# nathancunn/ParticleMDI.jl

Hardware: AMD Instinct MI355X
Metric: Gibbs iters/sec (and obs·particles/sec) at 1/2/4/8 GPUs vs CPU ref (higher is better)
Workload: dtype f64

## Files before the change

### include/pmdi_hip.h

```cpp
#ifndef PMDI_HIP_H
#define PMDI_HIP_H

#include <stdint.h>

#ifdef __cplusplus
extern "C" {
#endif

#define PMDI_ABI_VERSION 2
#define PMDI_KMAX 8

enum { PMDI_GAUSSIAN = 0, PMDI_CATEGORICAL = 1, PMDI_NEGBINOM = 2 };

enum {
    PMDI_OK = 0,
    PMDI_E_ARG = -1,
    PMDI_E_DEVICE = -2,
    PMDI_E_MEMORY = -3,
    PMDI_E_POOL = -4,
    PMDI_E_DATA = -5,
    PMDI_E_STATE = -6
};

typedef struct {
    int32_t kind;
    int32_t D;
    int64_t ld;
    const double  *xf;
    const int64_t *xi;
} pmdi_dataset;

typedef struct {
    int32_t settled;
    int32_t continue_inplace;
    int32_t sticky;
    int32_t light_ids;
    int32_t s2_cols, s2_idcap, s2_cls;
    int32_t ksplit;
    int32_t requeue_ksplit;
    int32_t split;
    int32_t heavy_threads;
    int32_t two_per_cu;
    int32_t very_heavy;
    int32_t start_gate;
    int32_t terms_cap;
    int32_t lds_target;
    int32_t phase_timers;
    int32_t profiled;
    int32_t ticket;
    int32_t reserved[5];
} pmdi_tuning;

typedef struct {
    int32_t abi_version;
    int32_t device;
    int32_t K;
    int32_t N;
    int32_t P;
    int32_t n_chains;
    int64_t n;
    uint64_t seed;
    int32_t q1_mode;
    int32_t q2_mode;
    int64_t pool_cap;
    int32_t block_threads;
    int32_t reserved;
    const pmdi_tuning *tuning;
} pmdi_config;

typedef struct pmdi_handle pmdi_handle;

typedef struct {
    int64_t n_operations;
    int64_t n_resamples;
    int64_t n_clones;
    int64_t max_id;
    int64_t sum_classes;
    int64_t steps_fast;
    int64_t steps_converted;
    int64_t steps_fallback;
} pmdi_sweep_stats;

int pmdi_create(const pmdi_config *cfg, const pmdi_dataset *datasets, pmdi_handle **out);

void pmdi_tuning_default(pmdi_tuning *t);
void pmdi_tuning_from_env(pmdi_tuning *t);
int pmdi_destroy(pmdi_handle *h);
const char *pmdi_last_error(void);
int pmdi_abi_version(void);

int pmdi_sweep(pmdi_handle *h, int64_t iter, const int64_t *s_in, const int64_t *order_obs,
               int64_t n1, const double *Pi, const double *Phi, const uint8_t *feature_flag,
               double lw_init, int64_t *s_out, double *logweight, int64_t *p_star,
               pmdi_sweep_stats *stats, double *trace);

int pmdi_sweep_device(pmdi_handle *h, int64_t iter, const int32_t *s_in, const int32_t *order_obs,
                      int64_t n1, const double *Pi, const double *log1p_phi,
                      const uint8_t *feature_flag, double lw_init, int32_t *s_out,
                      double *logweight, int32_t *p_star, int64_t *stats, int32_t *err,
                      void *stream);

int pmdi_feature_select(pmdi_handle *h, int64_t iter, const int64_t *s_traj,
                        uint8_t *feature_flag, double *feature_prob);

int pmdi_export_state(pmdi_handle *h, int32_t chain, int64_t *particle, int64_t *counts,
                      int64_t *cluster_n, int64_t *max_id);

typedef struct pmdi_cluster_batch pmdi_cluster_batch;
int pmdi_clusters_new(pmdi_handle *h, int32_t k, int32_t B, pmdi_cluster_batch **out);
int pmdi_clusters_free(pmdi_cluster_batch *cb);
int pmdi_cluster_add(pmdi_cluster_batch *cb, const int64_t *rows, const uint8_t *feature_flag);
int pmdi_calc_logprob(pmdi_cluster_batch *cb, const int64_t *obs_rows, const uint8_t *feature_flag,
                      double *out);
int pmdi_calc_logmarginal(pmdi_cluster_batch *cb, double *out );
int pmdi_cluster_stats(pmdi_cluster_batch *cb, double *out, int64_t *stride);

int pmdi_label_counts_device(pmdi_handle *h, const int32_t *s, int32_t *counts, void *stream);

int pmdi_psm_counts_device(int32_t device, const uint8_t *samples, int64_t S, int32_t K, int64_t n,
                           int64_t row_lo, int64_t row_hi, int32_t n_labels, int32_t *counts, void *stream);

enum { PMDI_LINK_SINGLE = 0, PMDI_LINK_AVERAGE = 1, PMDI_LINK_COMPLETE = 2, PMDI_LINK_WARD = 3 };
int pmdi_psm_distance_device(int32_t device, const int32_t *counts, int64_t S, int32_t K, int64_t n, int32_t which,
                             double *dist_out, void *stream);
int pmdi_hclust_device(int32_t device, double *dist, int32_t B, int64_t n, int32_t linkage, int64_t *merges_out,
                       double *heights_out, int64_t *order_out, void *stream);
int pmdi_cutree(int64_t n, const int64_t *merges, const double *heights, int64_t k, double h, int64_t *labels_out);

int pmdi_psm_score_device(int32_t device, const int32_t *counts, int64_t S, int32_t K, int64_t n, int32_t which,
                          const int32_t *cand, int64_t B, int64_t ld,
                          int64_t *agree_out , int64_t *pairs_out , int64_t *total_out ,
                          void *stream);

#define PMDI_REFINE_GMAX 4096
int pmdi_psm_rowscore_device(int32_t device, const int32_t *counts, int64_t S, int32_t K, int64_t n, int32_t which,
                             const int32_t *cand, int64_t B, int64_t ld,
                             int64_t *own_out , int32_t *size_out ,
                             int64_t *rowtotal_out , void *stream);
int pmdi_psm_refine_device(int32_t device, const int32_t *counts, int64_t S, int32_t K, int64_t n, int32_t which,
                           const int32_t *start, int64_t B, int64_t ld, int32_t max_sweeps,
                           int32_t *labels_out , int64_t *moves_out ,
                           int32_t *sweeps_out , void *stream);

int pmdi_vi_log2_table(int32_t *out );
int pmdi_psm_refine_vi_device(int32_t device, const int32_t *counts, int64_t S, int32_t K, int64_t n, int32_t which,
                              const int32_t *start, int64_t B, int64_t ld, int32_t max_sweeps,
                              int32_t *labels_out , int64_t *moves_out ,
                              int32_t *sweeps_out , int64_t *objective_out ,
                              void *stream);

#define PMDI_PARTDIST_GMAX 255
int pmdi_partition_rows_device(int32_t device, const void *labels , int32_t is_bytes, int64_t R, int64_t n, int64_t ld,
                               int32_t G, uint8_t *bytes_out , int64_t *pairs_out ,
                               int64_t *hl_out , int32_t *nclust_out , void *stream);
int pmdi_partition_distance_device(int32_t device, const uint8_t *cand_bytes , int64_t B, int32_t Gc,
                                   const uint8_t *draw_bytes , int64_t R, int32_t Gd, int64_t n,
                                   int64_t *both_out , int64_t *jl_out , void *stream);

int pmdi_partition_refine_device(int32_t device, const uint8_t *draw_bytes , int64_t R, int32_t Gd, int64_t n,
                                 const int32_t *start , int64_t B, int64_t ld, int32_t gcap, int32_t loss ,
                                 int32_t max_sweeps, int32_t *labels_out , int64_t *moves_out ,
                                 int32_t *sweeps_out , int32_t *converged_out ,
                                 int64_t *marginal_out , int64_t *joint_out , void *stream);

#define PMDI_BLOCKSUM_GMAX 2048
int pmdi_psm_blocksum_device(int32_t device, const int32_t *counts, int64_t S, int32_t K, int64_t n,
                             const int32_t *group , int32_t G,
                             int64_t *out , void *stream);

enum { PMDI_DATA_RAW = 0, PMDI_DATA_SQDEV = 1, PMDI_DATA_ZBIN = 2, PMDI_DATA_LEVELS = 3 };
int pmdi_data_groupsum_device(int32_t device, int32_t kind, const void *x, int64_t n, int32_t D, int64_t ld,
                              const int32_t *group , int32_t G, int32_t mode,
                              const double *shift , const double *scale ,
                              int32_t L, void *out , void *stream);

typedef struct pmdi_gibbs pmdi_gibbs;
int pmdi_gibbs_create(pmdi_handle *h, double rho, int32_t feature_select, pmdi_gibbs **out);
int pmdi_gibbs_destroy(pmdi_gibbs *g);

int pmdi_gibbs_iterate(pmdi_gibbs *g, int64_t n_iter, uint8_t *samples, void *stream);

int pmdi_gibbs_pack_samples(pmdi_gibbs *g, uint8_t *out, void *stream);

enum { PMDI_STEP_BEGIN = 0, PMDI_STEP_HYPERS = 1, PMDI_STEP_SWEEP = 2, PMDI_STEP_FEATSEL = 3, PMDI_STEP_ALIGN = 4 };
int pmdi_gibbs_step(pmdi_gibbs *g, int32_t what, void *stream);
int64_t pmdi_gibbs_iterations(const pmdi_gibbs *g);

int pmdi_gibbs_get(pmdi_gibbs *g, int32_t chain, double *M, double *gamma, double *gamma0, double *Phi, double *vZ,
                   int64_t *s, int64_t *order_obs, uint8_t *feature_flag);
int pmdi_gibbs_set(pmdi_gibbs *g, int32_t chain, const double *M, const double *gamma, const double *gamma0,
                   const double *Phi, const double *vZ, const int64_t *s, const int64_t *order_obs,
                   const uint8_t *feature_flag);
int pmdi_gibbs_results(pmdi_gibbs *g, int64_t *stats, int32_t *err, int64_t *p_star, double *logweight);

typedef struct pmdi_psm_acc pmdi_psm_acc;
int pmdi_psm_acc_create(int32_t device, int32_t K, int64_t n, int32_t n_labels, pmdi_psm_acc **out);
int pmdi_psm_acc_destroy(pmdi_psm_acc *a);
int pmdi_psm_acc_reset(pmdi_psm_acc *a, void *stream);
int pmdi_psm_acc_add_samples(pmdi_psm_acc *a, const uint8_t *samples, int64_t S, void *stream);
int pmdi_psm_acc_add_gibbs(pmdi_psm_acc *a, pmdi_gibbs *g, void *stream);
int pmdi_psm_acc_merge(pmdi_psm_acc *a, const int32_t *counts, int64_t S, void *stream);
int64_t pmdi_psm_acc_samples(const pmdi_psm_acc *a);
int pmdi_psm_acc_counts(pmdi_psm_acc *a, const int32_t **counts, int64_t *S, void *stream);

int pmdi_gibbs_run(pmdi_gibbs *g, int64_t n_iter, int64_t burnin, int64_t thin, pmdi_psm_acc *acc, void *stream);

typedef struct pmdi_summary pmdi_summary;
int pmdi_summary_create(int32_t device, int32_t n_chains, int32_t K, int32_t N, int64_t n, int64_t sumD, int64_t trace_cap,
                        pmdi_summary **out);
int pmdi_summary_destroy(pmdi_summary *a);
int pmdi_summary_reset(pmdi_summary *a, void *stream);
int pmdi_summary_add_gibbs(pmdi_summary *a, pmdi_gibbs *g, void *stream);
int pmdi_summary_add_arrays(pmdi_summary *a, const int32_t *s, const double *M, const double *Phi, const uint8_t *flags,
                            void *stream);
int64_t pmdi_summary_samples(const pmdi_summary *a);
int pmdi_summary_get(pmdi_summary *a, int64_t *nclust_hist, int64_t *nclust_sum, int64_t *nclust_sumsq, double *M_mean,
                     double *M_m2, double *Phi_mean, double *Phi_m2, int64_t *flag_count, int64_t *trace_nclust,
                     double *trace_M, double *trace_Phi, void *stream);

int pmdi_gibbs_run2(pmdi_gibbs *g, int64_t n_iter, int64_t burnin, int64_t thin, pmdi_psm_acc *acc, pmdi_summary *summ,
                    void *stream);

typedef struct pmdi_fusion pmdi_fusion;
int pmdi_fusion_create(int32_t device, int32_t K, int64_t n, int32_t n_labels, int32_t n_groups, const uint8_t *group_masks,
                       int32_t with_matrix, pmdi_fusion **out);
int pmdi_fusion_destroy(pmdi_fusion *a);
int pmdi_fusion_reset(pmdi_fusion *a, void *stream);
int pmdi_fusion_add_samples(pmdi_fusion *a, const uint8_t *samples, int64_t S, void *stream);
int pmdi_fusion_add_gibbs(pmdi_fusion *a, pmdi_gibbs *g, void *stream);
int pmdi_fusion_merge(pmdi_fusion *a, const int32_t *fused, const int32_t *counts, int64_t S, void *stream);
int64_t pmdi_fusion_samples(const pmdi_fusion *a);
int pmdi_fusion_groups(const pmdi_fusion *a, int32_t *n_groups, uint8_t *masks);
int pmdi_fusion_counts(pmdi_fusion *a, const int32_t **fused, const int32_t **counts, int64_t *S, void *stream);

int pmdi_gibbs_run3(pmdi_gibbs *g, int64_t n_iter, int64_t burnin, int64_t thin, pmdi_psm_acc *acc, pmdi_summary *summ,
                    pmdi_fusion *fus, void *stream);

typedef struct pmdi_mixing pmdi_mixing;
int pmdi_mixing_create(int32_t device, int32_t n_chains, int32_t K, int32_t N, int64_t n, int32_t maxlag, pmdi_mixing **out);
int pmdi_mixing_destroy(pmdi_mixing *a);
int pmdi_mixing_reset(pmdi_mixing *a, void *stream);
int pmdi_mixing_add_gibbs(pmdi_mixing *a, pmdi_gibbs *g, void *stream);
int pmdi_mixing_add_arrays(pmdi_mixing *a, const int32_t *s, const double *M, const double *Phi, void *stream);
int64_t pmdi_mixing_samples(const pmdi_mixing *a);
int pmdi_mixing_get(pmdi_mixing *a, int64_t *rand_num, double *ari_sum, double *sum_y, double *prod, double *head, double *tail,
                    double *first, void *stream);

int pmdi_gibbs_run4(pmdi_gibbs *g, int64_t n_iter, int64_t burnin, int64_t thin, pmdi_psm_acc *acc, pmdi_summary *summ,
                    pmdi_fusion *fus, pmdi_mixing *mix, void *stream);

#define PMDI_PREDICT_MMAX 1048576
#define PMDI_PREDICT_MAX_BYTES 34359738368LL
typedef struct pmdi_predict pmdi_predict;
int pmdi_predict_create(pmdi_handle *h, int64_t m, const pmdi_dataset *new_rows, int32_t keep_last, pmdi_predict **out);
int pmdi_predict_destroy(pmdi_predict *a);
int pmdi_predict_reset(pmdi_predict *a, void *stream);
int64_t pmdi_predict_samples(const pmdi_predict *a);
int pmdi_predict_add_gibbs(pmdi_predict *a, pmdi_gibbs *g, void *stream);
int pmdi_predict_add_arrays(pmdi_predict *a, const int32_t *s, const double *Pi, const uint8_t *flags, void *stream);
int pmdi_predict_merge(pmdi_predict *a, const int64_t *sim, const int64_t *new_cluster, const double *lpd_sum, int64_t T, void *stream);
int pmdi_predict_get(pmdi_predict *a, int64_t *sim, int64_t *new_cluster, double *lpd_sum, void *stream);
int pmdi_predict_counts(pmdi_predict *a, const int64_t **sim_device, int64_t *T, void *stream);
int pmdi_predict_last(pmdi_predict *a, double *lp, double *inc, int32_t *q);
int pmdi_predict_create_coupled(pmdi_handle *h, int64_t m, const pmdi_dataset *new_rows, int32_t keep_last, pmdi_predict **out);
int pmdi_predict_add_arrays_coupled(pmdi_predict *a, const int32_t *s, const double *Pi, const uint8_t *flags, const double *Phi, void *stream);
int pmdi_predict_merge_coupled(pmdi_predict *a, const int64_t *sim, const int64_t *new_cluster, const double *lpd_sum, const int64_t *sim_joint,
                               const int64_t *new_cluster_joint, const int64_t *fused_new, const double *lpd_joint_sum, int64_t T, void *stream);
int pmdi_predict_get_coupled(pmdi_predict *a, int64_t *sim_joint, int64_t *new_cluster_joint, int64_t *fused_new, double *lpd_joint_sum, void *stream);
int pmdi_predict_last_coupled(pmdi_predict *a, double *g, double *Z, int32_t *qj, int32_t *fq, double *incj, double *logZ0, double *Z0);
int pmdi_predict_create_masked(pmdi_handle *h, int64_t m, const pmdi_dataset *new_rows, const uint8_t *const *observed, int32_t keep_last,
                               int32_t coupled, int32_t impute, pmdi_predict **out);
int pmdi_predict_get_imputed(pmdi_predict *a, double *loc_sum, double *loc_joint_sum , int64_t *flag_on, void *stream);
int pmdi_predict_merge_imputed(pmdi_predict *a, const double *loc_sum, const double *loc_joint_sum ,
                               const int64_t *flag_on, void *stream);
int pmdi_predict_last_imputed(pmdi_predict *a, double *mu );

int pmdi_gibbs_run5(pmdi_gibbs *g, int64_t n_iter, int64_t burnin, int64_t thin, pmdi_psm_acc *acc, pmdi_summary *summ,
                    pmdi_fusion *fus, pmdi_mixing *mix, pmdi_predict *pred, void *stream);

#define PMDI_LOO_BUDGET_BYTES 268435456LL
#define PMDI_LOO_E_EMPTY (-9187201950435737472LL)
typedef struct pmdi_loo pmdi_loo;
int pmdi_loo_create(pmdi_handle *h, int32_t coupled, int32_t keep_last, pmdi_loo **out);
int pmdi_loo_destroy(pmdi_loo *a);
int pmdi_loo_reset(pmdi_loo *a, void *stream);
int64_t pmdi_loo_samples(const pmdi_loo *a);
int pmdi_loo_set_budget(pmdi_loo *a, int64_t bytes);
int pmdi_loo_add_gibbs(pmdi_loo *a, pmdi_gibbs *g, void *stream);
int pmdi_loo_add_arrays(pmdi_loo *a, const int32_t *s, const double *Pi, const uint8_t *flags, const double *Phi ,
                        void *stream);
int pmdi_loo_merge(pmdi_loo *a, const int64_t *own_sum, const int64_t *new_sum, const int64_t *zero, const double *lcp_sum,
                   const double *lcp_sq_sum, const int64_t *E, const int64_t *S , int64_t T, void *stream);
int pmdi_loo_get(pmdi_loo *a, int64_t *own_sum, int64_t *new_sum, int64_t *zero, double *lcp_sum, double *lcp_sq_sum, int64_t *E,
                 int64_t *S , void *stream);
int pmdi_loo_last(pmdi_loo *a, double *lp, double *ell, int32_t *p_own, int32_t *p_new, int64_t *e, double *mant);

int pmdi_gibbs_run6(pmdi_gibbs *g, int64_t n_iter, int64_t burnin, int64_t thin, pmdi_psm_acc *acc, pmdi_summary *summ,
                    pmdi_fusion *fus, pmdi_mixing *mix, pmdi_predict *pred, pmdi_loo *loo, void *stream);

typedef struct {
    double *M, *gamma, *gamma0, *Phi, *vZ, *Pi, *log1p_phi, *feature_prob, *logweight;
    int32_t *s, *order_obs, *p_star, *err;
    int64_t *stats;
    uint8_t *feature_flag;
    int64_t n1;
} pmdi_gibbs_view;
int pmdi_gibbs_device_view(pmdi_gibbs *g, pmdi_gibbs_view *v);

typedef struct pmdi_csv pmdi_csv;
int pmdi_csv_open(const char *path, int32_t K, int64_t n, const char *const *data_names, pmdi_csv **out);
int pmdi_csv_write_row(pmdi_csv *w, const double *M, const double *Phi, double ll, const int64_t *s);
int pmdi_csv_write_gibbs(pmdi_csv *w, pmdi_gibbs *g, int32_t chain, double ll);
int pmdi_csv_open_features(const char *path, int32_t K, const int32_t *D, const char *const *data_names, pmdi_csv **out);
int pmdi_csv_write_flags(pmdi_csv *w, const uint8_t *flags);
int pmdi_csv_close(pmdi_csv *w);
int pmdi_csv_read_allocations(const char *path, int64_t burnin, int64_t thin, int32_t *K_out, int64_t *n_obs_out,
                              int64_t *n_iter_out, uint8_t *labels, int64_t labels_cap, char *names, int32_t names_cap);

int pmdi_format_float64(double x, char *out, int32_t cap);

#define PMDI_COMM_ID_BYTES 128
typedef struct pmdi_comm pmdi_comm;
int pmdi_comm_unique_id(uint8_t id[PMDI_COMM_ID_BYTES]);
int pmdi_comm_init_rank(int32_t device, int32_t n_ranks, int32_t rank, const uint8_t id[PMDI_COMM_ID_BYTES], pmdi_comm **out);
int pmdi_comm_init_all(int32_t n_devices, const int32_t *devices, pmdi_comm **out);
int pmdi_comm_destroy(pmdi_comm *c);
int pmdi_comm_rank(const pmdi_comm *c);
int pmdi_comm_size(const pmdi_comm *c);
int pmdi_allgather_samples(pmdi_comm *const *comms, int32_t n_local, const uint8_t *const *send, uint8_t *const *recv,
                           int64_t bytes_per_rank, void *const *streams);

int pmdi_phase_timers(pmdi_handle *h, int32_t chain, int64_t *out16);

int pmdi_chain_costs(pmdi_handle *h, int64_t *out);

int pmdi_work_counters(pmdi_handle *h, int64_t *out);

int pmdi_settled_kernel(pmdi_handle *h, int64_t *given_back4);

int pmdi_chain_swept_by(pmdi_handle *h, int32_t *out);

int pmdi_sweep_layout(const pmdi_handle *h, int32_t *out32);

int pmdi_sum_D(const pmdi_handle *h);
int pmdi_block_threads(const pmdi_handle *h);
int pmdi_is_split(const pmdi_handle *h);
int64_t pmdi_shader_clock_hz(const pmdi_handle *h);
int64_t pmdi_lds_bytes(const pmdi_handle *h);
int64_t pmdi_pool_cap(const pmdi_handle *h);
int pmdi_categorical_L(const pmdi_handle *h, int32_t k);

#ifdef __cplusplus
}
#endif
#endif
```

### particlemdi.jl_amd/_lib.py

```python
import ctypes as C
import glob
import os
import subprocess

import numpy as np

_PKG = os.path.dirname(os.path.abspath(__file__))
_ROOT = os.path.dirname(_PKG)
LIB_PATH = os.environ.get("PMDI_LIB_PATH") or os.path.join(_PKG, "libpmdi_hip.so")
_SOURCES = [os.path.join(_PKG, "csrc", f) for f in ("pmdi_sweep.hip", "pmdi_sweep2.hip", "pmdi_kernels.hip", "pmdi_psm_acc.hip", "pmdi_fusion.hip", "pmdi_summary.hip", "pmdi_mixing.hip", "pmdi_predict.hip", "pmdi_predict_coupled.hip", "pmdi_loo.hip", "pmdi_hypers.hip", "pmdi_hclust.hip", "pmdi_psm_score.hip", "pmdi_psm_rowscore.hip", "pmdi_psm_refine.hip", "pmdi_psm_refine_vi.hip", "pmdi_partdist.hip", "pmdi_partdist_refine.hip", "pmdi_psm_blocksum.hip", "pmdi_data_groupsum.hip", "pmdi_api.cpp", "pmdi_plan.cpp", "pmdi_acc.cpp", "pmdi_csv.cpp", "pmdi_comm.cpp")]
_HEADERS = sorted(glob.glob(os.path.join(_PKG, "csrc", "*.h"))) + [os.path.join(_ROOT, "include", "pmdi_hip.h")]

GAUSSIAN, CATEGORICAL, NEGBINOM = 0, 1, 2
KIND_BY_NAME = {"gaussian": GAUSSIAN, "categorical": CATEGORICAL, "negbinom": NEGBINOM,
                "GaussianCluster": GAUSSIAN, "CategoricalCluster": CATEGORICAL,
                "NegBinomCluster": NEGBINOM}
ABI_VERSION = 2
KMAX = 8
REFINE_GMAX = 4096
BLOCKSUM_GMAX = 2048
PARTDIST_GMAX = 255
DATA_RAW, DATA_SQDEV, DATA_ZBIN, DATA_LEVELS = 0, 1, 2, 3

EXPORTS = [
    "pmdi_create", "pmdi_destroy", "pmdi_last_error", "pmdi_abi_version", "pmdi_sweep",
    "pmdi_sweep_device", "pmdi_feature_select", "pmdi_export_state", "pmdi_clusters_new",
    "pmdi_clusters_free", "pmdi_cluster_add", "pmdi_calc_logprob", "pmdi_calc_logmarginal",
    "pmdi_cluster_stats", "pmdi_sum_D", "pmdi_pool_cap", "pmdi_categorical_L", "pmdi_phase_timers",
    "pmdi_block_threads", "pmdi_lds_bytes", "pmdi_chain_costs", "pmdi_label_counts_device", "pmdi_psm_counts_device",
    "pmdi_gibbs_create", "pmdi_gibbs_destroy", "pmdi_gibbs_iterate", "pmdi_gibbs_step", "pmdi_gibbs_iterations",
    "pmdi_gibbs_get", "pmdi_gibbs_set", "pmdi_gibbs_results", "pmdi_gibbs_device_view", "pmdi_gibbs_pack_samples",
    "pmdi_csv_open", "pmdi_csv_write_row", "pmdi_csv_write_gibbs", "pmdi_csv_open_features", "pmdi_csv_write_flags",
    "pmdi_csv_close", "pmdi_csv_read_allocations", "pmdi_format_float64", "pmdi_work_counters", "pmdi_shader_clock_hz", "pmdi_is_split",
    "pmdi_comm_unique_id", "pmdi_comm_init_rank", "pmdi_comm_init_all", "pmdi_comm_destroy", "pmdi_comm_rank", "pmdi_comm_size",
    "pmdi_allgather_samples", "pmdi_settled_kernel", "pmdi_chain_swept_by", "pmdi_tuning_default", "pmdi_tuning_from_env",
    "pmdi_psm_distance_device", "pmdi_hclust_device", "pmdi_cutree",
    "pmdi_psm_acc_create", "pmdi_psm_acc_destroy", "pmdi_psm_acc_reset", "pmdi_psm_acc_add_samples", "pmdi_psm_acc_add_gibbs",
    "pmdi_psm_acc_merge", "pmdi_psm_acc_samples", "pmdi_psm_acc_counts", "pmdi_gibbs_run",
    "pmdi_summary_create", "pmdi_summary_destroy", "pmdi_summary_reset", "pmdi_summary_add_gibbs", "pmdi_summary_add_arrays",
    "pmdi_summary_samples", "pmdi_summary_get", "pmdi_gibbs_run2",
    "pmdi_psm_score_device", "pmdi_psm_rowscore_device", "pmdi_psm_refine_device", "pmdi_vi_log2_table", "pmdi_psm_refine_vi_device",
    "pmdi_psm_blocksum_device", "pmdi_data_groupsum_device",
    "pmdi_fusion_create", "pmdi_fusion_destroy", "pmdi_fusion_reset", "pmdi_fusion_add_samples", "pmdi_fusion_add_gibbs",
    "pmdi_fusion_merge", "pmdi_fusion_samples", "pmdi_fusion_groups", "pmdi_fusion_counts", "pmdi_gibbs_run3",
    "pmdi_sweep_layout",
    "pmdi_mixing_create", "pmdi_mixing_destroy", "pmdi_mixing_reset", "pmdi_mixing_add_gibbs", "pmdi_mixing_add_arrays",
    "pmdi_mixing_samples", "pmdi_mixing_get", "pmdi_gibbs_run4",
    "pmdi_predict_create", "pmdi_predict_destroy", "pmdi_predict_reset", "pmdi_predict_samples", "pmdi_predict_add_gibbs",
    "pmdi_predict_add_arrays", "pmdi_predict_merge", "pmdi_predict_get", "pmdi_predict_counts", "pmdi_predict_last", "pmdi_gibbs_run5",
    "pmdi_predict_create_coupled", "pmdi_predict_add_arrays_coupled", "pmdi_predict_merge_coupled", "pmdi_predict_get_coupled",
    "pmdi_predict_last_coupled",
    "pmdi_predict_create_masked", "pmdi_predict_get_imputed", "pmdi_predict_merge_imputed", "pmdi_predict_last_imputed",
    "pmdi_partition_rows_device", "pmdi_partition_distance_device", "pmdi_partition_refine_device",
    "pmdi_loo_create", "pmdi_loo_destroy", "pmdi_loo_reset", "pmdi_loo_samples", "pmdi_loo_set_budget", "pmdi_loo_add_gibbs",
    "pmdi_loo_add_arrays", "pmdi_loo_merge", "pmdi_loo_get", "pmdi_loo_last", "pmdi_gibbs_run6",
]


def build(force=False, verbose=False):
    if os.environ.get("PMDI_NO_BUILD") and os.path.exists(LIB_PATH):
        return LIB_PATH
    hipcc = os.environ.get("HIPCC", "/opt/rocm/bin/hipcc")
    extra = os.environ.get("PMDI_EXTRA_HIPCC_FLAGS", "").split()
    bdir = os.path.join(_PKG, "build" if not os.environ.get("PMDI_LIB_PATH") else "build_ab")
    if not force and _up_to_date(extra, bdir):
        return LIB_PATH
    os.makedirs(bdir, exist_ok=True)
    import fcntl
    with open(os.path.join(bdir, ".lock"), "w") as lock:
        fcntl.flock(lock, fcntl.LOCK_EX)
        return _build_locked(force, verbose, hipcc, extra, bdir)


def _up_to_date(extra, bdir):
    stamp = os.path.join(bdir, "flags.txt")
    if not os.path.exists(stamp) or not os.path.exists(LIB_PATH) or open(stamp).read() != " ".join(extra):
        return False
    hdr_time = max(os.path.getmtime(p) for p in _HEADERS)
    objs = [os.path.join(bdir, os.path.basename(src) + ".o") for src in _SOURCES]
    if not all(os.path.exists(o) and os.path.getmtime(o) >= max(os.path.getmtime(src), hdr_time) for o, src in zip(objs, _SOURCES)):
        return False
    return os.path.getmtime(LIB_PATH) >= max(os.path.getmtime(o) for o in objs)


def _build_locked(force, verbose, hipcc, extra, bdir):
    hdr_time = max(os.path.getmtime(p) for p in _HEADERS)
    stamp = os.path.join(bdir, "flags.txt")
    flags_now = " ".join(extra)
    if not os.path.exists(stamp) or open(stamp).read() != flags_now:
        force = True
    procs, objs = [], []
    for src in _SOURCES:
        obj = os.path.join(bdir, os.path.basename(src) + ".o")
        objs.append(obj)
        if (not force and os.path.exists(obj) and os.path.getmtime(obj) >= max(os.path.getmtime(src), hdr_time)):
            continue
        cmd = [hipcc, "--offload-arch=gfx950", "-O3", "-std=c++17", "-ffp-contract=off", "-fPIC", "-x", "hip",
               "-c", src, "-o", obj] + extra
        if verbose:
            print(" ".join(cmd))
        procs.append((cmd, subprocess.Popen(cmd)))
    failed = [cmd for cmd, p in procs if p.wait() != 0]
    if failed:
        raise subprocess.CalledProcessError(1, failed[0])
    if procs or not os.path.exists(LIB_PATH) or os.path.getmtime(LIB_PATH) < max(os.path.getmtime(o) for o in objs):
        cmd = [hipcc, "--offload-arch=gfx950", "-fPIC", "-shared", "-o", LIB_PATH] + objs
        if verbose:
            print(" ".join(cmd))
        subprocess.check_call(cmd)
        with open(stamp, "w") as f:
            f.write(flags_now)
    return LIB_PATH


class PmdiError(RuntimeError):
    def __init__(self, code, msg):
        super().__init__(f"[{code}] {msg}")
        self.code = code


class _Dataset(C.Structure):
    _fields_ = [("kind", C.c_int32), ("D", C.c_int32), ("ld", C.c_int64),
                ("xf", C.POINTER(C.c_double)), ("xi", C.POINTER(C.c_int64))]


class _Tuning(C.Structure):
    _fields_ = [(name, C.c_int32) for name in (
        "settled", "continue_inplace", "sticky", "light_ids", "s2_cols", "s2_idcap", "s2_cls", "ksplit", "requeue_ksplit", "split",
        "heavy_threads", "two_per_cu", "very_heavy", "start_gate", "terms_cap", "lds_target", "phase_timers", "profiled", "ticket")] + [("reserved", C.c_int32 * 5)]


class _Config(C.Structure):
    _fields_ = [("abi_version", C.c_int32), ("device", C.c_int32), ("K", C.c_int32),
                ("N", C.c_int32), ("P", C.c_int32), ("n_chains", C.c_int32), ("n", C.c_int64),
                ("seed", C.c_uint64), ("q1_mode", C.c_int32), ("q2_mode", C.c_int32),
                ("pool_cap", C.c_int64), ("block_threads", C.c_int32), ("reserved", C.c_int32),
                ("tuning", C.POINTER(_Tuning))]


class SweepStats(C.Structure):
    _fields_ = [("n_operations", C.c_int64), ("n_resamples", C.c_int64), ("n_clones", C.c_int64),
                ("max_id", C.c_int64), ("sum_classes", C.c_int64), ("steps_fast", C.c_int64),
                ("steps_converted", C.c_int64), ("steps_fallback", C.c_int64)]

    def as_dict(self):
        return {f: getattr(self, f) for f, _ in self._fields_}


_lib = None


def lib():
    global _lib
    if _lib is not None:
        return _lib
    if not os.path.exists(LIB_PATH):
        raise PmdiError(-2, f"{LIB_PATH} is missing: run __graft_entry__.build() (hipcc --offload-arch=gfx950)")
    if not os.environ.get("PMDI_NO_TORCH_PRELOAD"):
        try:
            import torch
        except Exception:
            pass
    L = C.CDLL(LIB_PATH)
    vp, i32, i64, dbl = C.c_void_p, C.c_int32, C.c_int64, C.c_double
    L.pmdi_last_error.restype = C.c_char_p
    L.pmdi_abi_version.restype = C.c_int
    L.pmdi_create.restype = C.c_int
    L.pmdi_create.argtypes = [C.POINTER(_Config), C.POINTER(_Dataset), C.POINTER(vp)]
    L.pmdi_destroy.argtypes = [vp]
    L.pmdi_sweep.restype = C.c_int
    L.pmdi_sweep.argtypes = [vp, i64, vp, vp, i64, vp, vp, vp, dbl, vp, vp, vp, vp, vp]
    L.pmdi_sweep_device.restype = C.c_int
    L.pmdi_sweep_device.argtypes = [vp, i64, vp, vp, i64, vp, vp, vp, dbl, vp, vp, vp, vp, vp, vp]
    L.pmdi_feature_select.restype = C.c_int
    L.pmdi_feature_select.argtypes = [vp, i64, vp, vp, vp]
    L.pmdi_export_state.restype = C.c_int
    L.pmdi_export_state.argtypes = [vp, i32, vp, vp, vp, vp]
    L.pmdi_clusters_new.restype = C.c_int
    L.pmdi_clusters_new.argtypes = [vp, i32, i32, C.POINTER(vp)]
    L.pmdi_clusters_free.argtypes = [vp]
    L.pmdi_cluster_add.restype = C.c_int
    L.pmdi_cluster_add.argtypes = [vp, vp, vp]
    L.pmdi_calc_logprob.restype = C.c_int
    L.pmdi_calc_logprob.argtypes = [vp, vp, vp, vp]
    L.pmdi_calc_logmarginal.restype = C.c_int
    L.pmdi_calc_logmarginal.argtypes = [vp, vp]
    L.pmdi_cluster_stats.restype = C.c_int
    L.pmdi_cluster_stats.argtypes = [vp, vp, vp]
    L.pmdi_sum_D.restype = C.c_int
    L.pmdi_sum_D.argtypes = [vp]
    L.pmdi_pool_cap.restype = i64
    L.pmdi_pool_cap.argtypes = [vp]
    L.pmdi_categorical_L.restype = C.c_int
    L.pmdi_categorical_L.argtypes = [vp, i32]
    L.pmdi_block_threads.restype = C.c_int
    L.pmdi_block_threads.argtypes = [vp]
    L.pmdi_lds_bytes.restype = i64
    L.pmdi_lds_bytes.argtypes = [vp]
    L.pmdi_psm_counts_device.restype = C.c_int
    L.pmdi_psm_counts_device.argtypes = [C.c_int32, vp, C.c_int64, C.c_int32, C.c_int64, C.c_int64, C.c_int64, C.c_int32, vp, vp]
    L.pmdi_label_counts_device.restype = C.c_int
    L.pmdi_label_counts_device.argtypes = [vp, vp, vp, vp]
    L.pmdi_psm_distance_device.restype = C.c_int
    L.pmdi_psm_distance_device.argtypes = [i32, vp, i64, i32, i64, i32, vp, vp]
    L.pmdi_hclust_device.restype = C.c_int
    L.pmdi_hclust_device.argtypes = [i32, vp, i32, i64, i32, vp, vp, vp, vp]
    L.pmdi_psm_score_device.restype = C.c_int
    L.pmdi_psm_score_device.argtypes = [i32, vp, i64, i32, i64, i32, vp, i64, i64, vp, vp, vp, vp]
    L.pmdi_psm_rowscore_device.restype = C.c_int
    L.pmdi_psm_rowscore_device.argtypes = [i32, vp, i64, i32, i64, i32, vp, i64, i64, vp, vp, vp, vp]
    L.pmdi_psm_refine_device.restype = C.c_int
    L.pmdi_psm_refine_device.argtypes = [i32, vp, i64, i32, i64, i32, vp, i64, i64, i32, vp, vp, vp, vp]
    L.pmdi_vi_log2_table.restype = C.c_int
    L.pmdi_vi_log2_table.argtypes = [vp]
    L.pmdi_psm_refine_vi_device.restype = C.c_int
    L.pmdi_psm_refine_vi_device.argtypes = [i32, vp, i64, i32, i64, i32, vp, i64, i64, i32, vp, vp, vp, vp, vp]
    L.pmdi_partition_rows_device.restype = C.c_int
    L.pmdi_partition_rows_device.argtypes = [i32, vp, i32, i64, i64, i64, i32, vp, vp, vp, vp, vp]
    L.pmdi_partition_distance_device.restype = C.c_int
    L.pmdi_partition_distance_device.argtypes = [i32, vp, i64, i32, vp, i64, i32, i64, vp, vp, vp]
    L.pmdi_partition_refine_device.restype = C.c_int
    L.pmdi_partition_refine_device.argtypes = [i32, vp, i64, i32, i64, vp, i64, i64, i32, i32, i32, vp, vp, vp, vp, vp, vp, vp]
    L.pmdi_psm_blocksum_device.restype = C.c_int
    L.pmdi_psm_blocksum_device.argtypes = [i32, vp, i64, i32, i64, vp, i32, vp, vp]
    L.pmdi_data_groupsum_device.restype = C.c_int
    L.pmdi_data_groupsum_device.argtypes = [i32, i32, vp, i64, i32, i64, vp, i32, i32, vp, vp, i32, vp, vp]
    L.pmdi_cutree.restype = C.c_int
    L.pmdi_cutree.argtypes = [i64, vp, vp, i64, dbl, vp]
    L.pmdi_psm_acc_create.restype = C.c_int
    L.pmdi_psm_acc_create.argtypes = [i32, i32, i64, i32, C.POINTER(vp)]
    L.pmdi_psm_acc_destroy.argtypes = [vp]
    L.pmdi_psm_acc_reset.restype = C.c_int
    L.pmdi_psm_acc_reset.argtypes = [vp, vp]
    L.pmdi_psm_acc_add_samples.restype = C.c_int
    L.pmdi_psm_acc_add_samples.argtypes = [vp, vp, i64, vp]
    L.pmdi_psm_acc_add_gibbs.restype = C.c_int
    L.pmdi_psm_acc_add_gibbs.argtypes = [vp, vp, vp]
    L.pmdi_psm_acc_merge.restype = C.c_int
    L.pmdi_psm_acc_merge.argtypes = [vp, vp, i64, vp]
    L.pmdi_psm_acc_samples.restype = i64
    L.pmdi_psm_acc_samples.argtypes = [vp]
    L.pmdi_psm_acc_counts.restype = C.c_int
    L.pmdi_psm_acc_counts.argtypes = [vp, C.POINTER(vp), C.POINTER(i64), vp]
    L.pmdi_gibbs_run.restype = C.c_int
    L.pmdi_gibbs_run.argtypes = [vp, i64, i64, i64, vp, vp]
    L.pmdi_gibbs_run2.restype = C.c_int
    L.pmdi_gibbs_run2.argtypes = [vp, i64, i64, i64, vp, vp, vp]
    L.pmdi_gibbs_run3.restype = C.c_int
    L.pmdi_gibbs_run3.argtypes = [vp, i64, i64, i64, vp, vp, vp, vp]
    L.pmdi_gibbs_run4.restype = C.c_int
    L.pmdi_gibbs_run4.argtypes = [vp, i64, i64, i64, vp, vp, vp, vp, vp]
    L.pmdi_gibbs_run5.restype = C.c_int
    L.pmdi_gibbs_run5.argtypes = [vp, i64, i64, i64, vp, vp, vp, vp, vp, vp]
    L.pmdi_gibbs_run6.restype = C.c_int
    L.pmdi_gibbs_run6.argtypes = [vp, i64, i64, i64, vp, vp, vp, vp, vp, vp, vp]
    L.pmdi_loo_create.restype = C.c_int
    L.pmdi_loo_create.argtypes = [vp, i32, i32, C.POINTER(vp)]
    L.pmdi_loo_destroy.argtypes = [vp]
    L.pmdi_loo_reset.restype = C.c_int
    L.pmdi_loo_reset.argtypes = [vp, vp]
    L.pmdi_loo_samples.restype = i64
    L.pmdi_loo_samples.argtypes = [vp]
    L.pmdi_loo_set_budget.restype = C.c_int
    L.pmdi_loo_set_budget.argtypes = [vp, i64]
    L.pmdi_loo_add_gibbs.restype = C.c_int
    L.pmdi_loo_add_gibbs.argtypes = [vp, vp, vp]
    L.pmdi_loo_add_arrays.restype = C.c_int
    L.pmdi_loo_add_arrays.argtypes = [vp, vp, vp, vp, vp, vp]
    L.pmdi_loo_merge.restype = C.c_int
    L.pmdi_loo_merge.argtypes = [vp] + [vp] * 7 + [i64, vp]
    L.pmdi_loo_get.restype = C.c_int
    L.pmdi_loo_get.argtypes = [vp] + [vp] * 7 + [vp]
    L.pmdi_loo_last.restype = C.c_int
    L.pmdi_loo_last.argtypes = [vp] + [vp] * 6
    L.pmdi_predict_create.restype = C.c_int
    L.pmdi_predict_create.argtypes = [vp, i64, C.POINTER(_Dataset), i32, C.POINTER(vp)]
    L.pmdi_predict_destroy.argtypes = [vp]
    L.pmdi_predict_reset.restype = C.c_int
    L.pmdi_predict_reset.argtypes = [vp, vp]
    L.pmdi_predict_samples.restype = i64
    L.pmdi_predict_samples.argtypes = [vp]
    L.pmdi_predict_add_gibbs.restype = C.c_int
    L.pmdi_predict_add_gibbs.argtypes = [vp, vp, vp]
    L.pmdi_predict_add_arrays.restype = C.c_int
    L.pmdi_predict_add_arrays.argtypes = [vp, vp, vp, vp, vp]
    L.pmdi_predict_merge.restype = C.c_int
    L.pmdi_predict_merge.argtypes = [vp, vp, vp, vp, i64, vp]
    L.pmdi_predict_get.restype = C.c_int
    L.pmdi_predict_get.argtypes = [vp, vp, vp, vp, vp]
    L.pmdi_predict_counts.restype = C.c_int
    L.pmdi_predict_counts.argtypes = [vp, C.POINTER(vp), C.POINTER(i64), vp]
    L.pmdi_predict_last.restype = C.c_int
    L.pmdi_predict_last.argtypes = [vp, vp, vp, vp]
    L.pmdi_predict_create_coupled.restype = C.c_int
    L.pmdi_predict_create_coupled.argtypes = [vp, i64, C.POINTER(_Dataset), i32, C.POINTER(vp)]
    L.pmdi_predict_add_arrays_coupled.restype = C.c_int
    L.pmdi_predict_add_arrays_coupled.argtypes = [vp, vp, vp, vp, vp, vp]
    L.pmdi_predict_merge_coupled.restype = C.c_int
    L.pmdi_predict_merge_coupled.argtypes = [vp] + [vp] * 7 + [i64, vp]
    L.pmdi_predict_get_coupled.restype = C.c_int
    L.pmdi_predict_get_coupled.argtypes = [vp, vp, vp, vp, vp, vp]
    L.pmdi_predict_last_coupled.restype = C.c_int
    L.pmdi_predict_last_coupled.argtypes = [vp] + [vp] * 7
    L.pmdi_predict_create_masked.restype = C.c_int
    L.pmdi_predict_create_masked.argtypes = [vp, i64, C.POINTER(_Dataset), C.POINTER(vp), i32, i32, i32, C.POINTER(vp)]
    L.pmdi_predict_get_imputed.restype = C.c_int
    L.pmdi_predict_get_imputed.argtypes = [vp, vp, vp, vp, vp]
    L.pmdi_predict_merge_imputed.restype = C.c_int
    L.pmdi_predict_merge_imputed.argtypes = [vp, vp, vp, vp, vp]
    L.pmdi_predict_last_imputed.restype = C.c_int
    L.pmdi_predict_last_imputed.argtypes = [vp, vp]
    L.pmdi_mixing_create.restype = C.c_int
    L.pmdi_mixing_create.argtypes = [i32, i32, i32, i32, i64, i32, C.POINTER(vp)]
    L.pmdi_mixing_destroy.argtypes = [vp]
    L.pmdi_mixing_reset.restype = C.c_int
    L.pmdi_mixing_reset.argtypes = [vp, vp]
    L.pmdi_mixing_add_gibbs.restype = C.c_int
    L.pmdi_mixing_add_gibbs.argtypes = [vp, vp, vp]
    L.pmdi_mixing_add_arrays.restype = C.c_int
    L.pmdi_mixing_add_arrays.argtypes = [vp, vp, vp, vp, vp]
    L.pmdi_mixing_samples.restype = i64
    L.pmdi_mixing_samples.argtypes = [vp]
    L.pmdi_mixing_get.restype = C.c_int
    L.pmdi_mixing_get.argtypes = [vp] + [vp] * 7 + [vp]
    L.pmdi_fusion_create.restype = C.c_int
    L.pmdi_fusion_create.argtypes = [i32, i32, i64, i32, i32, vp, i32, C.POINTER(vp)]
    L.pmdi_fusion_destroy.argtypes = [vp]
    L.pmdi_fusion_reset.restype = C.c_int
    L.pmdi_fusion_reset.argtypes = [vp, vp]
    L.pmdi_fusion_add_samples.restype = C.c_int
    L.pmdi_fusion_add_samples.argtypes = [vp, vp, i64, vp]
    L.pmdi_fusion_add_gibbs.restype = C.c_int
    L.pmdi_fusion_add_gibbs.argtypes = [vp, vp, vp]
    L.pmdi_fusion_merge.restype = C.c_int
    L.pmdi_fusion_merge.argtypes = [vp, vp, vp, i64, vp]
    L.pmdi_fusion_samples.restype = i64
    L.pmdi_fusion_samples.argtypes = [vp]
    L.pmdi_fusion_groups.restype = C.c_int
    L.pmdi_fusion_groups.argtypes = [vp, C.POINTER(i32), vp]
    L.pmdi_fusion_counts.restype = C.c_int
    L.pmdi_fusion_counts.argtypes = [vp, C.POINTER(vp), C.POINTER(vp), C.POINTER(i64), vp]
    L.pmdi_summary_create.restype = C.c_int
    L.pmdi_summary_create.argtypes = [i32, i32, i32, i32, i64, i64, i64, C.POINTER(vp)]
    L.pmdi_summary_destroy.argtypes = [vp]
    L.pmdi_summary_reset.restype = C.c_int
    L.pmdi_summary_reset.argtypes = [vp, vp]
    L.pmdi_summary_add_gibbs.restype = C.c_int
    L.pmdi_summary_add_gibbs.argtypes = [vp, vp, vp]
    L.pmdi_summary_add_arrays.restype = C.c_int
    L.pmdi_summary_add_arrays.argtypes = [vp, vp, vp, vp, vp, vp]
    L.pmdi_summary_samples.restype = i64
    L.pmdi_summary_samples.argtypes = [vp]
    L.pmdi_summary_get.restype = C.c_int
    L.pmdi_summary_get.argtypes = [vp] + [vp] * 11 + [vp]
    L.pmdi_chain_costs.restype = C.c_int
    L.pmdi_chain_costs.argtypes = [vp, vp]
    L.pmdi_comm_unique_id.restype = C.c_int
    L.pmdi_comm_unique_id.argtypes = [vp]
    L.pmdi_comm_init_rank.restype = C.c_int
    L.pmdi_comm_init_rank.argtypes = [i32, i32, i32, vp, C.POINTER(vp)]
    L.pmdi_comm_init_all.restype = C.c_int
    L.pmdi_comm_init_all.argtypes = [i32, vp, vp]
    L.pmdi_comm_destroy.argtypes = [vp]
    L.pmdi_comm_rank.argtypes = [vp]
    L.pmdi_comm_size.argtypes = [vp]
    L.pmdi_allgather_samples.restype = C.c_int
    L.pmdi_allgather_samples.argtypes = [vp, i32, vp, vp, i64, vp]
    L.pmdi_is_split.argtypes = [vp]
    L.pmdi_sweep_layout.restype = C.c_int
    L.pmdi_sweep_layout.argtypes = [vp, vp]
    L.pmdi_settled_kernel.restype = C.c_int
    L.pmdi_settled_kernel.argtypes = [vp, vp]
    L.pmdi_chain_swept_by.restype = C.c_int
    L.pmdi_chain_swept_by.argtypes = [vp, vp]
    L.pmdi_tuning_default.restype = None
    L.pmdi_tuning_default.argtypes = [C.POINTER(_Tuning)]
    L.pmdi_tuning_from_env.restype = None
    L.pmdi_tuning_from_env.argtypes = [C.POINTER(_Tuning)]
    L.pmdi_shader_clock_hz.restype = i64
    L.pmdi_shader_clock_hz.argtypes = [vp]
    L.pmdi_work_counters.restype = C.c_int
    L.pmdi_work_counters.argtypes = [vp, vp]
    L.pmdi_phase_timers.restype = C.c_int
    L.pmdi_phase_timers.argtypes = [vp, i32, vp]
    L.pmdi_gibbs_create.restype = C.c_int
    L.pmdi_gibbs_create.argtypes = [vp, dbl, i32, C.POINTER(vp)]
    L.pmdi_gibbs_destroy.argtypes = [vp]
    L.pmdi_gibbs_iterate.restype = C.c_int
    L.pmdi_gibbs_iterate.argtypes = [vp, i64, vp, vp]
    L.pmdi_gibbs_step.restype = C.c_int
    L.pmdi_gibbs_step.argtypes = [vp, i32, vp]
    L.pmdi_gibbs_iterations.restype = i64
    L.pmdi_gibbs_iterations.argtypes = [vp]
    L.pmdi_gibbs_get.restype = C.c_int
    L.pmdi_gibbs_get.argtypes = [vp, i32] + [vp] * 8
    L.pmdi_gibbs_set.restype = C.c_int
    L.pmdi_gibbs_set.argtypes = [vp, i32] + [vp] * 8
    L.pmdi_gibbs_results.restype = C.c_int
    L.pmdi_gibbs_results.argtypes = [vp, vp, vp, vp, vp]
    L.pmdi_gibbs_device_view.restype = C.c_int
    L.pmdi_gibbs_device_view.argtypes = [vp, vp]
    L.pmdi_gibbs_pack_samples.restype = C.c_int
    L.pmdi_gibbs_pack_samples.argtypes = [vp, vp, vp]
    L.pmdi_csv_open.restype = C.c_int
    L.pmdi_csv_open.argtypes = [C.c_char_p, i32, i64, vp, C.POINTER(vp)]
    L.pmdi_csv_write_row.restype = C.c_int
    L.pmdi_csv_write_row.argtypes = [vp, vp, vp, dbl, vp]
    L.pmdi_csv_write_gibbs.restype = C.c_int
    L.pmdi_csv_write_gibbs.argtypes = [vp, vp, i32, dbl]
    L.pmdi_csv_open_features.restype = C.c_int
    L.pmdi_csv_open_features.argtypes = [C.c_char_p, i32, vp, vp, C.POINTER(vp)]
    L.pmdi_csv_write_flags.restype = C.c_int
    L.pmdi_csv_write_flags.argtypes = [vp, vp]
    L.pmdi_csv_close.argtypes = [vp]
    L.pmdi_csv_read_allocations.restype = C.c_int
    L.pmdi_csv_read_allocations.argtypes = [C.c_char_p, i64, i64, vp, vp, vp, vp, i64, C.c_char_p, i32]
    L.pmdi_format_float64.restype = C.c_int
    L.pmdi_format_float64.argtypes = [dbl, C.c_char_p, i32]
    _lib = L
    return L


def _check(rc):
    if rc != 0:
        raise PmdiError(rc, lib().pmdi_last_error().decode())


def _ptr(a):
    return a.ctypes.data_as(C.c_void_p) if a is not None else None


class _Handle:
    _prefix = _destroy = None
    h = None

    def close(self):
        if self.h:
            getattr(lib(), self._destroy or self._prefix + "_destroy")(self.h)
            self.h = None

    def __del__(self):
        try:
            self.close()
        except Exception:
            pass


class _Accumulator(_Handle):

    def _stream(self):
        import torch
        return C.c_void_p(torch.cuda.current_stream(torch.device("cuda", self.device)).cuda_stream)

    def _samples(self):
        return int(getattr(lib(), self._prefix + "_samples")(self.h))

    def reset(self):
        _check(getattr(lib(), self._prefix + "_reset")(self.h, self._stream()))

    def add_gibbs(self, gibbs):
        _check(getattr(lib(), self._prefix + "_add_gibbs")(self.h, gibbs.h, self._stream()))

    def _checked_tensor(self, t, dtype, shape, what):
        if t is None or not t.is_cuda or t.dtype != dtype or t.dim() != len(shape) or (t.device.index or 0) != self.device \
                or any(want is not None and want != got for want, got in zip(shape, t.shape)):
            got = "None" if t is None else f"{t.dtype} {tuple(t.shape)} on {t.device}"
            want = "(" + ", ".join("*" if w is None else str(w) for w in shape) + ")"
            raise ValueError(f"{type(self).__name__}.{what} must be a CUDA {dtype} tensor {want} on device {self.device}, not {got}")
        return t.contiguous()


class Sweeper(_Handle):
    _destroy = "pmdi_destroy"

    def __init__(self, data, kinds, N, P, n_chains=1, seed=0, device=0, q1_mode=0, q2_mode=0,
                 pool_cap=0, block_threads=0, tuning=None):
        known = {name for name, _ in _Tuning._fields_} - {"reserved"}
        for name in (tuning or {}):
            if name not in known:
                raise KeyError(f"unknown tuning knob {name!r}; pmdi_tuning has {sorted(known)}")
        L = lib()
        self.K = len(data)
        if self.K > KMAX:
            raise PmdiError(-1, f"K={self.K} > {KMAX}")
        self.n = int(data[0].shape[0])
        self.N, self.P, self.C = int(N), int(P), int(n_chains)
        self.D = [int(x.shape[1]) for x in data]
        self.kinds = [KIND_BY_NAME.get(k, k) for k in kinds]
        if len(self.kinds) != self.K:
            raise PmdiError(-1, "Number of datatypes not equal to number of datasets")
        ds = (_Dataset * self.K)()
        self._keep = []
        for k, (x, kind) in enumerate(zip(data, self.kinds)):
            if x.shape[0] != self.n:
                raise PmdiError(-1, "Datasets don't have same number of observations.")
            ds[k].kind, ds[k].D, ds[k].ld = kind, x.shape[1], self.n
            if kind == GAUSSIAN:
                xf = np.asfortranarray(x, dtype=np.float64)
                self._keep.append(xf)
                ds[k].xf = xf.ctypes.data_as(C.POINTER(C.c_double))
            else:
                xi = np.asfortranarray(x, dtype=np.int64)
                self._keep.append(xi)
                ds[k].xi = xi.ctypes.data_as(C.POINTER(C.c_int64))
        self.device = int(device)
        tun = _Tuning()
        L.pmdi_tuning_from_env(C.byref(tun))
        for name, value in (tuning or {}).items():
            setattr(tun, name, int(value))
        cfg = _Config(ABI_VERSION, device, self.K, self.N, self.P, self.C, self.n, int(seed),
                      q1_mode, q2_mode, int(pool_cap), int(block_threads), 0, C.pointer(tun))
        h = C.c_void_p()
        _check(L.pmdi_create(C.byref(cfg), ds, C.byref(h)))
        self.h = h
        self.sumD = L.pmdi_sum_D(h)
        self.cap = L.pmdi_pool_cap(h)
        self.block_threads = L.pmdi_block_threads(h)
        self.lds_bytes = L.pmdi_lds_bytes(h)
        self.clock_hz = L.pmdi_shader_clock_hz(h)
        self.split = bool(L.pmdi_is_split(h))
        self.settled = bool(L.pmdi_settled_kernel(h, None))
        self.npairs = max(1, self.K * (self.K - 1) // 2)
        self.column_sums = [np.array([np.cumsum(x[:, q])[-1] for q in range(x.shape[1])]) if kind == GAUSSIAN else np.zeros(x.shape[1])
                            for x, kind in zip(self._keep, self.kinds)]
        self._keep = None

    def sweep(self, it, s, order_obs, n1, Pi, Phi, flags=None, lw_init=None, trace=False):
        C_, K, n, N, P = self.C, self.K, self.n, self.N, self.P
        s_a = np.asarray(s, dtype=np.int64).reshape(C_, n, K)
        s_in = np.ascontiguousarray(np.transpose(s_a, (0, 2, 1)))
        order = np.ascontiguousarray(np.asarray(order_obs, dtype=np.int64).reshape(C_, n))
        Pi_a = np.asarray(Pi, dtype=np.float64).reshape(C_, N, K)
        Pi_in = np.ascontiguousarray(np.transpose(Pi_a, (0, 2, 1)))
        Phi_in = np.ascontiguousarray(np.asarray(Phi, dtype=np.float64).reshape(C_, self.npairs))
        fl = None
        if flags is not None:
            fl = np.ascontiguousarray(np.asarray(flags, dtype=np.uint8).reshape(C_, self.sumD))
        if lw_init is None:
            lw_init = 0.0 if it == 1 else 1.0
        s_out = np.zeros((C_, K, n), dtype=np.int64)
        lw = np.zeros((C_, P), dtype=np.float64)
        p_star = np.zeros(C_, dtype=np.int64)
        st = (SweepStats * C_)()
        tr = np.zeros((C_, n - n1 + 1, 2 + 2 * K), dtype=np.float64) if trace else None
        _check(lib().pmdi_sweep(self.h, int(it), _ptr(s_in), _ptr(order), int(n1), _ptr(Pi_in),
                                _ptr(Phi_in), _ptr(fl), float(lw_init), _ptr(s_out), _ptr(lw),
                                _ptr(p_star), C.cast(st, C.c_void_p), _ptr(tr)))
        out = {"s": np.transpose(s_out, (0, 2, 1)).copy(), "logweight": lw, "p_star": p_star,
               "stats": [st[c].as_dict() for c in range(C_)]}
        if trace:
            out["trace"] = tr
        return out

    def feature_select(self, it, s_traj):
        C_, K, n = self.C, self.K, self.n
        s_a = np.asarray(s_traj, dtype=np.int64).reshape(C_, n, K)
        s_in = np.ascontiguousarray(np.transpose(s_a, (0, 2, 1)))
        flags = np.zeros((C_, self.sumD), dtype=np.uint8)
        prob = np.zeros((C_, self.sumD), dtype=np.float64)
        _check(lib().pmdi_feature_select(self.h, int(it), _ptr(s_in), _ptr(flags), _ptr(prob)))
        return flags, prob

    def export_state(self, chain=0):
        K, N, P, cap = self.K, self.N, self.P, self.cap
        particle = np.zeros((K, P, N), dtype=np.int64)
        counts = np.zeros((K, cap), dtype=np.int64)
        cn = np.zeros((K, cap), dtype=np.int64)
        mx = np.zeros(K, dtype=np.int64)
        _check(lib().pmdi_export_state(self.h, int(chain), _ptr(particle), _ptr(counts), _ptr(cn), _ptr(mx)))
        return {"particle": particle, "counts": counts, "cluster_n": cn, "max_id": mx}

    def label_counts(self, s):
        import torch
        s0 = np.ascontiguousarray(np.asarray(s).reshape(self.C, self.K, self.n) - 1, dtype=np.int32)
        dev = torch.device("cuda", self.device)
        ds = torch.from_numpy(s0).to(dev)
        out = torch.zeros((self.C, self.K, self.N), dtype=torch.int32, device=dev)
        st = torch.cuda.current_stream(dev)
        _check(lib().pmdi_label_counts_device(self.h, C.c_void_p(ds.data_ptr()), C.c_void_p(out.data_ptr()),
                                              C.c_void_p(st.cuda_stream)))
        return out.cpu().numpy().astype(np.int64)

    def layout(self):
        v = np.zeros(32, dtype=np.int32)
        _check(lib().pmdi_sweep_layout(self.h, _ptr(v)))
        v = [int(x) for x in v]
        group = lambda g: dict(zip(("threads", "terms_cap", "pid_lds", "pp_lds", "col_lds"), g)) if g[0] else None
        out = {"wide": group(v[0:5]), "light": group(v[5:10]), "handover": group(v[10:15]),
               "two_per_cu": v[15], "split": v[16], "ksplit": v[17], "ksplit_batch": v[18], "very_heavy": v[19], "start_gate": v[20],
               "s2_ok": v[21], "s2": None, "continue_inplace": None, "requeue_ksplit": None}
        if v[21]:
            out["s2"] = {"cols_l": v[22], "idcap": v[23], "cls": v[24], "cdfl": v[25], "threads": v[26], "lds_bytes": v[27]}
            out["continue_inplace"], out["requeue_ksplit"] = v[28], v[29]
        return out

    def given_back(self):
        out = np.zeros(4, dtype=np.int64)
        lib().pmdi_settled_kernel(self.h, _ptr(out))
        return out

    def swept_by(self):
        out = np.zeros(self.C, dtype=np.int32)
        _check(lib().pmdi_chain_swept_by(self.h, _ptr(out)))
        return out

    def chain_costs(self):
        out = np.zeros(self.C, dtype=np.int64)
        _check(lib().pmdi_chain_costs(self.h, _ptr(out)))
        return out

    def work_counters(self):
        out = np.zeros((self.C, self.K, 8), dtype=np.int64)
        _check(lib().pmdi_work_counters(self.h, _ptr(out)))
        return out

    def phase_timers(self, chain=0):
        out = np.zeros(16, dtype=np.int64)
        _check(lib().pmdi_phase_timers(self.h, int(chain), _ptr(out)))
        return out

    def clusters(self, k, B):
        return ClusterBatch(self, k, B)


class CsvWriter(_Handle):
    _destroy = "pmdi_csv_close"

    def __init__(self, path, K, n, data_names=None, feature_D=None):
        names = None
        if data_names is not None:
            names = (C.c_char_p * K)(*[str(x).encode() for x in data_names])
        h = C.c_void_p()
        if feature_D is None:
            _check(lib().pmdi_csv_open(str(path).encode(), int(K), int(n), names, C.byref(h)))
        else:
            D = np.ascontiguousarray(feature_D, dtype=np.int32)
            _check(lib().pmdi_csv_open_features(str(path).encode(), int(K), _ptr(D), names, C.byref(h)))
        self.h = h

    def row(self, M, Phi, ll, s):
        M = np.ascontiguousarray(M, dtype=np.float64); Phi = np.ascontiguousarray(Phi, dtype=np.float64)
        s_ = np.ascontiguousarray(np.asarray(s, dtype=np.int64).T)
        _check(lib().pmdi_csv_write_row(self.h, _ptr(M), _ptr(Phi), float(ll), _ptr(s_)))

    def gibbs_row(self, gibbs, chain, ll):
        _check(lib().pmdi_csv_write_gibbs(self.h, gibbs.h, int(chain), float(ll)))

    def flags(self, fl):
        f = np.ascontiguousarray(fl, dtype=np.uint8)
        _check(lib().pmdi_csv_write_flags(self.h, _ptr(f)))


def read_allocations(path, burnin=0, thin=1):
    K, n, S = C.c_int32(0), C.c_int64(0), C.c_int64(0)
    names = C.create_string_buffer(1 << 16)
    pth = str(path).encode()
    _check(lib().pmdi_csv_read_allocations(pth, int(burnin), int(thin), C.byref(K), C.byref(n), C.byref(S), None, 0, names, len(names)))
    out = np.zeros((S.value, K.value, n.value), dtype=np.uint8)
    _check(lib().pmdi_csv_read_allocations(pth, int(burnin), int(thin), C.byref(K), C.byref(n), C.byref(S), _ptr(out), out.size, None, 0))
    return out, names.value.decode().split("\n")


def format_float64(x):
    buf = C.create_string_buffer(64)
    k = lib().pmdi_format_float64(float(x), buf, 64)
    if k < 0:
        raise PmdiError(k, lib().pmdi_last_error().decode())
    return buf.value.decode()


class Comm(_Handle):
    _destroy = "pmdi_comm_destroy"

    def __init__(self, device, n_ranks, rank, unique_id):
        uid = np.ascontiguousarray(unique_id, dtype=np.uint8)
        h = C.c_void_p()
        _check(lib().pmdi_comm_init_rank(int(device), int(n_ranks), int(rank), _ptr(uid), C.byref(h)))
        self.h, self.n_ranks, self.rank = h, int(n_ranks), int(rank)

    @staticmethod
    def unique_id():
        uid = np.zeros(128, dtype=np.uint8)
        _check(lib().pmdi_comm_unique_id(_ptr(uid)))
        return uid

    def allgather(self, send_ptr, recv_ptr, bytes_per_rank, stream=None):
        comms = (C.c_void_p * 1)(self.h)
        send = (C.c_void_p * 1)(send_ptr)
        recv = (C.c_void_p * 1)(recv_ptr)
        st = (C.c_void_p * 1)(stream or None)
        _check(lib().pmdi_allgather_samples(comms, 1, send, recv, int(bytes_per_rank), st))


class GibbsView(C.Structure):
    _fields_ = [(f, C.c_void_p) for f in ("M", "gamma", "gamma0", "Phi", "vZ", "Pi", "log1p_phi", "feature_prob", "logweight",
                                          "s", "order_obs", "p_star", "err", "stats", "feature_flag")] + [("n1", C.c_int64)]


STEP_BEGIN, STEP_HYPERS, STEP_SWEEP, STEP_FEATSEL, STEP_ALIGN = range(5)


class Gibbs(_Handle):
    _destroy = "pmdi_gibbs_destroy"

    def __init__(self, sweeper, rho=0.25, feature_select=False):
        self.sw = sweeper
        h = C.c_void_p()
        _check(lib().pmdi_gibbs_create(sweeper.h, float(rho), int(bool(feature_select)), C.byref(h)))
        self.h = h
        self.n1 = int(np.floor(rho * sweeper.n))

    def iterate(self, n_iter=1, samples_ptr=None, stream=None):
        _check(lib().pmdi_gibbs_iterate(self.h, int(n_iter), C.c_void_p(samples_ptr) if samples_ptr else None,
                                        C.c_void_p(stream) if stream else None))

    def run(self, n_iter, burnin=0, thin=1, acc=None, stream=None, summary=None, fusion=None, mixing=None, predict=None, loo=None):
        _check(lib().pmdi_gibbs_run6(self.h, int(n_iter), int(burnin), int(thin), acc.h if acc is not None else None,
                                     summary.h if summary is not None else None, fusion.h if fusion is not None else None,
                                     mixing.h if mixing is not None else None, predict.h if predict is not None else None,
                                     loo.h if loo is not None else None, C.c_void_p(stream) if stream else None))

    def pack_samples(self, out_ptr, stream=None):
        _check(lib().pmdi_gibbs_pack_samples(self.h, C.c_void_p(out_ptr), C.c_void_p(stream) if stream else None))

    def step(self, what, stream=None):
        _check(lib().pmdi_gibbs_step(self.h, int(what), C.c_void_p(stream) if stream else None))

    @property
    def iterations(self):
        return int(lib().pmdi_gibbs_iterations(self.h))

    def get(self, chain=0):
        sw = self.sw
        K, N, n = sw.K, sw.N, sw.n
        M = np.zeros(K); gam = np.zeros((K, N)); gam0 = np.zeros((K, N)); Phi = np.zeros(sw.npairs); vZ = np.zeros(2)
        s = np.zeros((K, n), dtype=np.int64); order = np.zeros(n, dtype=np.int64); fl = np.zeros(sw.sumD, dtype=np.uint8)
        _check(lib().pmdi_gibbs_get(self.h, int(chain), _ptr(M), _ptr(gam), _ptr(gam0), _ptr(Phi), _ptr(vZ), _ptr(s), _ptr(order), _ptr(fl)))
        return {"M": M, "gamma": gam.T.copy(), "gamma0": gam0.T.copy(), "Phi": Phi, "v": vZ[0], "Z": vZ[1],
                "s": s.T.copy(), "order": order, "flags": fl}

    def set(self, chain=0, M=None, gamma=None, gamma0=None, Phi=None, v=None, Z=None, s=None, order=None, flags=None):
        f64 = lambda a: None if a is None else np.ascontiguousarray(a, dtype=np.float64)
        vZ = None
        if v is not None or Z is not None:
            cur = self.get(chain)
            vZ = np.array([cur["v"] if v is None else v, cur["Z"] if Z is None else Z], dtype=np.float64)
        g = None if gamma is None else np.ascontiguousarray(np.asarray(gamma, dtype=np.float64).T)
        g0 = None if gamma0 is None else np.ascontiguousarray(np.asarray(gamma0, dtype=np.float64).T)
        s_ = None if s is None else np.ascontiguousarray(np.asarray(s, dtype=np.int64).T)
        o_ = None if order is None else np.ascontiguousarray(order, dtype=np.int64)
        fl = None if flags is None else np.ascontiguousarray(flags, dtype=np.uint8)
        _check(lib().pmdi_gibbs_set(self.h, int(chain), _ptr(f64(M)), _ptr(g), _ptr(g0), _ptr(f64(Phi)), _ptr(vZ), _ptr(s_), _ptr(o_), _ptr(fl)))

    def results(self, check=True):
        sw = self.sw
        stats = np.zeros((sw.C, 8), dtype=np.int64); err = np.zeros(sw.C, dtype=np.int32)
        ps = np.zeros(sw.C, dtype=np.int64); lw = np.zeros((sw.C, sw.P))
        rc = lib().pmdi_gibbs_results(self.h, _ptr(stats), _ptr(err), _ptr(ps), _ptr(lw))
# ... 45 lines not shown
```

### particlemdi.jl_amd/csrc/pmdi_api.cpp

```cpp
#include "pmdi_arith.h"
#include "pmdi_host.h"
#include "pmdi_data_groupsum_plan.h"
#include "pmdi_psm_blocksum_plan.h"
#include "pmdi_sweep_carve.h"

#include <cmath>
#include <cstdarg>
#include <cstdio>
#include <cstdlib>
#include <cstring>
#include <new>
#include <string>
#include <utility>
#include <vector>

#ifndef M_PI
#define M_PI 3.14159265358979323846
#endif

namespace {

thread_local char g_err[512] = "";

size_t align_up(size_t v, size_t a) { return (v + a - 1) / a * a; }

unsigned __int128 psm_divisor(int64_t S, int32_t K, int32_t which) { return (unsigned __int128)S * (unsigned)(which == K ? K : 1); }

size_t layout_arena(DsetDev &d, int N, int P, long long cap, long long n_rows_sstar, bool sweep_state)
{
    size_t o = 0;
    auto take = [&](size_t bytes) { size_t at = o; o = align_up(o + bytes, 256); return at; };
    const size_t ids = (size_t)cap + 1;
    if (sweep_state) {
        d.o_particle[0] = take((size_t)N * P * 4);
        d.o_particle[1] = take((size_t)N * P * 4);
        d.o_col = take((size_t)P * 4);
        d.o_cgrp = take((size_t)(N > 3 ? N : 3) * P * 8);
        d.o_pid = take((size_t)P * 4);
        d.o_sid = take((size_t)P * 4);
        d.o_kv = take((size_t)P * 4);
        d.o_newid = take((size_t)N * P * 4);
        d.o_counts = take(ids * 4);
        d.o_ncop = take(ids * 4);
        d.o_firstc = take(ids * 4);
        d.o_lp = take(ids * 8);
        d.o_sstar = take((size_t)n_rows_sstar * P);
        d.o_clslead = take((size_t)P * 4);
        d.o_clsval = take((size_t)P * 4);
        d.o_cdf = take((size_t)P * (N + 2) * 8);
        d.o_dl = take((size_t)3 * P * 4);
        d.o_s2x = take((size_t)2048 * 12);
    }
    d.o_cn = take(ids * 4);
    if (d.kind == K_GAUSSIAN) {
        if (!sweep_state) d.o_ml = take(ids * d.D * 16);
        d.o_sb = take(ids * d.D * 16);
    } else if (d.kind == K_CATEGORICAL) {
        d.o_cnt = take(ids * d.D * d.L * 4);
    } else {
        d.o_nbs = take(ids * d.D * 8);
    }
    return o;
}

}

int pmdi_set_error(int code, const char *fmt, ...)
{
    va_list ap;
    va_start(ap, fmt);
    vsnprintf(g_err, sizeof(g_err), fmt, ap);
    va_end(ap);
    return code;
}

int pmdi_psm_shared_args(const char *who, int64_t S, int32_t K, int64_t n, int32_t which, bool cand, int64_t B, int64_t ld)
{
    if (cand && (K < 1 || K > PMDI_KMAX || S < 1 || n < 1 || n > 65535 || B < 1 || ld < n))
        return fail(PMDI_E_ARG, "%s: S=%lld K=%d n=%lld B=%lld ld=%lld out of range (K <= %d, n <= 65535, ld >= n)", who,
                    (long long)S, K, (long long)n, (long long)B, (long long)ld, PMDI_KMAX);
    if (!cand && (S < 1 || K < 1 || n < 1 || n > 65535))
        return fail(PMDI_E_ARG, "%s: S=%lld K=%d n=%lld out of range (n <= 65535)", who, (long long)S, K, (long long)n);
    if (which < 0 || which > K || (which == K && K == 1))
        return fail(PMDI_E_ARG, "%s: which=%d, but there are %d matrices (the Overall one only for K > 1)", who, which, K + (K > 1));
    return PMDI_OK;
}

struct pmdi_cluster_batch {
    pmdi_handle *h = nullptr;
    int k = 0, B = 0;
    DsetDev d{};
    void *arena = nullptr;
    DevBuf d_rows, d_flags, d_out;
};

namespace {

int dev_alloc(pmdi_handle *h, void **p, size_t bytes)
{
    if (bytes == 0) bytes = 16;
    hipError_t e = hipMalloc(p, bytes);
    if (e != hipSuccess) { *p = nullptr; return fail(PMDI_E_MEMORY, "hipMalloc(%zu bytes): %s", bytes, hipGetErrorString(e)); }
    h->owned.push_back(*p);
    return 0;
}

template <class Tt>
int upload(pmdi_handle *h, const std::vector<Tt> &v, const Tt **out)
{
    void *p = nullptr;
    int rc = dev_alloc(h, &p, v.size() * sizeof(Tt));
    if (rc) return rc;
    if (!v.empty()) HIP_TRY(hipMemcpy(p, v.data(), v.size() * sizeof(Tt), hipMemcpyHostToDevice));
    *out = (const Tt *)p;
    return 0;
}

void fill_sweep_common(const pmdi_handle *h, SweepArgs &a)
{
    memset(&a, 0, sizeof(a));
    a.K = h->cfg.K; a.N = h->cfg.N; a.P = h->cfg.P; a.cap = (int)h->cap;
    a.Dmax = h->Dmax; a.sumD = h->sumD; a.npairs = h->npairs;
    a.q1 = h->cfg.q1_mode; a.q2 = h->cfg.q2_mode;
    const SweepPlan &pl = h->plan;
    pmdi_put_tables(pl.wide, a);
    a.item_cap = h->cfg.N > 32 ? PMDI_ITEM_CAP_BIGN : PMDI_ITEM_CAP;
    a.two_per_cu = pl.two_per_cu;
    a.phase = pl.phase_on ? (long long *)h->d_phase.p : nullptr;
    a.cost = (long long *)h->d_cost.p;
    a.work = (long long *)h->d_work.p;
    a.anclog = (int *)h->d_anclog.p; a.evpos = (int *)h->d_evpos.p;
    a.ksplit = pl.ksplit; a.xcnt = (int *)h->d_xcnt.p; a.xinc = (double *)h->d_xinc.p; a.xlab = (int *)h->d_xlab.p; a.xhdr = (unsigned long long *)h->d_xhdr.p;
    a.chain_order = h->have_order ? (const int *)h->d_lorder.p : nullptr;
    a.s2 = pl.s2;
    a.requeue = pl.s2_ok ? (int *)h->d_requeue.p : nullptr;
    a.requeue_total = pl.s2_ok ? (long long *)h->d_requeue_total.p : nullptr;
    a.handed = pl.s2_ok ? (int *)h->d_handed.p : nullptr;
    a.sweep_no = h->sweep_no;
    a.swept_by = (int *)h->d_swept_by.p;
    a.resume = (pl.s2_ok && pl.s2_continue) ? (int *)h->d_resume.p : nullptr;
    a.n = h->cfg.n;
    a.seed = h->cfg.seed;
    for (int k = 0; k < h->cfg.K; ++k) a.ds[k] = h->ds[k];
}

void fill_sweep_call(const pmdi_handle *h, SweepArgs &a, int64_t iter, int64_t n1, double lw_init, const int *s_in, const int *order,
                     const double *Pi, const double *logphi, const unsigned char *flags, int *s_out, double *lw_out, int *pstar,
                     long long *stats, int *err, double *trace)
{
    fill_sweep_common(h, a);
    a.iter = (unsigned)iter; a.n1 = n1; a.lw_init = lw_init;
    a.s_in = s_in; a.order = order; a.Pi = Pi; a.logphi = logphi; a.flags = flags;
    a.s_out = s_out; a.lw_out = lw_out;
    a.pstar = pstar ? pstar : (int *)h->d_pstar.p;
    a.stats = stats ? stats : (long long *)h->d_stats.p;
    a.err = err ? err : (int *)h->d_err.p;
    a.trace = trace; a.trace_on = trace ? 1 : 0;
    a.uscratch = (double *)h->d_usc.p; a.partstar = (int *)h->d_partstar.p; a.kstate = (int *)h->d_kstate.p;
}

SweepArgs *next_slot(pmdi_handle *h, hipStream_t st_of_copy, int *idx)
{
    (void)st_of_copy;
    if (!h->ring) { *idx = -1; return nullptr; }
    const int i = h->ring_head;
    h->ring_head = (i + 1) % pmdi_handle::RING;
    if (h->ring_used[i]) (void)hipEventSynchronize(h->ring_ev[i]);
    *idx = i;
    return h->ring + i;
}

hipError_t launch_one(pmdi_handle *h, const SweepArgs &a, SweepArgs *d_args, int n_chains, int T, hipStream_t st)
{
    int idx;
    SweepArgs *slot = next_slot(h, st, &idx);
    hipError_t e = pmdi_launch_sweep(a, d_args, n_chains, T, st, slot);
    if (e == hipSuccess && idx >= 0) { e = hipEventRecord(h->ring_ev[idx], st); h->ring_used[idx] = true; }
    return e;
}

hipError_t launch_maybe_batched(pmdi_handle *h, const SweepArgs &a, SweepArgs *d_args, int n_chains, int T, hipStream_t st)
{
    const int batch = h->plan.ksplit_batch;
    if (!a.ksplit || batch <= 0 || n_chains <= batch) return launch_one(h, a, d_args, n_chains, T, st);
    for (int b0 = 0; b0 < n_chains; b0 += batch) {
        SweepArgs ab = a;
        ab.n_slots = n_chains; ab.slot_base = b0;
        const int nb = (n_chains - b0 < batch) ? n_chains - b0 : batch;
        hipError_t e = launch_one(h, ab, d_args, nb, T, st);
        if (e != hipSuccess) return e;
    }
    return hipSuccess;
}

int launch_sweep_groups(pmdi_handle *h, SweepArgs &a, hipStream_t st)
{
    const int C = h->cfg.n_chains;
    const SweepPlan &pl = h->plan;
    auto args = [&](int which) { return (SweepArgs *)h->d_args[which].p; };
    hipError_t e;
    a.err_keep = h->err_keep;
    a.sweep_no = ++h->sweep_no;
    if (pl.s2_ok) HIP_TRY(hipMemsetAsync(h->d_requeue.p, 0, (size_t)C * 4, st));
    if (pl.ksplit) {
        HIP_TRY(hipMemsetAsync(h->d_xcnt.p, 0, (size_t)C * 32 * 4, st));
        HIP_TRY(hipMemsetAsync(a.stats, 0, (size_t)C * 64, st));
        if (!h->err_keep) HIP_TRY(hipMemsetAsync(a.err, 0, (size_t)C * 4, st));
    }
    if (!pl.split) {
        e = launch_maybe_batched(h, a, args(ARGS_MAIN), C, pl.T, st);
        if (e != hipSuccess) return fail(PMDI_E_DEVICE, "sweep launch: %s", hipGetErrorString(e));
    } else {
        HIP_TRY(hipEventRecord(h->ev_fork, st));
        a.group_flag = (const unsigned char *)h->d_group.p;
        a.group_sel = 1;
        const int vh = pl.very_heavy < C ? pl.very_heavy : C;
        if (vh > 0) {
            SweepArgs av = a;
            av.two_per_cu = 0; av.rank_lo = 0; av.rank_hi = vh;
            HIP_TRY(hipStreamWaitEvent(h->stream3, h->ev_fork, 0));
            const bool gate = h->start_sig != nullptr && !pl.ksplit;
            if (gate) av.start_sig = h->start_sig;
            e = launch_one(h, av, args(ARGS_HEAVIEST), vh, pl.T, h->stream3);
            if (e != hipSuccess) return fail(PMDI_E_DEVICE, "sweep launch (heaviest chains): %s", hipGetErrorString(e));
            HIP_TRY(hipEventRecord(h->ev_join3, h->stream3));
            if (gate) {
                const unsigned n_wg = (unsigned)vh;
                HIP_TRY(hipStreamWaitValue32(st, h->start_sig, n_wg, hipStreamWaitValueGte, 0xFFFFFFFFu));
                HIP_TRY(hipStreamWaitEvent(h->stream2, h->ev_fork, 0));
                HIP_TRY(hipStreamWaitValue32(h->stream2, h->start_sig, n_wg, hipStreamWaitValueGte, 0xFFFFFFFFu));
            }
        }
        a.rank_lo = vh; a.rank_hi = C;
        e = launch_maybe_batched(h, a, args(ARGS_MAIN), C, pl.T, st);
        if (e != hipSuccess) return fail(PMDI_E_DEVICE, "sweep launch (heavy group): %s", hipGetErrorString(e));
        if (vh > 0) HIP_TRY(hipStreamWaitEvent(st, h->ev_join3, 0));
        SweepArgs al = a;
        al.group_sel = 0; al.rank_lo = 0; al.rank_hi = C;
        pmdi_put_tables(pl.light, al);
        HIP_TRY(hipStreamWaitEvent(h->stream2, h->ev_fork, 0));
        if (pl.s2_ok) {
            pmdi_put_tables(pl.resume, al);
            int idx;
            SweepArgs *slot = next_slot(h, h->stream2, &idx);
            SweepArgs as = al;
            as.ticket = (h->tun.ticket != 0) ? (int *)h->d_ticket.p : nullptr;
            e = pmdi_launch_sweep2(as, args(ARGS_SETTLED), C, h->stream2, slot);
            if (e == hipSuccess && idx >= 0) { e = hipEventRecord(h->ring_ev[idx], h->stream2); h->ring_used[idx] = true; }
            if (e != hipSuccess) return fail(PMDI_E_DEVICE, "sweep launch (settled chains): %s", hipGetErrorString(e));
            if (!pl.s2_continue) {
                SweepArgs ar = al;
                ar.group_flag = nullptr; ar.requeue_only = 1;
                pmdi_put_tables(pl.light, ar);
                if (h->cfg.K > 1 && h->d_xcnt.p && pl.requeue_ksplit) {
                    ar.ksplit = 1;
                    HIP_TRY(hipMemsetAsync(h->d_xcnt.p, 0, (size_t)C * 32 * 4, h->stream2));
                }
                e = launch_one(h, ar, args(ARGS_GIVEN_BACK), C, 256, h->stream2);
                if (e != hipSuccess) return fail(PMDI_E_DEVICE, "sweep launch (chains given back by the settled-chain kernel): %s", hipGetErrorString(e));
            }
        } else {
            e = launch_maybe_batched(h, al, args(ARGS_LIGHT), C, 256, h->stream2);
            if (e != hipSuccess) return fail(PMDI_E_DEVICE, "sweep launch (light group): %s", hipGetErrorString(e));
        }
        HIP_TRY(hipEventRecord(h->ev_join, h->stream2));
        HIP_TRY(hipStreamWaitEvent(st, h->ev_join, 0));
        if (vh > 0 && h->start_sig && !pl.ksplit) HIP_TRY(hipStreamWriteValue32(st, h->start_sig, 0, 0));
    }
    if (C > 1 || pl.split) {
        const long long steps = (a.n - a.n1 + 1) * (long long)a.K;
        e = pmdi_launch_chain_order((const long long *)h->d_cost.p, (int *)h->d_lorder.p, a.stats,
                                    pl.split ? (unsigned char *)h->d_group.p : nullptr, pl.light_ids * steps, C, st,
                                    pl.s2_ok ? (const int *)h->d_handed.p : nullptr, h->sweep_no + 3 - pl.sticky);
        if (e != hipSuccess) return fail(PMDI_E_DEVICE, "chain-order launch: %s", hipGetErrorString(e));
        h->have_order = true;
    }
    return PMDI_OK;
}


int upload_dataset(pmdi_handle *h, int k, const pmdi_dataset &src)
{
    const int N = h->cfg.N, P = h->cfg.P;
    const long long n = h->cfg.n, cap = h->cap;
    DsetDev &d = h->ds[k];
    int rc = 0;
    if (src.D < 1) return fail(PMDI_E_ARG, "dataset %d: D=%d", k, src.D);
    if (src.ld < n) return fail(PMDI_E_ARG, "dataset %d: ld=%lld < n. Datasets don't have same number of observations.", k, (long long)src.ld);
    d.kind = src.kind; d.D = src.D; d.L = 0; d.flag_off = h->sumD;
    h->sumD += src.D;
    if (src.D > h->Dmax) h->Dmax = src.D;
    const int D = src.D;
    if (src.kind == PMDI_GAUSSIAN) {
        if (!src.xf) return fail(PMDI_E_ARG, "dataset %d: xf is null", k);
        std::vector<double> x((size_t)n * D);
        for (long long i = 0; i < n; ++i)
            for (int q = 0; q < D; ++q) x[(size_t)i * D + q] = src.xf[(size_t)q * src.ld + i];
        if ((rc = upload(h, x, &d.xf))) return rc;
        std::vector<double> g((size_t)n + 1), lm((size_t)n + 1);
        for (long long m = 0; m <= n; ++m) {
            const double nn = (double)m;
            g[m] = (log(1.0 / sqrt(M_PI)) + lgamma(0.5 * nn + 1.0)) - lgamma(0.5 * nn + 0.5);
            const double a_n = (nn / 2.0 + 0.5), a_0 = 0.5, b_0 = 0.5, k_0 = 0.001, k_n = nn + k_0;
            lm[m] = (a_0 * log(b_0)) + lgamma(a_n) - lgamma(a_0) + 0.5 * (log(k_0) - log(k_n)) -
                    (nn * 0.5) * log(2.0 * M_PI);
        }
        if ((rc = upload(h, g, &d.gtab))) return rc;
        if ((rc = upload(h, lm, &d.lmtab))) return rc;
    } else if (src.kind == PMDI_CATEGORICAL || src.kind == PMDI_NEGBINOM) {
        if (!src.xi) return fail(PMDI_E_ARG, "dataset %d: xi is null", k);
        std::vector<int> x((size_t)n * D);
        std::vector<int> maxcol(D, 0);
        std::vector<long long> colsum(D, 0);
        long long gmax = 0;
        for (long long i = 0; i < n; ++i)
            for (int q = 0; q < D; ++q) {
                const long long v = src.xi[(size_t)q * src.ld + i];
                if (src.kind == PMDI_CATEGORICAL && v < 1) return fail(PMDI_E_DATA, "dataset %d: categorical level %lld < 1", k, v);
                if (src.kind == PMDI_NEGBINOM && v < 0) return fail(PMDI_E_DATA, "dataset %d: negative count %lld", k, v);
                if (v > 0x3fffffff) return fail(PMDI_E_DATA, "dataset %d: value %lld too large", k, v);
                x[(size_t)i * D + q] = (int)v;
                if (v > maxcol[q]) maxcol[q] = (int)v;
                if (v > gmax) gmax = v;
                colsum[q] += v;
            }
        if ((rc = upload(h, x, &d.xi))) return rc;
        if (src.kind == PMDI_CATEGORICAL) {
            if (gmax > 4096) return fail(PMDI_E_DATA, "dataset %d: %lld categorical levels (max 4096)", k, gmax);
            d.L = (int)gmax;
            if ((rc = upload(h, maxcol, &d.maxcol))) return rc;
            std::vector<double> lh((size_t)(2 * n + gmax + 3)), lgh((size_t)(2 * (n + gmax) + 3));
            for (size_t j = 0; j < lh.size(); ++j) lh[j] = log(0.5 * (double)j);
            for (size_t j = 0; j < lgh.size(); ++j) lgh[j] = lgamma(0.5 * (double)j);
            if ((rc = upload(h, lh, &d.lhtab))) return rc;
            if ((rc = upload(h, lgh, &d.lghtab))) return rc;
        } else {
            long long smax = 0;
            for (int q = 0; q < D; ++q) if (colsum[q] > smax) smax = colsum[q];
            const long long len = n + gmax + smax + 8;
            if (len > (1LL << 27)) return fail(PMDI_E_DATA, "dataset %d: NegBinom lgamma table of %lld entries is too large", k, len);
            std::vector<double> lg((size_t)len);
            for (long long m = 0; m < len; ++m) lg[m] = lgamma((double)m);
            if ((rc = upload(h, lg, &d.lgtab))) return rc;
            d.lgtab_len = len;
        }
    } else {
        return fail(PMDI_E_ARG, "dataset %d: unknown kind %d", k, src.kind);
    }
    d.stride = layout_arena(d, N, P, cap, n, true);
    void *arena = nullptr;
    if ((rc = dev_alloc(h, &arena, d.stride * (size_t)h->cfg.n_chains))) return rc;
    d.arena = (char *)arena;
    if (hipMemset(arena, 0, d.stride * (size_t)h->cfg.n_chains) != hipSuccess) return fail(PMDI_E_DEVICE, "hipMemset failed");
    return PMDI_OK;
}

int create_launch_objects(pmdi_handle *h)
{
    if (!h->plan.split) return PMDI_OK;
    int prio_lo = 0, prio_hi = 0;
    (void)hipDeviceGetStreamPriorityRange(&prio_lo, &prio_hi);
    if (hipStreamCreateWithPriority(&h->stream2, hipStreamNonBlocking, prio_lo) != hipSuccess ||
        hipEventCreateWithFlags(&h->ev_fork, hipEventDisableTiming) != hipSuccess ||
        hipEventCreateWithFlags(&h->ev_join, hipEventDisableTiming) != hipSuccess ||
        hipStreamCreateWithPriority(&h->stream3, hipStreamNonBlocking, prio_hi) != hipSuccess ||
        hipEventCreateWithFlags(&h->ev_join3, hipEventDisableTiming) != hipSuccess)
        return fail(PMDI_E_DEVICE, "stream/event creation failed");
    void *sig = nullptr;
    if (h->plan.want_gate && hipExtMallocWithFlags(&sig, 8, hipMallocSignalMemory) == hipSuccess) {
        h->start_sig = (unsigned *)sig; h->owned.push_back(sig);
        (void)hipMemset(sig, 0, 8);
    }
    return PMDI_OK;
}

int alloc_sweep_state(pmdi_handle *h)
{
    const int K = h->cfg.K, P = h->cfg.P;
    const long long n = h->cfg.n;
    int rc = 0;
    const int C = h->cfg.n_chains;
    for (DevBuf &b : h->d_args) if ((rc = b.ensure(sizeof(SweepArgs)))) return rc;
    if ((rc = h->d_usc.ensure((size_t)C * K * P * 8)) || (rc = h->d_partstar.ensure((size_t)C * K * P * 4)) ||
        (rc = h->d_kstate.ensure((size_t)C * PMDI_KMAX_I * 2 * 4)) || (rc = h->d_err.ensure((size_t)C * 4)) ||
        (rc = h->d_stats.ensure((size_t)C * 8 * 8)) || (rc = h->d_pstar.ensure((size_t)C * 4)) ||
        (rc = h->d_phase.ensure((size_t)C * 16 * 8)) ||
        (rc = h->d_cost.ensure((size_t)C * 8)) || (rc = h->d_work.ensure((size_t)C * PMDI_KMAX_I * 8 * 8)) || (rc = h->d_lorder.ensure((size_t)C * 4)) || (rc = h->d_ticket.ensure(((size_t)C + 1) * 4)) ||
        (rc = h->d_group.ensure((size_t)C)) || (rc = h->d_requeue.ensure((size_t)C * 4)) ||
        (rc = h->d_requeue_total.ensure(4 * 8)) || (rc = h->d_handed.ensure((size_t)C * 4)) || (rc = h->d_swept_by.ensure((size_t)C * 4)) ||
        (rc = h->d_resume.ensure((size_t)C * 16 * 4)))
        return rc;
    if (hipMemset(h->d_swept_by.p, 0, (size_t)C * 4) != hipSuccess) return fail(PMDI_E_DEVICE, "hipMemset failed");
    {
        std::vector<int> never((size_t)C, -1000);
        if (hipMemcpy(h->d_handed.p, never.data(), (size_t)C * 4, hipMemcpyHostToDevice) != hipSuccess) return fail(PMDI_E_DEVICE, "memcpy failed");
    }
    if (hipMemset(h->d_requeue.p, 0, (size_t)C * 4) != hipSuccess || hipMemset(h->d_requeue_total.p, 0, 32) != hipSuccess)
        return fail(PMDI_E_DEVICE, "hipMemset failed");
    if (h->plan.want_xchg && ((rc = h->d_xcnt.ensure((size_t)C * 32 * 4)) || (rc = h->d_xinc.ensure((size_t)C * 2 * K * P * 8)) ||
                      (rc = h->d_xlab.ensure((size_t)C * 2 * K * P * 4)) || (rc = h->d_xhdr.ensure((size_t)C * 2 * K * 16))))
        return rc;
    if (h->cfg.q2_mode == 1 &&
        ((rc = h->d_anclog.ensure((size_t)C * (size_t)n * P * 4)) || (rc = h->d_evpos.ensure((size_t)C * 2 * (size_t)n * 4))))
        return rc;
    if (hipMemset(h->d_group.p, (h->plan.s2_ok && h->tun.settled == 2) ? 0 : 1, (size_t)C) != hipSuccess)
        return fail(PMDI_E_DEVICE, "hipMemset failed");
    return PMDI_OK;
}

void alloc_staging_ring(pmdi_handle *h)
{
    void *ring = nullptr;
    if (hipHostMalloc(&ring, sizeof(SweepArgs) * pmdi_handle::RING, hipHostMallocDefault) == hipSuccess) {
        h->ring = (SweepArgs *)ring;
        for (int i = 0; i < pmdi_handle::RING; ++i)
            if (hipEventCreateWithFlags(&h->ring_ev[i], hipEventDisableTiming) != hipSuccess) {
                for (int j = 0; j < i; ++j) { (void)hipEventDestroy(h->ring_ev[j]); h->ring_ev[j] = nullptr; }
                (void)hipHostFree(ring); h->ring = nullptr;
                break;
            }
    }
}

int null_marginal(pmdi_handle *h)
{
    const int K = h->cfg.K, N = h->cfg.N, C = h->cfg.n_chains;
    const long long n = h->cfg.n;
    int rc = 0;
    std::vector<int> traj((size_t)K * n, 0);
    if ((rc = h->d_traj.ensure((size_t)C * K * n * 4)) || (rc = h->d_lm.ensure((size_t)C * h->sumD * N * 8)) ||
        (rc = h->d_firstpos.ensure((size_t)C * K * N * 4)) || (rc = h->d_fnull.ensure((size_t)h->sumD * 8)) ||
        (rc = h->d_fflags.ensure((size_t)C * h->sumD)) || (rc = h->d_fprob.ensure((size_t)C * h->sumD * 8)))
        return rc;
    if (hipMemcpy(h->d_traj.p, traj.data(), traj.size() * 4, hipMemcpyHostToDevice) != hipSuccess) return fail(PMDI_E_DEVICE, "memcpy failed");
    std::vector<double> zero((size_t)h->sumD, 0.0);
    if (hipMemcpy(h->d_fnull.p, zero.data(), zero.size() * 8, hipMemcpyHostToDevice) != hipSuccess) return fail(PMDI_E_DEVICE, "memcpy failed");
    FeatSelArgs fa;
    memset(&fa, 0, sizeof(fa));
    fa.K = K; fa.N = 1; fa.sumD = h->sumD; fa.n = n; fa.iter = 0; fa.seed = h->cfg.seed;
    for (int k = 0; k < K; ++k) fa.ds[k] = h->ds[k];
    fa.traj = (const int *)h->d_traj.p; fa.lm = (double *)h->d_lm.p; fa.firstpos = (int *)h->d_firstpos.p;
    fa.fnull = (const double *)h->d_fnull.p; fa.flags_out = (unsigned char *)h->d_fflags.p; fa.prob_out = (double *)h->d_fprob.p;
    hipError_t e = pmdi_launch_featsel(fa, 1, h->stream);
    if (e != hipSuccess) return fail(PMDI_E_DEVICE, "null-marginal launch: %s", hipGetErrorString(e));
    if (hipStreamSynchronize(h->stream) != hipSuccess) return fail(PMDI_E_DEVICE, "null-marginal kernel failed");
    std::vector<double> lm((size_t)h->sumD);
    if (hipMemcpy(lm.data(), h->d_lm.p, lm.size() * 8, hipMemcpyDeviceToHost) != hipSuccess) return fail(PMDI_E_DEVICE, "memcpy failed");
    for (double &v : lm) v = -v;
    if (hipMemcpy(h->d_fnull.p, lm.data(), lm.size() * 8, hipMemcpyHostToDevice) != hipSuccess) return fail(PMDI_E_DEVICE, "memcpy failed");
    return PMDI_OK;
}

}

extern "C" {

const char *pmdi_last_error(void) { return g_err; }

void pmdi_tuning_default(pmdi_tuning *t)
{
    if (!t) return;
    int32_t *f = (int32_t *)t;
    for (size_t i = 0; i < sizeof(pmdi_tuning) / sizeof(int32_t); ++i) f[i] = -1;
}

void pmdi_tuning_from_env(pmdi_tuning *t)
{
    if (!t) return;
    pmdi_tuning_default(t);
    auto env = [](const char *name, int32_t &field) { const char *v = getenv(name); if (v && *v) field = (int32_t)atoi(v); };
    env("PMDI_SETTLED", t->settled); env("PMDI_CONTINUE", t->continue_inplace); env("PMDI_STICKY", t->sticky);
    env("PMDI_LIGHT_IDS", t->light_ids); env("PMDI_S2_COLS", t->s2_cols); env("PMDI_S2_IDCAP", t->s2_idcap); env("PMDI_S2_CLS", t->s2_cls);
    env("PMDI_KSPLIT", t->ksplit); env("PMDI_REQUEUE_KSPLIT", t->requeue_ksplit); env("PMDI_SPLIT", t->split);
    env("PMDI_HEAVY_T", t->heavy_threads); env("PMDI_TWO_PER_CU", t->two_per_cu); env("PMDI_VERY_HEAVY", t->very_heavy);
    env("PMDI_START_GATE", t->start_gate); env("PMDI_TICKET", t->ticket); env("PMDI_TERMS_CAP", t->terms_cap); env("PMDI_LDS_TARGET", t->lds_target);
    if (getenv("PMDI_PHASE_TIMERS")) t->phase_timers = 1;
    auto has = [](const char *name, const char *what) { const char *v = getenv(name); return v && strstr(v, what) != nullptr; };
    t->profiled = (has("LD_PRELOAD", "rocprof") || has("ROCP_TOOL_LIBRARIES", "rocprof") || has("HSA_TOOLS_LIB", "rocprof")) ? 1 : 0;
}
int pmdi_abi_version(void) { return PMDI_ABI_VERSION; }

int pmdi_destroy(pmdi_handle *h)
{
    if (!h) return PMDI_OK;
    if (h->children > 0)
        return fail(PMDI_E_STATE, "pmdi_destroy: %d object(s) created from this handle (pmdi_gibbs_create / pmdi_clusters_new) are still alive", h->children);
    (void)hipSetDevice(h->cfg.device);
    if (h->stream) (void)hipStreamSynchronize(h->stream);
    (void)hipDeviceSynchronize();
    for (int i = 0; i < pmdi_handle::RING; ++i) if (h->ring_ev[i]) (void)hipEventDestroy(h->ring_ev[i]);
    if (h->ring) (void)hipHostFree(h->ring);
    for (void *p : h->owned) (void)hipFree(p);
    if (h->stream) (void)hipStreamDestroy(h->stream);
    if (h->stream2) { (void)hipStreamSynchronize(h->stream2); (void)hipStreamDestroy(h->stream2); }
    if (h->stream3) { (void)hipStreamSynchronize(h->stream3); (void)hipStreamDestroy(h->stream3); }
    if (h->ev_join3) (void)hipEventDestroy(h->ev_join3);
    if (h->ev_fork) (void)hipEventDestroy(h->ev_fork);
    if (h->ev_join) (void)hipEventDestroy(h->ev_join);
    delete h;
    return PMDI_OK;
}

int pmdi_create(const pmdi_config *cfg, const pmdi_dataset *datasets, pmdi_handle **out)
{
    if (!cfg || !datasets || !out) return fail(PMDI_E_ARG, "null argument");
    *out = nullptr;
    if (cfg->abi_version != PMDI_ABI_VERSION) return fail(PMDI_E_ARG, "abi_version %d != %d", cfg->abi_version, PMDI_ABI_VERSION);
    const int K = cfg->K, N = cfg->N, P = cfg->P;
    const long long n = cfg->n;
    if (K < 1 || K > PMDI_KMAX_I) return fail(PMDI_E_ARG, "K=%d outside 1..%d", K, PMDI_KMAX_I);
    if (n < 2 || n > 0x7fffffffLL / 4) return fail(PMDI_E_ARG, "n=%lld out of range", n);
    if (!(N <= n && N > 1)) return fail(PMDI_E_ARG, "Number of clusters must be greater than 1 and not greater than the number of observations");
    if (N > 255) return fail(PMDI_E_ARG, "N=%d: this build supports N <= 255 (labels travel as bytes; the mutation CDF of a particle class is formed by one wave, up to four labels per lane, pairwise beyond 128 like Base.cumsum)", N);
    if (P < 2) return fail(PMDI_E_ARG, "Conditional particle filter requires 2 or more particles");
    if (P > 1048575) return fail(PMDI_E_ARG, "P=%d too large", P);
    if (cfg->n_chains < 1) return fail(PMDI_E_ARG, "n_chains must be >= 1");
    if (cfg->q1_mode < 0 || cfg->q1_mode > 1) return fail(PMDI_E_ARG, "q1_mode must be 0 or 1");
    if (cfg->q2_mode < 0 || cfg->q2_mode > 1) return fail(PMDI_E_ARG, "q2_mode must be 0 or 1");
    long long cap = cfg->pool_cap > 0 ? cfg->pool_cap : (long long)N * P + 1;
    if (cap > (long long)N * P + 1) cap = (long long)N * P + 1;
    if (cap < N + 2) return fail(PMDI_E_ARG, "pool_cap too small");

    int ndev = 0;
    if (hipGetDeviceCount(&ndev) != hipSuccess || ndev < 1)
        return fail(PMDI_E_DEVICE, "no HIP device visible (this library has no CPU path)");
    if (cfg->device < 0 || cfg->device >= ndev) return fail(PMDI_E_DEVICE, "device %d not in 0..%d", cfg->device, ndev - 1);
    HIP_TRY(hipSetDevice(cfg->device));
    hipDeviceProp_t prop;
    HIP_TRY(hipGetDeviceProperties(&prop, cfg->device));
    if (strncmp(prop.gcnArchName, "gfx950", 6) != 0)
        return fail(PMDI_E_DEVICE, "device %d is %s; the kernels are built for gfx950 only", cfg->device, prop.gcnArchName);

    pmdi_handle *h = new (std::nothrow) pmdi_handle();
    if (!h) return fail(PMDI_E_MEMORY, "out of host memory");
    h->cfg = *cfg;
    if (cfg->tuning) h->tun = *cfg->tuning; else pmdi_tuning_default(&h->tun);
    h->cfg.tuning = nullptr;
    h->cap = cap;
    h->npairs = K > 1 ? K * (K - 1) / 2 : 1;
    int rc = 0;
    auto bail = [&](int code) { pmdi_destroy(h); return code; };
    if (hipStreamCreateWithFlags(&h->stream, hipStreamNonBlocking) != hipSuccess) return bail(fail(PMDI_E_DEVICE, "hipStreamCreate failed"));

    for (int k = 0; k < K; ++k)
        if ((rc = upload_dataset(h, k, datasets[k]))) return bail(rc);
    PlanDevice dev;
    dev.cus = prop.multiProcessorCount;
    int can_wait = 0;
    (void)hipDeviceGetAttribute(&can_wait, hipDeviceAttributeCanUseStreamWaitValue, cfg->device);
    dev.wait_value = can_wait != 0;
    dev.blocks_per_cu = [](const SweepArgs &a, int T) { int blocks = 0; return pmdi_sweep_blocks_per_cu(a, T, &blocks) == hipSuccess ? blocks : 0; };
    if ((rc = pmdi_plan_sweep(h->cfg, h->tun, h->Dmax, cap, dev, &h->plan)) ||
        (rc = create_launch_objects(h)) || (rc = alloc_sweep_state(h)))
        return bail(rc);
    alloc_staging_ring(h);
    if ((rc = null_marginal(h))) return bail(rc);
    *out = h;
    return PMDI_OK;
}

int pmdi_phase_timers(pmdi_handle *h, int32_t chain, int64_t *out16)
{
    if (!h || !out16 || chain < 0 || chain >= h->cfg.n_chains) return fail(PMDI_E_ARG, "bad argument");
    if (!h->plan.phase_on) return fail(PMDI_E_STATE, "set PMDI_PHASE_TIMERS=1 before pmdi_create");
    HIP_TRY(hipSetDevice(h->cfg.device));
    HIP_TRY(hipDeviceSynchronize());
    HIP_TRY(hipMemcpy(out16, (char *)h->d_phase.p + (size_t)chain * 16 * 8, 16 * 8, hipMemcpyDeviceToHost));
    return PMDI_OK;
}

int pmdi_chain_costs(pmdi_handle *h, int64_t *out)
{
    if (!h || !out) return fail(PMDI_E_ARG, "null argument");
    HIP_TRY(hipSetDevice(h->cfg.device));
    HIP_TRY(hipDeviceSynchronize());
    HIP_TRY(hipMemcpy(out, h->d_cost.p, (size_t)h->cfg.n_chains * 8, hipMemcpyDeviceToHost));
    return PMDI_OK;
}
int pmdi_work_counters(pmdi_handle *h, int64_t *out)
{
    if (!h || !out) return fail(PMDI_E_ARG, "null argument");
    const int C = h->cfg.n_chains, K = h->cfg.K;
    HIP_TRY(hipSetDevice(h->cfg.device));
    HIP_TRY(hipDeviceSynchronize());
    std::vector<long long> w((size_t)C * PMDI_KMAX_I * 8);
    HIP_TRY(hipMemcpy(w.data(), h->d_work.p, w.size() * 8, hipMemcpyDeviceToHost));
    for (int c = 0; c < C; ++c)
        for (int k = 0; k < K; ++k)
            for (int j = 0; j < 8; ++j) out[((size_t)c * K + k) * 8 + j] = w[((size_t)c * PMDI_KMAX_I + k) * 8 + j];
    return PMDI_OK;
}
int pmdi_block_threads(const pmdi_handle *h) { return h ? h->plan.T : 0; }
int pmdi_is_split(const pmdi_handle *h) { return h ? h->plan.ksplit : 0; }
int64_t pmdi_shader_clock_hz(const pmdi_handle *h)
{
    if (!h) return 0;
    int khz = 0;
    if (hipDeviceGetAttribute(&khz, hipDeviceAttributeClockRate, h->cfg.device) != hipSuccess) return 0;
    return (int64_t)khz * 1000;
}
int64_t pmdi_lds_bytes(const pmdi_handle *h)
{
    if (!h) return 0;
    SweepArgs a;
    fill_sweep_common(h, a);
    return (int64_t)pmdi_sweep_lds_bytes(a, h->plan.T);
}
int pmdi_sweep_layout(const pmdi_handle *h, int32_t *out32)
{
    if (!h || !out32) return fail(PMDI_E_ARG, "null argument");
    pmdi_plan_layout32(h->plan, h->start_sig != nullptr, h->d_xcnt.p != nullptr, h->cfg.K, h->cfg.P, out32);
    return PMDI_OK;
}
int pmdi_sum_D(const pmdi_handle *h) { return h ? h->sumD : 0; }
int pmdi_settled_kernel(pmdi_handle *h, int64_t *given_back4)
{
    if (!h) return 0;
    if (given_back4) {
        given_back4[0] = given_back4[1] = given_back4[2] = given_back4[3] = 0;
        if (h->plan.s2_ok) {
            if (hipSetDevice(h->cfg.device) != hipSuccess || hipDeviceSynchronize() != hipSuccess ||
                hipMemcpy(given_back4, h->d_requeue_total.p, 32, hipMemcpyDeviceToHost) != hipSuccess)
                return fail(PMDI_E_DEVICE, "pmdi_settled_kernel: reading the counters failed");
        }
    }
    return h->plan.s2_ok ? 1 : 0;
}
int pmdi_chain_swept_by(pmdi_handle *h, int32_t *out)
{
    if (!h || !out) return fail(PMDI_E_ARG, "null argument");
    HIP_TRY(hipSetDevice(h->cfg.device));
    HIP_TRY(hipDeviceSynchronize());
    HIP_TRY(hipMemcpy(out, h->d_swept_by.p, (size_t)h->cfg.n_chains * 4, hipMemcpyDeviceToHost));
    return PMDI_OK;
}
int64_t pmdi_pool_cap(const pmdi_handle *h) { return h ? h->cap : 0; }
int pmdi_categorical_L(const pmdi_handle *h, int32_t k) { return (h && k >= 0 && k < h->cfg.K) ? h->ds[k].L : 0; }

int pmdi_sweep_device(pmdi_handle *h, int64_t iter, const int32_t *s_in, const int32_t *order_obs, int64_t n1,
                      const double *Pi, const double *log1p_phi, const uint8_t *feature_flag, double lw_init,
                      int32_t *s_out, double *logweight, int32_t *p_star, int64_t *stats, int32_t *err, void *stream)
{
    if (!h || !s_in || !order_obs || !Pi || !log1p_phi || !s_out) return fail(PMDI_E_ARG, "null argument");
    if (n1 < 1 || n1 > h->cfg.n) return fail(PMDI_E_ARG, "n1=%lld outside 1..n (rho*n < 1 is undefined in the reference)", (long long)n1);
    HIP_TRY(hipSetDevice(h->cfg.device));
    SweepArgs a;
    fill_sweep_call(h, a, iter, n1, lw_init, s_in, order_obs, Pi, log1p_phi, feature_flag, s_out, logweight, p_star, (long long *)stats, err, nullptr);
    hipStream_t st = (hipStream_t)stream;
    const int lrc = launch_sweep_groups(h, a, st);
    if (lrc) return lrc;
    h->swept = true; h->last_n1 = n1;
    return PMDI_OK;
}

int pmdi_psm_counts_device(int32_t device, const uint8_t *samples, int64_t S, int32_t K, int64_t n,
                           int64_t row_lo, int64_t row_hi, int32_t n_labels, int32_t *counts, void *stream)
{
    if (!samples || !counts) return fail(PMDI_E_ARG, "null argument");
    if (S < 1 || K < 1 || n < 1 || row_lo < 0 || row_hi > n || row_lo > row_hi)
        return fail(PMDI_E_ARG, "S=%lld K=%d n=%lld rows [%lld, %lld): out of range", (long long)S, K, (long long)n,
                    (long long)row_lo, (long long)row_hi);
    if (S > 2147483647LL) return fail(PMDI_E_ARG, "S=%lld samples overflow the int32 counts", (long long)S);
    if ((n + 63) / 64 > 2147483647LL || (row_hi - row_lo + 63) / 64 > 65535 || K > 65535)
        return fail(PMDI_E_ARG, "grid too large: split the rows into blocks of at most 4194240");
    HIP_TRY(hipSetDevice(device));
    if (n_labels < 0 || n_labels > 256) return fail(PMDI_E_ARG, "n_labels=%d outside 0..256", n_labels);
    const bool mfma = n_labels >= 1 && n_labels <= 64 && (row_hi - row_lo + 127) / 128 <= 65535;
    hipError_t e = mfma ? pmdi_launch_psm_counts_mfma(samples, S, K, n, row_lo, row_hi, n_labels, counts, (hipStream_t)stream)
                        : pmdi_launch_psm_counts(samples, S, K, n, row_lo, row_hi, counts, (hipStream_t)stream);
    if (e != hipSuccess) return fail(PMDI_E_DEVICE, "psm-count launch: %s", hipGetErrorString(e));
    return PMDI_OK;
}

int pmdi_psm_score_device(int32_t device, const int32_t *counts, int64_t S, int32_t K, int64_t n, int32_t which,
                          const int32_t *cand, int64_t B, int64_t ld, int64_t *agree_out, int64_t *pairs_out, int64_t *total_out,
                          void *stream)
{
    if (!counts || !cand || !agree_out || !pairs_out || !total_out) return fail(PMDI_E_ARG, "pmdi_psm_score_device: null argument");
    const int rc = pmdi_psm_shared_args("pmdi_psm_score_device", S, K, n, which, true, B, ld);
    if (rc) return rc;
    const unsigned __int128 P = (unsigned __int128)(n * (n - 1) / 2);
    const unsigned __int128 D = psm_divisor(S, K, which);
    if (D * P >= ((unsigned __int128)1 << 62))
        return fail(PMDI_E_ARG, "pmdi_psm_score_device: S=%lld with n=%lld: D n (n - 1) / 2 >= 2^62", (long long)S, (long long)n);
    if (n == 1) {
        for (int64_t b = 0; b < B; ++b) agree_out[b] = pairs_out[b] = 0;
        *total_out = 0;
        return PMDI_OK;
    }
    HIP_TRY(hipSetDevice(device));
    hipStream_t st = (hipStream_t)stream;
    Scratch out;
    const size_t bytes = ((size_t)2 * B + 1) * sizeof(unsigned long long);
    HIP_TRY(hipMalloc(&out.p, bytes));
    HIP_TRY(hipMemsetAsync(out.p, 0, bytes, st));
    const hipError_t e = pmdi_launch_psm_score(counts, K, n, which, D > ((unsigned __int128)1 << 22) ? 1 : 0, cand, B, ld,
                                               (unsigned long long *)out.p, st);
    if (e != hipSuccess) return fail(PMDI_E_DEVICE, "psm-score launch: %s", hipGetErrorString(e));
    HIP_TRY(hipMemcpyAsync(agree_out, out.p, (size_t)B * 8, hipMemcpyDeviceToHost, st));
    HIP_TRY(hipMemcpyAsync(pairs_out, (const char *)out.p + (size_t)B * 8, (size_t)B * 8, hipMemcpyDeviceToHost, st));
    HIP_TRY(hipMemcpyAsync(total_out, (const char *)out.p + (size_t)B * 16, 8, hipMemcpyDeviceToHost, st));
    HIP_TRY(hipStreamSynchronize(st));
    return PMDI_OK;
}

int pmdi_psm_rowscore_device(int32_t device, const int32_t *counts, int64_t S, int32_t K, int64_t n, int32_t which,
                             const int32_t *cand, int64_t B, int64_t ld, int64_t *own_out, int32_t *size_out, int64_t *rowtotal_out,
                             void *stream)
{
    if (!counts || !cand || !own_out || !size_out || !rowtotal_out) return fail(PMDI_E_ARG, "pmdi_psm_rowscore_device: null argument");
    const int rc = pmdi_psm_shared_args("pmdi_psm_rowscore_device", S, K, n, which, true, B, ld);
    if (rc) return rc;
    const unsigned __int128 D = psm_divisor(S, K, which);
    if (D * (unsigned __int128)(n - 1) >= ((unsigned __int128)1 << 62))
        return fail(PMDI_E_ARG, "pmdi_psm_rowscore_device: S=%lld with n=%lld: D (n - 1) >= 2^62", (long long)S, (long long)n);
    HIP_TRY(hipSetDevice(device));
    const hipError_t e = pmdi_launch_psm_rowscore(counts, K, n, which, D > ((unsigned __int128)1 << 22) ? 1 : 0, cand, B, ld,
                                                  (unsigned long long *)own_out, size_out, (unsigned long long *)rowtotal_out,
                                                  (hipStream_t)stream);
    if (e != hipSuccess) return fail(PMDI_E_DEVICE, "psm-rowscore launch: %s", hipGetErrorString(e));
    return PMDI_OK;
}

static_assert(PMDI_REFINE_GMAX == PMDI_REFINE_GMAX_I, "the header's slot count is the kernels'");

int pmdi_psm_refine_device(int32_t device, const int32_t *counts, int64_t S, int32_t K, int64_t n, int32_t which,
                           const int32_t *start, int64_t B, int64_t ld, int32_t max_sweeps, int32_t *labels_out, int64_t *moves_out,
                           int32_t *sweeps_out, void *stream)
{
    if (!counts || !start || !labels_out || !moves_out || !sweeps_out) return fail(PMDI_E_ARG, "pmdi_psm_refine_device: null argument");
    const int rc = pmdi_psm_shared_args("pmdi_psm_refine_device", S, K, n, which, true, B, ld);
    if (rc) return rc;
    const unsigned __int128 D = psm_divisor(S, K, which);
    if (D > 2147483647u)
        return fail(PMDI_E_ARG, "pmdi_psm_refine_device: S=%lld: D > 2^31 - 1", (long long)S);
    if (max_sweeps < 1) return fail(PMDI_E_ARG, "pmdi_psm_refine_device: max_sweeps=%d < 1", max_sweeps);
    HIP_TRY(hipSetDevice(device));
    hipStream_t st = (hipStream_t)stream;
    Scratch work, out;
    const size_t out_bytes = (size_t)B * 12 + 8;
    HIP_TRY(hipMalloc(&work.p, (size_t)n * (size_t)n * 4));
    HIP_TRY(hipMalloc(&out.p, out_bytes));
    HIP_TRY(hipMemsetAsync(out.p, 0, out_bytes, st));
    long long *d_moves = (long long *)out.p;
    int *d_sweeps = (int *)((char *)out.p + (size_t)B * 8), *d_flag = d_sweeps + B;
    const hipError_t e = pmdi_launch_psm_refine(counts, K, n, which, (long long)D, D * (unsigned __int128)n >= ((unsigned __int128)1 << 32) ? 1 : 0,
                                                (unsigned *)work.p, start, B, ld, max_sweeps, labels_out, d_moves, d_sweeps, d_flag, st);
    if (e != hipSuccess) return fail(PMDI_E_DEVICE, "psm-refine launch: %s", hipGetErrorString(e));
    int bad = 0;
    HIP_TRY(hipMemcpyAsync(moves_out, d_moves, (size_t)B * 8, hipMemcpyDeviceToHost, st));
    HIP_TRY(hipMemcpyAsync(sweeps_out, d_sweeps, (size_t)B * 4, hipMemcpyDeviceToHost, st));
    HIP_TRY(hipMemcpyAsync(&bad, d_flag, 4, hipMemcpyDeviceToHost, st));
    HIP_TRY(hipStreamSynchronize(st));
    if (bad) return fail(PMDI_E_DATA, "pmdi_psm_refine_device: a start label outside 0..%d", PMDI_REFINE_GMAX - 1);
    return PMDI_OK;
}

int pmdi_vi_log2_table(int32_t *out)
{
    if (!out) return fail(PMDI_E_ARG, "pmdi_vi_log2_table: null argument");
    pmdi_vi_log2_table_host(out);
    return PMDI_OK;
}

// ... 793 lines not shown
```

### particlemdi.jl_amd/csrc/pmdi_host.h

```cpp
#pragma once
#include "pmdi_internal.h"
#include "pmdi_plan.h"
#include "../../include/pmdi_hip.h"

#include <vector>

constexpr auto fail = pmdi_set_error;

#define HIP_TRY(expr)                                                                  \
    do {                                                                               \
        hipError_t e__ = (expr);                                                       \
        if (e__ != hipSuccess)                                                         \
            return fail(e__ == hipErrorOutOfMemory ? PMDI_E_MEMORY : PMDI_E_DEVICE,    \
                        "%s: %s", #expr, hipGetErrorString(e__));                      \
    } while (0)

struct DevBuf {
    void *p = nullptr;
    size_t bytes = 0;
    DevBuf() = default;
    DevBuf(const DevBuf &) = delete;
    DevBuf &operator=(const DevBuf &) = delete;
    ~DevBuf() { if (p) (void)hipFree(p); }
    int ensure(size_t b)
    {
        if (b <= bytes && p) return 0;
        if (p) { (void)hipFree(p); p = nullptr; bytes = 0; }
        if (b == 0) b = 16;
        hipError_t e = hipMalloc(&p, b);
        if (e != hipSuccess) { p = nullptr; return fail(PMDI_E_MEMORY, "hipMalloc(%zu): %s", b, hipGetErrorString(e)); }
        bytes = b;
        return 0;
    }
};

struct Scratch {
    void *p = nullptr;
    ~Scratch() { if (p) (void)hipFree(p); }
};

enum { ARGS_MAIN = 0, ARGS_LIGHT, ARGS_HEAVIEST, ARGS_SETTLED, ARGS_GIVEN_BACK, ARGS_COUNT };

struct pmdi_handle {
    pmdi_config cfg{};
    pmdi_tuning tun{};
    long long cap = 0;
    int Dmax = 0, sumD = 0, npairs = 1;
    SweepPlan plan;
    hipStream_t stream = nullptr, stream2 = nullptr, stream3 = nullptr;
    hipEvent_t ev_fork = nullptr, ev_join = nullptr, ev_join3 = nullptr;
    unsigned *start_sig = nullptr;
    DsetDev ds[PMDI_KMAX_I]{};
    std::vector<void *> owned;
    DevBuf d_s_in, d_order, d_Pi, d_logphi, d_flags, d_s_out, d_lw, d_pstar, d_stats, d_err, d_trace;
    DevBuf d_swept_by, d_resume;
    DevBuf d_args[ARGS_COUNT];
    DevBuf d_usc, d_partstar, d_kstate, d_phase, d_requeue, d_requeue_total, d_handed, d_group, d_cost, d_lorder, d_ticket, d_work, d_anclog, d_evpos, d_xcnt, d_xinc, d_xlab, d_xhdr;
    bool have_order = false;
    static constexpr int RING = 64;
    SweepArgs *ring = nullptr;
    hipEvent_t ring_ev[RING] = {};
    bool ring_used[RING] = {};
    int ring_head = 0;
    int sweep_no = 0;
    int err_keep = 0;
    int children = 0;
    DevBuf d_traj, d_lm, d_firstpos, d_fnull, d_fflags, d_fprob;
    bool swept = false;
    long long last_n1 = 0;
};

struct pmdi_gibbs {
    pmdi_handle *h = nullptr;
    int device = 0;
    GibbsArgs ga{};
    int *s_next = nullptr;
    unsigned char *flags = nullptr;
    double *fprob = nullptr;
    double *lw = nullptr;
    int *pstar = nullptr;
    long long *stats = nullptr;
    int *err = nullptr;
    long long n1 = 0;
    int feature_select = 0;
    int64_t iter = 0;
    std::vector<void *> owned;
};
```

### particlemdi.jl_amd/csrc/pmdi_internal.h

```cpp
#pragma once
#include <hip/hip_runtime.h>
#include <stdint.h>

#define PMDI_KMAX_I 8
#define PMDI_INF_I 0x7fffffff

#define PMDI_ITEM_CAP 256
#define PMDI_ITEM_CAP_BIGN 384
#define PMDI_HT_SIZE 512
#define PMDI_CLS_LDS 128
#define PMDI_DL_LDS 128

enum { K_GAUSSIAN = 0, K_CATEGORICAL = 1, K_NEGBINOM = 2 };
enum { SITE_DRAW = 0, SITE_RESAMPLE_U = 1, SITE_RESAMPLE_SLOT = 2, SITE_PSTAR = 3, SITE_FEATSEL = 4,
       SITE_SHUFFLE = 5, SITE_M_NORMAL = 6, SITE_M_ACCEPT = 7, SITE_GAMMA = 8, SITE_PHI_ALPHA = 9, SITE_PHI_GAMMA = 10,
       SITE_V = 11, SITE_ALIGN = 12, SITE_INIT_GAMMA = 13, SITE_INIT_PHI = 14, SITE_INIT_S = 15, SITE_INIT_FLAGS = 16 };
enum { ST_NOPS = 0, ST_NRESAMPLE = 1, ST_NCLONES = 2, ST_MAXID = 3, ST_SUMCLASSES = 4 };
enum { WK_EVAL = 0, WK_UPD = 1, WK_CLONE = 2, WK_MOVED = 3, WK_MOVE_EVENTS = 4, WK_COLS = 5, WK_SPLITS = 6 };

struct DsetDev {
    int kind, D, L, flag_off;
    const double *xf;
    const int *xi;
    const double *gtab;
    const double *lmtab;
    const double *lhtab;
    const double *lghtab;
    const int *maxcol;
    const double *lgtab;
    long long lgtab_len;
    char *arena;
    size_t stride;
    size_t o_particle[2];
    size_t o_col;
    size_t o_cgrp;
    size_t o_pid;
    size_t o_sid;
    size_t o_kv;
    size_t o_newid;
    size_t o_counts;
    size_t o_ncop;
    size_t o_firstc;
    size_t o_lp;
    size_t o_cn;
    size_t o_ml;
    size_t o_sb;
    size_t o_cnt;
    size_t o_nbs;
    size_t o_sstar;
    size_t o_clslead;
    size_t o_clsval;
    size_t o_cdf;
    size_t o_dl;
    size_t o_s2x;
};

struct S2Layout {
    int red, sc, stat, wk, ph, leaf_i1, leaf_n, leaf_tot, leaf_carry, leaf_prog, xfl;
    int tr, tr_stride, tr_tb, tr_cdf, tr_bytes;
    int rs_jtab, rs_raw, rs_anc, rs_hist;
    int ds0, ds_stride;
    int tab, cmask, wmask, cbi, counts, cn, ncop, firstp, tgt, slotmap, ta, tax, lp, slot_id, slot_cn, slot_g, clsval, clslead, leadcol,
        minp, nidv, knew, itemj, clist, klist, kval, krep, bmc, bmf, cbm, kbm, xid, dsc;
    int Dp, cols_l, idcap, total;
    int cls, kcap;
    int cdfl;
};

struct SweepArgs {
    int K, N, P, cap;
    int Dmax, sumD, npairs, q1, q2, trace_on;
    int terms_cap;
    int pid_lds;
    int pp_lds;
    int col_lds;
    int two_per_cu;
    int item_cap;
    unsigned iter;
    long long n, n1;
    unsigned long long seed;
    double lw_init;
    DsetDev ds[PMDI_KMAX_I];
    const int *s_in;
    const int *order;
    const double *Pi;
    const double *logphi;
    const unsigned char *flags;
    int *s_out;
    double *lw_out;
    int *pstar;
    long long *stats;
    int *err;
    double *trace;
    double *uscratch;
    int *partstar;
    int *kstate;
    long long *phase;
    long long *work;
    int *anclog;
    int *evpos;
    long long *cost;
    const int *chain_order;
    const unsigned char *group_flag;
    int ksplit;
    int n_slots;
    int *xcnt;
    double *xinc;
    int *xlab;
    unsigned long long *xhdr;
    unsigned *start_sig;
    int group_sel;
    int rank_lo, rank_hi;
    S2Layout s2;
    int *requeue;
    int *handed;
    int sweep_no;
    long long *requeue_total;
    int requeue_only;
    int slot_base;
    int err_keep;
    int *resume;
    int resume_mode;
    int *ticket;
    int *swept_by;
};

struct ClusterBatchArgs {
    DsetDev ds;
    int B;
    const int *rows;
    const unsigned char *flags;
    double *out;
};

struct FeatSelArgs {
    int K, N, sumD;
    int ltile;
    long long n;
    unsigned iter;
    unsigned long long seed;
    DsetDev ds[PMDI_KMAX_I];
    const int *traj;
    double *lm;
    int *firstpos;
    const double *fnull;
    unsigned char *flags_out;
    double *prob_out;
};

struct GibbsArgs {
    int K, N, npairs, n_chains;
    long long n;
    unsigned iter;
    unsigned long long seed;
    double *M;
    double *gamma;
    double *gamma0;
    double *Phi;
    double *vZ;
    int *s;
    int *order;
    double *Pi;
    double *logphi;
    int *ctab;
    double *wscr;
    const double *lgtab;
    int ctab_lds;
    int order_lds;
};

size_t pmdi_hypers_lds_bytes(const GibbsArgs &a);
size_t pmdi_align_lds_bytes(const GibbsArgs &a);
hipError_t pmdi_launch_gibbs_init(const GibbsArgs &a, hipStream_t stream);
hipError_t pmdi_launch_hypers(const GibbsArgs &a, int do_shuffle, hipStream_t stream);
hipError_t pmdi_launch_align(const GibbsArgs &a, hipStream_t stream);
hipError_t pmdi_launch_pack_samples(const int *s, unsigned char *out, long long count, hipStream_t stream);

hipError_t pmdi_launch_sweep(const SweepArgs &a, SweepArgs *d_args, int n_chains, int T, hipStream_t stream, SweepArgs *staging = nullptr);
hipError_t pmdi_sweep_blocks_per_cu(const SweepArgs &a, int T, int *blocks);
hipError_t pmdi_sweep2_blocks_per_cu(const SweepArgs &a, int *blocks);
hipError_t pmdi_launch_sweep2(const SweepArgs &a, SweepArgs *d_args, int n_chains, hipStream_t stream, SweepArgs *staging = nullptr);
hipError_t pmdi_launch_cluster_add(const ClusterBatchArgs &a, hipStream_t stream);
hipError_t pmdi_launch_cluster_logprob(const ClusterBatchArgs &a, hipStream_t stream);
hipError_t pmdi_launch_cluster_logmarginal(const ClusterBatchArgs &a, hipStream_t stream);
hipError_t pmdi_launch_chain_order(const long long *cost, int *order, const long long *stats, unsigned char *group_flag,
                                   long long light_ops_max, int n_chains, hipStream_t stream, const int *handed = nullptr, int sweep_no = 0);
hipError_t pmdi_launch_featsel(const FeatSelArgs &a, int n_chains, hipStream_t stream);
hipError_t pmdi_launch_psm_counts(const unsigned char *samples, long long S, int K, long long n, long long row_lo, long long row_hi,
                                  int *counts, hipStream_t stream);
hipError_t pmdi_launch_psm_counts_mfma(const unsigned char *samples, long long S, int K, long long n, long long row_lo, long long row_hi,
                                       int n_labels, int *counts, hipStream_t stream);
hipError_t pmdi_launch_label_counts(const int *s, int *counts, int n_rows, long long n, int N, hipStream_t stream);
hipError_t pmdi_launch_psm_acc_add(const unsigned char *samples, long long S, int K, long long n, int n_labels, int *counts, hipStream_t stream);
hipError_t pmdi_launch_psm_acc_mirror(int *counts, int K, long long n, hipStream_t stream);
hipError_t pmdi_launch_psm_acc_merge(int *a, const int *b, int K, long long n, hipStream_t stream);
hipError_t pmdi_launch_fusion_add(const unsigned char *samples, long long S, int K, long long n, int n_labels, const unsigned char *masks,
                                  const unsigned char *order, const int *n_class, int *counts, hipStream_t stream);
hipError_t pmdi_launch_fusion_obs(const unsigned char *samples, long long S, int K, long long n, const unsigned char *masks, int G, int *fused,
                                  hipStream_t stream);
hipError_t pmdi_launch_fusion_diag(const int *counts, int G, long long n, int *fused, hipStream_t stream);
hipError_t pmdi_launch_fusion_merge_obs(int *a, const int *b, int G, long long n, hipStream_t stream);
hipError_t pmdi_launch_psm_score(const int *counts, int K, long long n, int which, int wide, const int *cand, long long B, long long ld,
                                 unsigned long long *out, hipStream_t stream);
hipError_t pmdi_launch_psm_rowscore(const int *counts, int K, long long n, int which, int wide, const int *cand, long long B, long long ld,
                                    unsigned long long *own, int *size, unsigned long long *rowtotal, hipStream_t stream);
#define PMDI_REFINE_GMAX_I 4096
hipError_t pmdi_launch_psm_refine(const int *counts, int K, long long n, int which, long long D, int wide, unsigned *W, const int *start,
                                  long long B, long long ld, int max_sweeps, int *labels, long long *moves, int *sweeps, int *flag,
                                  hipStream_t stream);
hipError_t pmdi_launch_psm_refine_build(const int *counts, int K, long long n, int which, unsigned *W, hipStream_t stream);
hipError_t pmdi_launch_psm_refine_vi(const int *counts, int K, long long n, int which, long long D, unsigned *W, long long *own,
                                     const int *start, long long B, long long ld, int max_sweeps, int *labels, long long *moves,
                                     int *sweeps, long long *objective, int *flag, hipStream_t stream);
void pmdi_vi_log2_table_host(int *out);
hipError_t pmdi_launch_partition_rows(const void *labels, int is_bytes, long long R, long long n, long long ld, int G, unsigned char *bytes,
                                      long long *pairs, long long *hl, int *nclust, int *err, hipStream_t stream);
hipError_t pmdi_launch_partition_distance(const unsigned char *cand, long long B, int Gc, const unsigned char *draws, long long R, int Gd,
                                          long long n, long long *both, long long *jl, hipStream_t stream);
hipError_t pmdi_launch_partition_refine(const unsigned char *draw_bytes, long long R, int Gd, long long n, unsigned char *dT,
                                        unsigned short *tables, int lgp, const int *start, long long B, long long ld, int gcap, int loss,
                                        int max_sweeps, int *labels, long long *moves, int *sweeps, int *converged, long long *marginal,
                                        long long *joint, int *flag, hipStream_t stream);
hipError_t pmdi_launch_psm_blocksum(const int *counts, long long S, int K, long long n, int G, const unsigned short *g16, long long npad,
                                    const int *perm, const int *chunk_at, const int *chunk_info, int nchunks, const int *gsize,
                                    unsigned long long *out, hipStream_t stream);
enum { PMDI_DATA_RAW_I = 0, PMDI_DATA_SQDEV_I = 1, PMDI_DATA_ZBIN_I = 2, PMDI_DATA_LEVELS_I = 3 };
hipError_t pmdi_launch_data_groupsum(int is_float, const void *x, int D, long long ld, int G, int mode, const int *perm, const int *chunk_at,
                                     const int *chunk_info, int nchunks, const int *chunks_at, const double *shift, const double *scale,
                                     int L, double *part, void *out, int *flag, hipStream_t stream);

struct SummaryArgs {
    int C, K, N, npairs;
    int phi_stride;
    long long n, sumD;
    const int *s;
    const double *M;
    const double *Phi;
    const unsigned char *flags;
    int *nclust;
    int *err;
    long long *hist;
    long long *nclust_sum, *nclust_sumsq;
    double *M_mean, *M_m2;
    double *Phi_mean, *Phi_m2;
    long long *flag_count;
    long long *tr_nclust;
    double *tr_M, *tr_Phi;
};
hipError_t pmdi_launch_summary_add(const SummaryArgs &a, long long t, hipStream_t stream);

struct MixingArgs {
    int C, K, N, npairs;
    int phi_stride;
    int L, J;
    int np;
    long long n;
    const int *s;
    const double *M;
    const double *Phi;
    unsigned char *ring;
    long long *P_ring;
    double *y_ring;
    long long *A;
    double *nclust;
    int *err;
    long long *rand_num;
    double *ari_sum;
    double *sum_y, *prod, *head, *tail, *first;
};
hipError_t pmdi_launch_mixing_add(const MixingArgs &a, long long t, hipStream_t stream);

struct PredictArgs {
    int C, K, N, sumD;
    int ltile;
    long long n, m;
    DsetDev ds[PMDI_KMAX_I];
    const double *nxf[PMDI_KMAX_I];
    const int *nxi[PMDI_KMAX_I];
    const int *s;
    const double *Pi;
    const unsigned char *flags;
    double *lp;
    int lp_all;
    int Cb;
    int *cn;
    int *q;
    double *inc;
    int *qnew;
    int *err;
    long long *sim;
    long long *new_cluster;
    double *lpd_sum;
    int masked;
    int Dmax;
    const unsigned char *obs[PMDI_KMAX_I];
    double *mu;
    double *loc_sum;
    double *loc_joint_sum;
    long long *flag_on;
};
struct CoupledArgs {
    int npairs, nsub;
    const double *Phi;
    double *conn;
    double *Z0, *logZ0;
    double *g;
    double *Z;
    int *qj;
    int *qjnew;
    int *fq;
    double *incj;
    long long *sim_joint;
    long long *new_cluster_joint;
    long long *fused_new;
    double *lpd_joint_sum;
};
hipError_t pmdi_launch_predict_add(const PredictArgs &a, hipStream_t stream, const CoupledArgs *cp = nullptr);
hipError_t pmdi_launch_predict_merge(const PredictArgs &a, const long long *sim_b, const long long *nc_b, const double *lpd_b, hipStream_t stream);
hipError_t pmdi_launch_predict_merge_imputed(const PredictArgs &a, const double *loc_b, const double *locj_b, const long long *flag_b, hipStream_t stream);
void pmdi_launch_predict_chain_tables(const PredictArgs &a, const CoupledArgs &cp, hipStream_t stream);
void pmdi_launch_predict_couple(const PredictArgs &a, const CoupledArgs &cp, int c0, int chains, hipStream_t stream);
void pmdi_launch_predict_coupled_reduce(const PredictArgs &a, const CoupledArgs &cp, hipStream_t stream);
hipError_t pmdi_launch_predict_coupled_merge(const PredictArgs &a, const CoupledArgs &cp, const long long *fused_b, const double *lpdj_b, hipStream_t stream);

struct LooArgs {
    int C, K, N, sumD;
    int npairs;
    int ltile;
    long long n;
    DsetDev ds[PMDI_KMAX_I];
    size_t stat_at[PMDI_KMAX_I];
    size_t stat_label[PMDI_KMAX_I];
    size_t stat_chain;
    const int *s;
    const double *Pi;
    const unsigned char *flags;
    const double *Phi;
    char *stats;
    double *start;
// ... 19 lines not shown
```

### particlemdi.jl_amd/csrc/pmdi_sweep.hip

```cpp
#include "pmdi_sweep_body.h"

namespace {

template <int T, int WPS, bool K1, bool MANY>
__global__ void __launch_bounds__(T, WPS) pmdi_sweep_kernel(const SweepArgs *__restrict__ ap)
{
    pmdi_sweep_body<T, WPS, K1, MANY, false>(ap);
}

__global__ void chain_order_kernel(const long long *cost, int *order, const long long *stats, unsigned char *group_flag,
                                   long long light_ops_max, int n_chains, const int *handed, int sweep_no)
{
    const int c = blockIdx.x * blockDim.x + threadIdx.x;
    if (c >= n_chains) return;
    if (group_flag) group_flag[c] = (stats[(size_t)c * 8] > light_ops_max || (handed && sweep_no - handed[c] < 3)) ? 1 : 0;
    const long long mine = cost[c];
    int rank = 0;
    for (int j = 0; j < n_chains; ++j) {
        const long long o = cost[j];
        rank += (o > mine || (o == mine && j < c)) ? 1 : 0;
    }
    order[rank] = c;
}

}

hipError_t pmdi_launch_chain_order(const long long *cost, int *order, const long long *stats, unsigned char *group_flag,
                                   long long light_ops_max, int n_chains, hipStream_t stream, const int *handed, int sweep_no)
{
    hipLaunchKernelGGL(chain_order_kernel, dim3((n_chains + 255) / 256), dim3(256), 0, stream, cost, order, stats, group_flag,
                       light_ops_max, n_chains, handed, sweep_no);
    return hipGetLastError();
}

static const void *sweep_kernel_for(const SweepArgs &a, int T)
{
    const bool two = a.two_per_cu != 0;
    const bool k1 = a.K == 1 || a.ksplit;
    const bool many = a.N > 64;
#define PMDI_PICK(T_, W_) (k1 ? (many ? (const void *)pmdi_sweep_kernel<T_, W_, true, true> : (const void *)pmdi_sweep_kernel<T_, W_, true, false>) \
                              : (many ? (const void *)pmdi_sweep_kernel<T_, W_, false, true> : (const void *)pmdi_sweep_kernel<T_, W_, false, false>))
    if (T == 1024) return PMDI_PICK(1024, 4);
    if (T == 512 && two) return PMDI_PICK(512, 4);
    if (T == 512) return PMDI_PICK(512, 2);
    if (T == 128) return PMDI_PICK(128, 2);
    if (T == 256) return PMDI_PICK(256, PMDI_LIGHT_WPS);
#undef PMDI_PICK
    return nullptr;
}

hipError_t pmdi_sweep_blocks_per_cu(const SweepArgs &a, int T, int *blocks)
{
    const void *fn = sweep_kernel_for(a, T);
    if (!fn) return hipErrorInvalidValue;
    const size_t lds = pmdi_sweep_lds_bytes(a, T);
    hipError_t e = hipFuncSetAttribute(fn, hipFuncAttributeMaxDynamicSharedMemorySize, (int)lds);
    if (e != hipSuccess) return e;
    return hipOccupancyMaxActiveBlocksPerMultiprocessor(blocks, fn, T, lds);
}

hipError_t pmdi_launch_sweep(const SweepArgs &a_in, SweepArgs *d_args, int n_chains, int T, hipStream_t stream, SweepArgs *staging)
{
    SweepArgs a = a_in;
    if (!a.ksplit || a.n_slots <= 0) { a.n_slots = n_chains; a.slot_base = 0; }
    const size_t lds = pmdi_sweep_lds_bytes(a, T);
    const void *fn = sweep_kernel_for(a, T);
    if (!fn) return hipErrorInvalidValue;
    hipError_t e = hipFuncSetAttribute(fn, hipFuncAttributeMaxDynamicSharedMemorySize, (int)lds);
    if (e != hipSuccess) return e;
    const SweepArgs *src = &a;
    if (staging) { *staging = a; src = staging; }
    e = hipMemcpyAsync(d_args, src, sizeof(SweepArgs), hipMemcpyHostToDevice, stream);
    if (e != hipSuccess) return e;
    const SweepArgs *ap = d_args;
    void *args[] = {(void *)&ap};
    const unsigned grid = a.ksplit ? (unsigned)((n_chains + 7) / 8) * 8u * (unsigned)a.K : (unsigned)n_chains;
    e = hipLaunchKernel(fn, dim3(grid), dim3(T), args, lds, stream);
    if (e != hipSuccess) return e;
    return hipGetLastError();
}
```

### particlemdi.jl_amd/csrc/pmdi_sweep2.hip

```cpp
#ifndef PM2_NO_RESUME_GENERAL
#define PMDI_BSLOT_FROM_TICKET 1
#include "pmdi_sweep_body.h"
template <int K, int NW>
__device__ __noinline__ void pmdi_resume_general(const SweepArgs *ap)
{
    pmdi_sweep_body<64 * NW, 2, K == 1, false, true>(ap);
}
#define PM2_RESUME_GENERAL(K_, NW_, ap_) pmdi_resume_general<K_, NW_>(ap_)
#endif
#include "pmdi_sweep2_body.h"
#include "pmdi_sweep_carve.h"

namespace {

template <int K, int PPL, int NW, bool GO>
__global__ void __launch_bounds__(64 * NW, 2) pmdi_sweep2_kernel(const SweepArgs *__restrict__ ap)
{
    const SweepArgs &a = *ap;
    int bslot = (int)blockIdx.x;
    if (a.ticket) {
        int *tk = (int *)pm2_smem_;
        if (threadIdx.x == 0) {
            const int t = __hip_atomic_fetch_add(a.ticket, 1, __ATOMIC_RELAXED, __HIP_MEMORY_SCOPE_AGENT);
            __hip_atomic_store(a.ticket + 1 + blockIdx.x, t, __ATOMIC_RELAXED, __HIP_MEMORY_SCOPE_AGENT);
            *tk = t;
        }
        __syncthreads();
        bslot = *tk;
        __syncthreads();
        if (bslot < 0 || bslot >= a.n_slots) return;
    }
    const int chain = a.chain_order ? a.chain_order[bslot] : bslot;
    if (a.group_flag && ((int)a.group_flag[chain] != a.group_sel || bslot < a.rank_lo || bslot >= a.rank_hi)) return;
    pmdi_s2::Sweep2<K, PPL, NW, GO> s;
    s.run(ap, chain);
}

template <int K>
const void *kernel_for_k(int P, int *nw, bool gauss_only)
{
    const pmdi_s2::Shape s = pmdi_s2::shape_for(P);
    *nw = s.nw;
    if (s.nw == 4 && gauss_only) {
        if (s.ppl == 1) return (const void *)pmdi_sweep2_kernel<K, 1, 4, true>;
        if (s.ppl == 2) return (const void *)pmdi_sweep2_kernel<K, 2, 4, true>;
        if (s.ppl == 4) return (const void *)pmdi_sweep2_kernel<K, 4, 4, true>;
    }
    if (s.nw == 4 && s.ppl == 1) return (const void *)pmdi_sweep2_kernel<K, 1, 4, false>;
    if (s.nw == 4 && s.ppl == 2) return (const void *)pmdi_sweep2_kernel<K, 2, 4, false>;
    if (s.nw == 4 && s.ppl == 4) return (const void *)pmdi_sweep2_kernel<K, 4, 4, false>;
    if (s.nw == 8 && s.ppl == 4) return (const void *)pmdi_sweep2_kernel<K, 4, 8, false>;
    return nullptr;
}

const void *kernel_for(int K, int P, int *nw, bool gauss_only = false)
{
    switch (K) {
    case 1: return kernel_for_k<1>(P, nw, gauss_only);
    case 2: return kernel_for_k<2>(P, nw, gauss_only);
    case 3: return kernel_for_k<3>(P, nw, gauss_only);
    case 4: return kernel_for_k<4>(P, nw, gauss_only);
    }
    return nullptr;
}

bool all_gaussian(const SweepArgs &a)
{
    for (int k = 0; k < a.K; ++k) if (a.ds[k].kind != K_GAUSSIAN) return false;
    return true;
}

}

static size_t launch_lds(const SweepArgs &a, int nw)
{
    size_t lds = (size_t)a.s2.total;
    if (a.resume) { const size_t g = pmdi_sweep_lds_bytes(a, 64 * nw); if (g > lds) lds = g; }
    return lds;
}

hipError_t pmdi_sweep2_blocks_per_cu(const SweepArgs &a, int *blocks)
{
    int nw = 0;
    const void *fn = kernel_for(a.K, a.P, &nw, all_gaussian(a));
    if (!fn) return hipErrorInvalidValue;
    const size_t lds = launch_lds(a, nw);
    hipError_t e = hipFuncSetAttribute(fn, hipFuncAttributeMaxDynamicSharedMemorySize, (int)lds);
    if (e != hipSuccess) return e;
    return hipOccupancyMaxActiveBlocksPerMultiprocessor(blocks, fn, 64 * nw, lds);
}

hipError_t pmdi_launch_sweep2(const SweepArgs &a_in, SweepArgs *d_args, int n_chains, hipStream_t stream, SweepArgs *staging)
{
    SweepArgs a = a_in;
    a.n_slots = n_chains;
    int nw = 0;
    const void *fn = kernel_for(a.K, a.P, &nw, all_gaussian(a));
    if (!fn) return hipErrorInvalidValue;
    const size_t lds = launch_lds(a, nw);
    hipError_t e = hipFuncSetAttribute(fn, hipFuncAttributeMaxDynamicSharedMemorySize, (int)lds);
    if (e != hipSuccess) return e;
    const SweepArgs *src = &a;
    if (staging) { *staging = a; src = staging; }
    e = hipMemcpyAsync(d_args, src, sizeof(SweepArgs), hipMemcpyHostToDevice, stream);
    if (e != hipSuccess) return e;
    if (a.ticket) {
        e = hipMemsetAsync(a.ticket, 0, sizeof(int), stream);
        if (e != hipSuccess) return e;
    }
    const SweepArgs *ap = d_args;
    void *args[] = {(void *)&ap};
    e = hipLaunchKernel(fn, dim3((unsigned)n_chains), dim3(64u * (unsigned)nw), args, lds, stream);
    if (e != hipSuccess) return e;
    return hipGetLastError();
}
```

### particlemdi.jl_amd/csrc/pmdi_sweep2_body.h

```cpp
#pragma once
#include "pmdi_arith.h"
#include "pmdi_internal.h"
#include "pmdi_sweep2_layout.h"

#ifndef PM2_LANE_API_PROVIDED
#include "pmdi_wave.h"
#define PM2_DEV __device__ __forceinline__
#define PM2_COLD __device__ __noinline__
extern __shared__ __attribute__((aligned(16))) unsigned char pm2_smem_[];
#define PM2_SMEM (pm2_smem_)
#define PM2_TID() ((int)threadIdx.x)
#define PM2_BID() ((int)blockIdx.x)
#define PM2_BALLOT(p) __ballot(p)
#define PM2_SHFL64(v, src) pm2_shfl64((v), (src))
#define PM2_WAVE_BARRIER() do { __builtin_amdgcn_fence(__ATOMIC_ACQ_REL, "wavefront"); __builtin_amdgcn_wave_barrier(); } while (0)
#define PM2_BARRIER() __syncthreads()
#define PM2_LDS_BARRIER() asm volatile("s_waitcnt lgkmcnt(0)\n\ts_barrier" ::: "memory")
#define PM2_UNI(x) __builtin_amdgcn_readfirstlane(x)
#define PM2_CLOCK() ((long long)clock64())
#define PM2_WALLCLOCK() ((long long)wall_clock64())
#if defined(__HIP_DEVICE_COMPILE__)
#define PM2_G(T, p) ((__attribute__((address_space(1))) T *)(p))
#define PM2_CONST __attribute__((address_space(4)))
#ifdef PM2_NO_LAUNDER
// ... 1858 lines not shown
                auto s_in = PM2_G(const int, a.s_in) + (size_t)chain * K * n;
                auto s_out = PM2_G(int, a.s_out) + (size_t)chain * K * n;
                for (long long e = tid; e < (long long)K * n; e += T) s_out[e] = s_in[e];
            }
            return;
        }
        PH2(9);
        finish(t_start);
        PH2(10);
        if (a.phase && tid == 0) {
            lds<long long>(L.ph)[14] = PM2_CLOCK() - t_start;
            lds<long long>(L.ph)[12] = t_wall; lds<long long>(L.ph)[13] = PM2_WALLCLOCK();
            for (int e = 0; e < 16; ++e) PM2_G(long long, a.phase)[(size_t)chain * 16 + e] = lds<long long>(L.ph)[e];
        }
#undef PH2
    }

    PM2_DEV void export_dataset(int k)
    {
        const auto &a = *ap;
        const DV v = view(k);
        const int ncol = v.dsc()[DS_NCOL], maxid = v.dsc()[DS_MAXID];
        auto tg = PM2_G(int, v.ar.tabg());
        for (int e = tid; e < ncol * N && e < v.cols_l * N; e += T) tg[e] = (int)lds<u16>(v.base + L.tab)[e];
        auto cg = PM2_G(int, v.ar.colg());
        auto pg = PM2_G(int, v.ar.pidg());
        int ck[PPL];
        col_get(k, ck);
#pragma unroll
        for (int u = 0; u < PPL; ++u) { cg[tid * PPL + u] = ck[u]; pg[tid * PPL + u] = lds<int>(v.base + L.clsval)[csl_get(k, u)]; }
        auto cng = PM2_G(int, v.ar.cn());
        auto ctg = PM2_G(int, v.ar.counts());
        for (int id = tid; id < v.idcap && id <= a.cap; id += T) { cng[id] = (id <= maxid) ? lds<int>(v.base + L.cn)[id] : cng[id]; ctg[id] = (id <= maxid) ? lds<int>(v.base + L.counts)[id] : 0; }
        for (int id = maxid + 1 + tid; id <= a.cap; id += T) ctg[id] = 0;
        if (tid == 0) {
            PM2_G(int, a.kstate)[((size_t)chain * PMDI_KMAX_I + k) * 2] = maxid;
            PM2_G(int, a.kstate)[((size_t)chain * PMDI_KMAX_I + k) * 2 + 1] = 0;
        }
    }

    PM2_DEV void hand_over(long long pos, int fcode, long long t_start)
    {
        const auto &a = *ap;
        PM2_BARRIER();
        int done_mask = 0;
#pragma nounroll
        for (int k = 0; k < K; ++k) {
            const DV v = view(k);
            int *dsc = v.dsc();
            const bool halted = dsc[DS_HALT] != 0;
            if (!halted) done_mask |= 1 << k;
            export_dataset(k);
            auto g1 = PM2_G(int, v.ar.ncop());
            auto g2 = PM2_G(int, v.ar.firstp());
            for (int e = tid; e < v.idcap && e <= a.cap; e += T) { g1[e] = 0; g2[e] = 0x7fffffff; }
            if (halted) {
                const int ndx = dsc[DS_NDX];
                for (int e = tid; e < ndx; e += T) { const int id = PM2_G(const int, v.ar.dl())[e]; g1[id] = 0; g2[id] = 0x7fffffff; }
            }
            if (tid == 0) {
                PM2_G(int, a.resume)[(size_t)chain * 16 + 2 + k] = dsc[DS_NCOL];
                if (halted) wk(k)[WK_EVAL] += dsc[DS_NNEED];
            }
        }
#pragma unroll
        for (int u = 0; u < PPL; ++u) PM2_G(double, a.uscratch)[(size_t)chain * K * P + tid * PPL + u] = lw[u];
        PM2_BARRIER();
        if (tid == 0) {
            auto st = PM2_G(long long, a.stats) + (size_t)chain * 8;
            const long long *s = stat();
            st[ST_NOPS] = s[0]; st[ST_NRESAMPLE] = s[1]; st[ST_NCLONES] = s[2]; st[ST_MAXID] = s[3]; st[ST_SUMCLASSES] = s[4];
            st[5] = s[5]; st[6] = 0; st[7] = 0;
            PM2_G(int, a.resume)[(size_t)chain * 16] = (int)pos;
            PM2_G(int, a.resume)[(size_t)chain * 16 + 1] = done_mask;
            PM2_G(int, a.requeue)[chain] = 0;
            if (!a.err_keep) PM2_G(int, a.err)[chain] = 0;
            if (a.handed) PM2_G(int, a.handed)[chain] = a.sweep_no;
            if (a.requeue_total) {
                pm2_atomic_add((u64 *)a.requeue_total + 3, (u64)1); pm2_atomic_add((u64 *)a.requeue_total + 2, (u64)1);
                if (fcode == 4 && sc()[SC_TMP1] > 2 * CLS) pm2_atomic_add((u64 *)a.requeue_total + 1, (u64)1);
            }
            PM2_G(long long, a.cost)[chain] = PM2_CLOCK() - t_start;
        }
        if (a.work && tid < K * 8) PM2_G(long long, a.work)[((size_t)chain * PMDI_KMAX_I) * 8 + tid] = lds<long long>(L.wk)[tid];
    }

    PM2_DEV void finish(long long t_start)
    {
        const auto &a = *ap;
        double *red = lds<double>(L.red);
        double *wt = lds<double>(L.tr);
        auto order = PM2_G(const int, a.order) + (size_t)chain * n;
        PM2_BARRIER();
        {
            double mx = lw[0];
#pragma unroll
            for (int u = 1; u < PPL; ++u) mx = (lw[u] > mx) ? lw[u] : mx;
            mx = wave_max_d(mx);
            if (lane == 0) red[wave] = mx;
        }
        PM2_BARRIER();
        double mx = red[0];
        for (int w_ = 1; w_ < T / 64; ++w_) mx = (red[w_] > mx) ? red[w_] : mx;
#pragma unroll
        for (int u = 0; u < PPL; ++u) wt[tid * PPL + u] = exp(lw[u] - mx);
        PM2_BARRIER();
        if (tid == 0) {
            double sum = 0.0;
            for (int p = 0; p < P; ++p) sum += wt[p];
            const double t = pmdi_arith::uniform01<false>(seed, iter, 0, 0, 0, SITE_PSTAR) * sum;
            int ip = 0;
            double cw = wt[0];
            while (cw < t && ip < P - 1) { ++ip; cw += wt[ip]; }
            sc()[SC_PSTAR] = ip;
        }
        PM2_BARRIER();
        const int pstar = sc()[SC_PSTAR];
        for (long long pp = tid; pp < n; pp += T) {
            const int i = order[pp];
            for (int k = 0; k < K; ++k) {
                int val;
                if (pp < n1 - 1) val = PM2_G(const int, a.s_in)[((size_t)chain * K + k) * n + i];
                else val = PM2_G(const u8, view(k).ar.sstar())[(size_t)pp * P + pstar];
                PM2_G(int, a.s_out)[((size_t)chain * K + k) * n + i] = val;
            }
        }
        if (a.lw_out)
#pragma unroll
            for (int u = 0; u < PPL; ++u) PM2_G(double, a.lw_out)[(size_t)chain * P + tid * PPL + u] = lw[u];
#pragma nounroll
        for (int k = 0; k < K; ++k) export_dataset(k);
        if (tid == 0) {
            auto st = PM2_G(long long, a.stats) + (size_t)chain * 8;
            const long long *s = stat();
            PM2_G(int, a.pstar)[chain] = pstar;
            st[ST_NOPS] = s[0]; st[ST_NRESAMPLE] = s[1]; st[ST_NCLONES] = s[2]; st[ST_MAXID] = s[3]; st[ST_SUMCLASSES] = s[4];
            st[5] = s[5]; st[6] = 0; st[7] = 0;
            if (!a.err_keep) PM2_G(int, a.err)[chain] = 0;
            if (a.requeue) PM2_G(int, a.requeue)[chain] = 0;
            if (a.swept_by) PM2_G(int, a.swept_by)[chain] = 1;
            PM2_G(long long, a.cost)[chain] = PM2_CLOCK() - t_start;
        }
        if (a.work && tid < K * 8) PM2_G(long long, a.work)[((size_t)chain * PMDI_KMAX_I) * 8 + tid] = lds<long long>(L.wk)[tid];
    }
#undef CLS
#undef L
};

template <int K, int PPL, int NW, bool GO> PM2_COLD void hand_over_cold(Sweep2<K, PPL, NW, GO> s, long long pos, int fcode, long long t_start)
{
    s.hand_over(pos, fcode, t_start);
}

}
```

### particlemdi.jl_amd/csrc/pmdi_sweep_body.h

```cpp
#pragma once
#define PMDI_SWEEP_TU 1
#include "pmdi_device.h"
#include "pmdi_sweep_carve.h"

using namespace pmdi_dev;

namespace {

typedef __attribute__((address_space(3))) int *lint;
typedef __attribute__((address_space(3))) unsigned *lu32;
typedef __attribute__((address_space(3))) double *ldbl;
typedef __attribute__((address_space(3))) unsigned long long *lu64;
typedef __attribute__((address_space(3))) long long *li64;
typedef __attribute__((address_space(3))) unsigned char *lu8;

template <class Tp>
__device__ __forceinline__ Tp *gen(__attribute__((address_space(3))) Tp *p) { return (Tp *)p; }
using pmdi_dev::gen;

struct HT {
    lint key, a, b;
    unsigned mask;
};

// ... 1067 lines not shown
}

template <int T>
__device__ PMDI_COLD_FINAL void sweep_final(const SweepArgs *__restrict__ ap)
{
    PMDI_PREAMBLE;
    {
        double mx = -INFINITY;
        for (int p = tid; p < P; p += T) { const double v = sh.lw[p]; mx = (v > mx) ? v : mx; }
        mx = block_max<T>(mx, gen(sh.red));
        double *wb = gen(sh.term);
        for (int p = tid; p < P; p += T) wb[p] = exp(sh.lw[p] - mx);
        __syncthreads();
        if (tid == 0) {
            double sum = 0.0;
            for (int p = 0; p < P; ++p) sum += wb[p];
            const double t = uniform01(seed, iter, 0, 0, 0, SITE_PSTAR) * sum;
            int ip = 0;
            double cw = wb[0];
            while (cw < t && ip < P - 1) { ++ip; cw += wb[ip]; }
            sh.misc[M_PSTAR] = ip;
        }
        __syncthreads();
        const int pstar = sh.misc[M_PSTAR];
        const int nev = a.q2 ? (int)sh.stat[1] : 0;
        const gint evp = a.q2 ? glob(a.evpos) + (size_t)chain * 2 * (size_t)(n - n1 + 1) : (gint)nullptr;
        const gint lin = evp + (n - n1 + 1);
        const gint anc = a.q2 ? glob(a.anclog) + (size_t)chain * (size_t)(n - n1 + 1) * P : (gint)nullptr;
        if (nev > 0) {
            __syncthreads();
            if (tid == 0) {
                int cur = pstar;
                for (int e = nev - 1; e >= 0; --e) { cur = anc[(size_t)e * P + cur]; lin[e] = cur; }
            }
            __syncthreads();
        }
        for (long long pp = tid; pp < n; pp += T) {
            const int i = order[pp];
            int slot = pstar;
            if (nev > 0 && pp >= n1 - 1 && (int)pp <= evp[nev - 1]) {
                int lo = 0, hi = nev - 1;
                while (lo < hi) { const int mid = (lo + hi) >> 1; if (evp[mid] >= (int)pp) hi = mid; else lo = mid + 1; }
                slot = lin[lo];
            }
            for (int k = 0; k < K; ++k) {
                int v;
                if (pp < n1 - 1) v = s_in[(size_t)k * n + i];
                else {
                    const unsigned char *ss = (const unsigned char *)(dsb[k].arena + (size_t)chain * dsb[k].stride + dsb[k].o_sstar);
                    v = ss[(size_t)pp * P + slot];
                }
                a.s_out[((size_t)chain * Kf + kd0 + k) * n + i] = v;
            }
        }
        if (a.lw_out && kd0 == 0) for (int p = tid; p < P; p += T) a.lw_out[(size_t)chain * P + p] = sh.lw[p];
        if (a.pid_lds)
            for (int k = 0; k < K; ++k) {
                int *gp = (int *)(dsb[k].arena + (size_t)chain * dsb[k].stride + dsb[k].o_pid);
                for (int p = tid; p < P; p += T) gp[p] = sh.pid[(size_t)k * P + p];
            }
        if (a.col_lds)
            for (int k = 0; k < K; ++k) {
                int *gc = (int *)(dsb[k].arena + (size_t)chain * dsb[k].stride + dsb[k].o_col);
                for (int p = tid; p < P; p += T) gc[p] = (int)sh.col[(size_t)k * P + p];
            }
        if (tid < K) {
            a.kstate[((size_t)chain * PMDI_KMAX_I + kd0 + tid) * 2] = sh.kmaxid[tid];
            a.kstate[((size_t)chain * PMDI_KMAX_I + kd0 + tid) * 2 + 1] = sh.kcur[tid];
        }
        if (tid == 0) {
            long long *st = a.stats + (size_t)chain * 8;
            if (!a.ksplit) {
                a.pstar[chain] = pstar;
                st[ST_NOPS] = sh.stat[0]; st[ST_NRESAMPLE] = sh.stat[1]; st[ST_NCLONES] = sh.stat[2];
                st[ST_MAXID] = sh.stat[3]; st[ST_SUMCLASSES] = sh.stat[4];
                st[5] = sh.stat[5]; st[6] = sh.stat[6]; st[7] = sh.stat[7];
                if (!a.err_keep) a.err[chain] = 0;
                if (a.requeue) a.requeue[chain] = 0;
            } else {
                if (kd0 == 0) { a.pstar[chain] = pstar; st[ST_NRESAMPLE] = sh.stat[1]; if (a.requeue_only && a.requeue) a.requeue[chain] = 0; }
                atomicAdd((unsigned long long *)&st[ST_NOPS], (unsigned long long)sh.stat[0]);
                atomicAdd((unsigned long long *)&st[ST_NCLONES], (unsigned long long)sh.stat[2]);
                atomicMax((unsigned long long *)&st[ST_MAXID], (unsigned long long)sh.stat[3]);
                atomicAdd((unsigned long long *)&st[ST_SUMCLASSES], (unsigned long long)sh.stat[4]);
                atomicAdd((unsigned long long *)&st[5], (unsigned long long)sh.stat[5]);
                atomicAdd((unsigned long long *)&st[6], (unsigned long long)sh.stat[6]);
                atomicAdd((unsigned long long *)&st[7], (unsigned long long)sh.stat[7]);
            }
        }
        if (a.work && tid < K * 8) a.work[((size_t)chain * PMDI_KMAX_I + kd0) * 8 + tid] = sh.wk[tid];
    }
}

template <int T, int WPS>
__device__ __noinline__ void sweep_replay(const SweepArgs *__restrict__ ap, long long pos, int i, int done)
{
    PMDI_PREAMBLE;
    long long ph_last = 0;
    int ph_cur = 0;
    for (int k = 0; k < K; ++k) {
        if ((done >> k) & 1) continue;
        const DsetDev &d = dsb[k];
        const KS s = make_ks(d, chain);
        const int D = d.D;
        const int maxid = sh.kmaxid[k], ncls = sh.kncls[k];
        const ClsList cl{sh.cl_lead + k * PMDI_CLS_LDS, sh.cl_val + k * PMDI_CLS_LDS, s.clslead, s.clsval, PMDI_CLS_LDS};
        for (int q = tid; q < D; q += T) {
            if (d.kind == K_GAUSSIAN) sh.xs[q] = glob(d.xf)[(size_t)i * D + q]; else ((int *)sh.xs)[q] = glob(d.xi)[(size_t)i * D + q];
        }
        for (int p = tid; p < P; p += T) sh.news[k * P + p] = s.sstar[(size_t)pos * P + p];
        for (int r = tid; r < ncls; r += T) sh.slot_of[cl.val(r)] = r;
        if (tid == 0) sh.misc[M_OVF] = 0;
        __syncthreads();
        sweep_slow<T, WPS>(ap, k, i, pos, false, true, maxid, ncls, ph_last, ph_cur);
        if (sh.misc[M_FAIL]) return;
        if (tid == 0) {
            const int nclone_r = sh.misc[M_NCLONE];
            sh.stat[7] += 1;
            sh.stat[0] += maxid;
            sh.stat[4] += ncls;
            sh.stat[2] += nclone_r;
            if (maxid + nclone_r > sh.stat[3]) sh.stat[3] = maxid + nclone_r;
            sh.kmaxid[k] = maxid + nclone_r; sh.kncls[k] = sh.misc[M_NCLS];
            sh.wk[k * 8 + WK_UPD] += sh.misc[M_ND]; sh.wk[k * 8 + WK_CLONE] += nclone_r;
        }
        __syncthreads();
    }
    double mx, ess;
    bool resample;
    PMDI_SWEEP_ESS(mx, ess, resample);
    if (resample) {
        if (tid == 0) sh.stat[1] += 1;
        sweep_resample<T>(ap, pos, mx);
    }
    if (tid == 0) sh.misc[M_XAB] = resample ? 1 : 0;
    if (a.trace_on && tid == 0) {
        double *tr = a.trace + ((size_t)chain * (n - n1 + 1) + (pos - (n1 - 1))) * (2 + 2 * Kf);
        tr[0] = ess; tr[1] = resample ? 1.0 : 0.0;
        for (int k = 0; k < K; ++k) { tr[2 + k] = (double)sh.kmaxid[k]; tr[2 + Kf + k] = (double)sh.kncls[k]; }
    }
    __syncthreads();
}

template <int T, int WPS, bool K1, bool MANY, bool RESUME>
__device__ __forceinline__ void pmdi_sweep_body(const SweepArgs *__restrict__ ap)
{
    PMDI_PREAMBLE_K(K1);
    if (!RESUME) {
    if (a.start_sig && tid == 0 && (!a.ksplit || bslot < a.n_slots))
        __hip_atomic_fetch_add(a.start_sig, 1u, __ATOMIC_RELAXED, __HIP_MEMORY_SCOPE_SYSTEM);
    if (bslot >= a.n_slots) return;
    if (a.group_flag && ((int)a.group_flag[chain] != a.group_sel || bslot < a.rank_lo || bslot >= a.rank_hi)) return;
    if (a.requeue_only && !a.requeue[chain]) return;
    }
#define XSPLIT (a.ksplit != 0)
#define XCNT (glob(a.xcnt) + (size_t)chain * 32)
#define XOFF(par_, kd_) ((((size_t)chain * 2 + (size_t)(par_)) * (size_t)a.K + (size_t)(kd_)) * (size_t)a.P)

    const long long t_start = clock64();
#ifdef PMDI_RESAMPLE_TIMERS
    if (tid < 24) sh.stat[tid] = 0;
#else
    if (tid < 8) sh.stat[tid] = 0;
#endif
    long long ph_last = 0;
    int ph_cur = 0;
#define PH(i_)                                                                  \
    do {                                                                        \
        if (a.phase && tid == 0) {                                              \
            const long long t_ = clock64();                                     \
            sh.ph[ph_cur] += t_ - ph_last; ph_last = t_; ph_cur = (i_);         \
        }                                                                       \
    } while (0)
    if (tid < 16) { sh.ph[tid] = 0; sh.misc[tid] = 0; }
    if (tid < PMDI_KMAX_I * 8) sh.wk[tid] = 0;
    if (tid < PMDI_KMAX_I) sh.khint[tid] = 0;
    long long ph_t0 = 0, ph_r0 = 0;
    if (a.phase && tid == 0) { ph_last = clock64(); ph_t0 = ph_last; ph_r0 = wall_clock64(); }

    for (int p = tid; p < P; p += T) sh.lw[p] = a.lw_init;
    for (int c = tid; c <= P; c += T) { sh.lead_of[c] = PMDI_INF_I; sh.slot_of[c] = 0; }
    for (int e = tid; e < H; e += T) { sh.h1.key[e] = 0; sh.h1.a[e] = 0; sh.h2.key[e] = 0; sh.h2.a[e] = 0; sh.h2.b[e] = PMDI_INF_I; }
    for (int e = tid; e < a.item_cap; e += T) sh.ktab_minp[e] = PMDI_INF_I;
    for (int e = tid; e < 2 * ((P >> 6) + 1); e += T) { sh.bm_fresh[e] = 0; sh.bm_clone[e] = 0; sh.bm_keep[e] = 0; sh.bm_reuse[e] = 0; }

    long long pos0 = n1 - 1;
    int failed = 0;
    bool lw_uniform = true;
    if (RESUME) {
        __syncthreads();
        sweep_resume_load<T>(ap);
        const long long posr = a.resume[(size_t)chain * 16];
        sweep_replay<T, WPS>(ap, posr, order[posr], a.resume[(size_t)chain * 16 + 1]);
        if (sh.misc[M_FAIL]) failed = 1;
        lw_uniform = sh.misc[M_XAB] != 0;
        __syncthreads();
        if (tid == 0) sh.misc[M_XAB] = 0;
        pos0 = posr + 1;
    } else
    sweep_prefix<T>(ap);
    PH(1);
    int i_next = pos0 < n ? order[pos0] : 0;
    double nx = 0.0;
    int nxi = 0;
    int ns0_next = s_in[i_next];
    {
        const DsetDev &d0 = dsb[0];
        if (tid < d0.D) {
            if (d0.kind == K_GAUSSIAN) nx = glob(d0.xf)[(size_t)i_next * d0.D + tid]; else nxi = glob(d0.xi)[(size_t)i_next * d0.D + tid];
        }
    }
    for (long long pos = pos0; pos < n && !failed; ++pos) {
        int xhdr = 0;
        const int i = i_next;
        if (pos + 1 < n) i_next = order[pos + 1];
        for (int k = 0; k < K && !failed; ++k) {
            const int tid_outer_ = tid, lane_outer_ = lane;
            {
            int tid = opaque_vgpr(tid_outer_), lane = opaque_vgpr(lane_outer_);
#define FRESH_LANE_IDS() asm volatile("" : "+v"(tid), "+v"(lane))
            const DsetDev &d = dsb[k];
            const KS s = make_ks(d, chain);
            const int D = d.D;
            const int maxid = sh.kmaxid[k];
            const int ncls = sh.kncls[k];
            const int cur = sh.kcur[k];
            const gint part = s.part[cur];
            const auto pidk = dual(a.pid_lds != 0, sh.pid + (size_t)k * P, s.pid);
            const auto colk = dual(a.col_lds != 0, sh.col + (size_t)k * P, s.col);
            const auto sidp = dual(a.pp_lds != 0, sh.sid, s.sid);
            const auto kvp = dual(a.pp_lds != 0, sh.kv, s.kv);
            const unsigned char *flk = gen(sh.fl + (size_t)k * Dp);
            const double *pik = gen(sh.pis + k * N);
            const ClsList cl{sh.cl_lead + k * PMDI_CLS_LDS, sh.cl_val + k * PMDI_CLS_LDS, s.clslead, s.clsval, PMDI_CLS_LDS};
            const int items = ncls * N;
            const bool small = items <= a.item_cap;
            if (ncls != 1) lw_uniform = false;

            PH(1);
            const int ns0_cur = ns0_next;
            if (tid < D) {
                if (d.kind == K_GAUSSIAN) sh.xs[tid] = nx; else ((int *)sh.xs)[tid] = nxi;
            }
            for (int r = tid; r < ncls; r += T) sh.slot_of[cl.val(r)] = r;
            if (tid == 0) sh.misc[M_OVF] = 0;

            if (small) {
                for (int w = tid; w < items; w += T) {
                    const int r = w / N, nn = w - r * N;
                    const int id = part[(size_t)colk[cl.lead(r)] * N + nn];
                    sh.item_id[w] = id;
                    bool won;
                    const int slot = ht_insert(sh.h1, id, won, H);
                    if (won) {
                        const int ps = atomicAdd(gen(&sh.misc[M_NEED]), 1);
                        sh.need[ps] = id; sh.need_slot[ps] = slot; sh.h1.a[slot] = ps;
                    }
                }
            }
            for (int q = T + tid; q < D; q += T) {
                if (d.kind == K_GAUSSIAN) sh.xs[q] = glob(d.xf)[(size_t)i * D + q]; else ((int *)sh.xs)[q] = glob(d.xi)[(size_t)i * D + q];
            }
            if (small) lds_barrier(); else __syncthreads();
            const int nneed = small ? sh.misc[M_NEED] : maxid;
            const int nflag = sh.knflag[k];

            if (!small) {
                PH(2); FRESH_LANE_IDS();
                sweep_logprob_all<T>(ap, k, maxid);
            }
            else {
                const int RS = 2 * D + 1, D1 = D + 1;
                int CH = a.terms_cap / RS;
                if (CH < 1) CH = 1;
                for (int j0 = 0; j0 < nneed; j0 += CH) {
                    const int nid = min(CH, nneed - j0);
                    PH(2); FRESH_LANE_IDS();
                    for (int it = tid; it < nid * D1; it += T) {
                        const int il = it / D1, q = it - il * D1;
                        const int id = small ? sh.need[j0 + il] : 1 + j0 + il;
                        const int cn = s.cn[id];
                        if (q == D) {
                            if (d.kind == K_GAUSSIAN) sh.term[il * RS + 2 * D] = (double)nflag * glob(d.gtab)[cn];
                            continue;
                        }
                        if (!flk[q]) continue;
                        double ta = 0.0, tb = 0.0;
                        if (d.kind == K_GAUSSIAN) {
                            gauss_terms(sh.xs[q], (double)cn, gauss_ml(cn, ld2(s.sb, (size_t)id * D + q)), ta, tb);
                        } else if (d.kind == K_CATEGORICAL) {
                            const int x = ((const int *)sh.xs)[q];
                            ta = glob(d.lhtab)[glob(d.maxcol)[q] + 2 * cn];
                            const int c = s.cnt[((size_t)id * D + q) * d.L + (x - 1)];
                            tb = (cn == 0) ? glob(d.lhtab)[1] : glob(d.lhtab)[2 * c + 1];
                        } else {
                            const int x = ((const int *)sh.xs)[q];
                            ta = negbin_term(glob(d.lgtab), cn, x, s.nbs[(size_t)id * D + q]);
                        }
                        sh.term[il * RS + 2 * q] = ta;
                        sh.term[il * RS + 2 * q + 1] = tb;
                    }
                    if (small) lds_barrier(); else __syncthreads();
                    PH(3); FRESH_LANE_IDS();
                    for (int il = tid; il < nid; il += T) {
                        const double *t = gen(sh.term + il * RS);
                        double out;
                        if (d.kind == K_GAUSSIAN) {
                            out = t[2 * D];
                            if (nflag == D) {
                                for (int q0 = 0; q0 < D; q0 += 8) {
                                    double ra[8], rb[8];
#pragma unroll
                                    for (int u = 0; u < 8; ++u) {
                                        const int q = min(q0 + u, D - 1);
                                        ra[u] = t[2 * q]; rb[u] = t[2 * q + 1];
                                    }
#pragma unroll
                                    for (int u = 0; u < 8; ++u)
                                        if (q0 + u < D) { out += ra[u]; out -= rb[u]; }
                                }
                            } else {
                                for (int q = 0; q < D; ++q)
                                    if (flk[q]) { out += t[2 * q]; out -= t[2 * q + 1]; }
                            }
                        } else if (d.kind == K_CATEGORICAL) {
                            double acc = 0.0;
                            for (int q = 0; q < D; ++q) if (flk[q]) acc += t[2 * q];
                            out = -acc;
                            for (int q = 0; q < D; ++q) if (flk[q]) out += t[2 * q + 1];
                        } else {
                            out = 0.0;
// ... 416 lines not shown
                lds_barrier();
                for (int j = tid; j < nf; j += T) { const int sl = sh.fl_slot[j]; sh.h2.key[sl] = 0; sh.h2.a[sl] = 0; sh.h2.b[sl] = PMDI_INF_I; }
                if (tid == 0) { sh.misc[M_NK] = 0; sh.misc[M_NF] = 0; }
            } else {
                sweep_slow<T, WPS>(ap, k, i, pos, small, converted, maxid, ncls, ph_last, ph_cur);
                if (sh.misc[M_FAIL]) { failed = 1; break; }
                nclone = sh.misc[M_NCLONE];
                new_ncls = sh.misc[M_NCLS];
                nd = sh.misc[M_ND];
            }
            }
            if (tid == 0) {
                sh.stat[fast ? 5 : (converted ? 6 : 7)] += 1;
                sh.stat[0] += maxid;
                sh.stat[4] += ncls;
                sh.stat[2] += nclone;
                if (maxid + nclone > sh.stat[3]) sh.stat[3] = maxid + nclone;
                sh.kmaxid[k] = maxid + nclone; sh.kncls[k] = new_ncls;
                sh.wk[k * 8 + WK_EVAL] += nneed; sh.wk[k * 8 + WK_UPD] += ustep ? 1 : nd; sh.wk[k * 8 + WK_CLONE] += nclone;
            }
            __syncthreads();
#undef FRESH_LANE_IDS
            }
        }
        if (failed) break;

        PH(9);
        if (XSPLIT) {
            if (tid == 0) {
                unsigned long long *hd = (unsigned long long *)a.xhdr + ((((size_t)chain * 2 + (size_t)((pos - (n1 - 1)) & 1)) * (size_t)a.K + (size_t)kd0) * 2);
                const unsigned long long w0 = (unsigned long long)(unsigned)(xhdr | ((int)sh.news[0] << 16));
                __hip_atomic_store(hd, w0, __ATOMIC_RELAXED, __HIP_MEMORY_SCOPE_AGENT);
                __hip_atomic_store(hd + 1, (unsigned long long)__double_as_longlong((double)sh.cdf[N]), __ATOMIC_RELAXED, __HIP_MEMORY_SCOPE_AGENT);
            }
            asm volatile("s_waitcnt vmcnt(0)" ::: "memory");
            __syncthreads();
            if (tid == 0) {
                __hip_atomic_fetch_add(gen(XCNT), 1, __ATOMIC_RELAXED, __HIP_MEMORY_SCOPE_AGENT);
                const int target = Kf * (int)(pos - (n1 - 1) + 1);
                const long long w0 = wall_clock64();
                int ab = 0;
                for (;;) {
                    const int v = __hip_atomic_load(gen(XCNT), __ATOMIC_RELAXED, __HIP_MEMORY_SCOPE_AGENT);
                    if (v >= (1 << 28)) { ab = 2; break; }
                    if (v >= target) break;
                    __builtin_amdgcn_s_sleep(2);
                    if (wall_clock64() - w0 > 2000000000LL) { ab = 3; break; }
                }
                sh.misc[M_XAB] = ab;
            }
            __syncthreads();
            if (sh.misc[M_XAB]) { failed = sh.misc[M_XAB]; break; }
            const unsigned long long *xi = (const unsigned long long *)a.xinc + XOFF((pos - (n1 - 1)) & 1, 0);
            const int *xl = a.xlab + XOFF((pos - (n1 - 1)) & 1, 0);
            const unsigned long long *xh = (const unsigned long long *)a.xhdr + (((size_t)chain * 2 + (size_t)((pos - (n1 - 1)) & 1)) * (size_t)a.K) * 2;
            PH(12);
            unsigned hw[PMDI_KMAX_I];
            unsigned long long hinc[PMDI_KMAX_I];
#pragma unroll
            for (int kk = 0; kk < PMDI_KMAX_I; ++kk) {
                hw[kk] = 0; hinc[kk] = 0;
                if (kk < Kf) {
                    hw[kk] = (unsigned)__hip_atomic_load(xh + 2 * kk, __ATOMIC_RELAXED, __HIP_MEMORY_SCOPE_AGENT);
                    hinc[kk] = __hip_atomic_load(xh + 2 * kk + 1, __ATOMIC_RELAXED, __HIP_MEMORY_SCOPE_AGENT);
                }
            }
            for (int p = tid; p < P; p += T) {
                unsigned long long labs = 0;
                double w = sh.lw[p];
                unsigned long long rinc[PMDI_KMAX_I];
                int rlab[PMDI_KMAX_I];
#pragma unroll
                for (int kk = 0; kk < PMDI_KMAX_I; ++kk) {
                    rinc[kk] = hinc[kk];
                    rlab[kk] = (p == 0) ? (int)((hw[kk] >> 16) & 0xffu) : (int)((hw[kk] >> 8) & 0xffu);
                    if (kk < Kf && !(hw[kk] & 1u)) {
                        rinc[kk] = __hip_atomic_load(xi + (size_t)kk * P + p, __ATOMIC_RELAXED, __HIP_MEMORY_SCOPE_AGENT);
                        rlab[kk] = __hip_atomic_load(xl + (size_t)kk * P + p, __ATOMIC_RELAXED, __HIP_MEMORY_SCOPE_AGENT);
                    }
                }
#pragma unroll
                for (int kk = 0; kk < PMDI_KMAX_I; ++kk) {
                    if (kk < Kf) {
                        labs |= (unsigned long long)(rlab[kk] & 0xff) << (8 * kk);
                        w = w + __longlong_as_double((long long)rinc[kk]);
                    }
                }
                int pr = 0;
                for (int k1 = 0; k1 < Kf - 1; ++k1)
                    for (int k2 = k1 + 1; k2 < Kf; ++k2) {
                        w += (((labs >> (8 * k1)) & 0xff) == ((labs >> (8 * k2)) & 0xff)) ? logphi[pr] : 0.0;
                        ++pr;
                    }
                sh.lw[p] = w;
            }
            lw_uniform = false;
            __syncthreads();
        } else if (K > 1) {
            for (int p = tid; p < P; p += T) {
                int pr = 0;
                double w = sh.lw[p];
                for (int k1 = 0; k1 < K - 1; ++k1)
                    for (int k2 = k1 + 1; k2 < K; ++k2) {
                        w += (sh.news[k1 * P + p] == sh.news[k2 * P + p]) ? logphi[pr] : 0.0;
                        ++pr;
                    }
                sh.lw[p] = w;
            }
            lw_uniform = false;
            __syncthreads();
        }

        double ess = (double)P;
        bool resample = false;
        double mx = 0.0;
        if (!lw_uniform) PMDI_SWEEP_ESS(mx, ess, resample);

        if (resample) {
            PH(10);
            if (tid == 0) sh.stat[1] += 1;
            sweep_resample<T>(ap, pos, mx);
            lw_uniform = true;
        }

        if (a.trace_on && tid == 0) {
            double *tr = a.trace + ((size_t)chain * (n - n1 + 1) + (pos - (n1 - 1))) * (2 + 2 * Kf);
            if (kd0 == 0) { tr[0] = ess; tr[1] = resample ? 1.0 : 0.0; }
            for (int k = 0; k < K; ++k) { tr[2 + kd0 + k] = (double)sh.kmaxid[k]; tr[2 + Kf + kd0 + k] = (double)sh.kncls[k]; }
        }
    }

    if (failed) {
        if (tid == 0) {
            if (failed == 1) a.err[chain] = -4;
            else if (failed == 3) a.err[chain] = -6;
            else if (failed == 2 && a.err[chain] == 0) a.err[chain] = -4;
            a.cost[chain] = clock64() - t_start;
            if (XSPLIT) __hip_atomic_fetch_add(gen(XCNT), 1 << 28, __ATOMIC_RELAXED, __HIP_MEMORY_SCOPE_AGENT);
        }
        for (int k = 0; k < K; ++k)
            for (long long pp = tid; pp < n; pp += T) a.s_out[((size_t)chain * Kf + kd0 + k) * n + pp] = s_in[(size_t)k * n + pp];
        return;
    }

    PH(11);
    sweep_final<T>(ap);
    PH(12);
    if (tid == 0 && kd0 == 0) {
        a.cost[chain] = (RESUME ? a.cost[chain] : 0) + (clock64() - t_start);
        if (a.swept_by) a.swept_by[chain] = (RESUME || a.requeue_only) ? 2 : 0;
    }
    if (a.phase && tid == 0) {
        sh.ph[14] = clock64() - ph_t0; sh.ph[15] = wall_clock64() - ph_r0;
    }
    __syncthreads();
    if (a.phase && tid < 16 && kd0 == 0) a.phase[(size_t)chain * 16 + tid] = sh.ph[tid];
#ifdef PMDI_RESAMPLE_TIMERS
    __syncthreads();
    if (a.phase && tid < 10) a.phase[(size_t)chain * 16 + tid] = sh.stat[8 + tid];
#endif
}

}
```

Baseline: 901.2.

## Let settled-chain sweep workgroups loop over ticketed chains with hold modes

The settled-chain sweep2 kernel becomes a persistent loop. A workgroup can grab further chain tickets after finishing one, either always (hold=2, which also allows a smaller grid) or once the heavy chains have all started (hold=1, tracked through a new heavy_left counter). The heavy counter is filled by the chain-order kernel and decremented by heavy sweep workgroups as they start. The aim is to rebalance work between the heavy and settled streams and cut the tail of idle or one-shot workgroups, at the cost of extra atomics and polling. Per-chain wall-clock stamps and a settled_launch query are added for diagnostics.

```diff
diff --git a/include/pmdi_hip.h b/include/pmdi_hip.h
--- a/include/pmdi_hip.h
+++ b/include/pmdi_hip.h
@@ -48,7 +48,9 @@
     int32_t phase_timers;
     int32_t profiled;
     int32_t ticket;
-    int32_t reserved[5];
+    int32_t hold;
+    int32_t sweep_grid;
+    int32_t reserved[3];
 } pmdi_tuning;
 
 typedef struct {
@@ -342,6 +344,10 @@
 
 int pmdi_sweep_layout(const pmdi_handle *h, int32_t *out32);
 
+int pmdi_settled_launch(pmdi_handle *h, int32_t *out4);
+
+int pmdi_chain_stamps(pmdi_handle *h, int64_t *out);
+
 int pmdi_sum_D(const pmdi_handle *h);
 int pmdi_block_threads(const pmdi_handle *h);
 int pmdi_is_split(const pmdi_handle *h);
diff --git a/particlemdi.jl_amd/_lib.py b/particlemdi.jl_amd/_lib.py
--- a/particlemdi.jl_amd/_lib.py
+++ b/particlemdi.jl_amd/_lib.py
@@ -54,6 +54,7 @@
     "pmdi_partition_rows_device", "pmdi_partition_distance_device", "pmdi_partition_refine_device",
     "pmdi_loo_create", "pmdi_loo_destroy", "pmdi_loo_reset", "pmdi_loo_samples", "pmdi_loo_set_budget", "pmdi_loo_add_gibbs",
     "pmdi_loo_add_arrays", "pmdi_loo_merge", "pmdi_loo_get", "pmdi_loo_last", "pmdi_gibbs_run6",
+    "pmdi_settled_launch", "pmdi_chain_stamps",
 ]
 
 
@@ -127,7 +128,7 @@
 class _Tuning(C.Structure):
     _fields_ = [(name, C.c_int32) for name in (
         "settled", "continue_inplace", "sticky", "light_ids", "s2_cols", "s2_idcap", "s2_cls", "ksplit", "requeue_ksplit", "split",
-        "heavy_threads", "two_per_cu", "very_heavy", "start_gate", "terms_cap", "lds_target", "phase_timers", "profiled", "ticket")] + [("reserved", C.c_int32 * 5)]
+        "heavy_threads", "two_per_cu", "very_heavy", "start_gate", "terms_cap", "lds_target", "phase_timers", "profiled", "ticket", "hold", "sweep_grid")] + [("reserved", C.c_int32 * 3)]
 
 
 class _Config(C.Structure):
@@ -373,6 +374,10 @@
     L.pmdi_settled_kernel.argtypes = [vp, vp]
     L.pmdi_chain_swept_by.restype = C.c_int
     L.pmdi_chain_swept_by.argtypes = [vp, vp]
+    L.pmdi_settled_launch.restype = C.c_int
+    L.pmdi_settled_launch.argtypes = [vp, vp]
+    L.pmdi_chain_stamps.restype = C.c_int
+    L.pmdi_chain_stamps.argtypes = [vp, vp]
     L.pmdi_tuning_default.restype = None
     L.pmdi_tuning_default.argtypes = [C.POINTER(_Tuning)]
     L.pmdi_tuning_from_env.restype = None
@@ -604,6 +609,16 @@
         _check(lib().pmdi_chain_swept_by(self.h, _ptr(out)))
         return out
 
+    def settled_launch(self):
+        v = np.zeros(4, dtype=np.int32)
+        _check(lib().pmdi_settled_launch(self.h, _ptr(v)))
+        return {"hold": int(v[0]), "grid": int(v[1]), "slots": int(v[2]), "draws": int(v[3])} if self.settled else None
+
+    def chain_stamps(self):
+        out = np.zeros((self.C, 2), dtype=np.int64)
+        _check(lib().pmdi_chain_stamps(self.h, _ptr(out)))
+        return out
+
     def chain_costs(self):
         out = np.zeros(self.C, dtype=np.int64)
         _check(lib().pmdi_chain_costs(self.h, _ptr(out)))
diff --git a/particlemdi.jl_amd/csrc/pmdi_api.cpp b/particlemdi.jl_amd/csrc/pmdi_api.cpp
--- a/particlemdi.jl_amd/csrc/pmdi_api.cpp
+++ b/particlemdi.jl_amd/csrc/pmdi_api.cpp
@@ -127,6 +127,7 @@
     a.item_cap = h->cfg.N > 32 ? PMDI_ITEM_CAP_BIGN : PMDI_ITEM_CAP;
     a.two_per_cu = pl.two_per_cu;
     a.phase = pl.phase_on ? (long long *)h->d_phase.p : nullptr;
+    a.stamp = pl.phase_on ? (long long *)h->d_stamp.p : nullptr;
     a.cost = (long long *)h->d_cost.p;
     a.work = (long long *)h->d_work.p;
     a.anclog = (int *)h->d_anclog.p; a.evpos = (int *)h->d_evpos.p;
@@ -214,6 +215,7 @@
         HIP_TRY(hipEventRecord(h->ev_fork, st));
         a.group_flag = (const unsigned char *)h->d_group.p;
         a.group_sel = 1;
+        a.heavy_left = pl.s2_ok ? (int *)h->d_heavy_left.p : nullptr;
         const int vh = pl.very_heavy < C ? pl.very_heavy : C;
         if (vh > 0) {
             SweepArgs av = a;
@@ -237,6 +239,7 @@
         if (vh > 0) HIP_TRY(hipStreamWaitEvent(st, h->ev_join3, 0));
         SweepArgs al = a;
         al.group_sel = 0; al.rank_lo = 0; al.rank_hi = C;
+        al.heavy_left = nullptr;
         pmdi_put_tables(pl.light, al);
         HIP_TRY(hipStreamWaitEvent(h->stream2, h->ev_fork, 0));
         if (pl.s2_ok) {
@@ -245,7 +248,9 @@
             SweepArgs *slot = next_slot(h, h->stream2, &idx);
             SweepArgs as = al;
             as.ticket = (h->tun.ticket != 0) ? (int *)h->d_ticket.p : nullptr;
-            e = pmdi_launch_sweep2(as, args(ARGS_SETTLED), C, h->stream2, slot);
+            as.hold = h->hold;
+            as.heavy_left = (int *)h->d_heavy_left.p;
+            e = pmdi_launch_sweep2(as, args(ARGS_SETTLED), C, h->sweep_grid, h->stream2, slot);
             if (e == hipSuccess && idx >= 0) { e = hipEventRecord(h->ring_ev[idx], h->stream2); h->ring_used[idx] = true; }
             if (e != hipSuccess) return fail(PMDI_E_DEVICE, "sweep launch (settled chains): %s", hipGetErrorString(e));
             if (!pl.s2_continue) {
@@ -269,9 +274,11 @@
     }
     if (C > 1 || pl.split) {
         const long long steps = (a.n - a.n1 + 1) * (long long)a.K;
+        if (pl.s2_ok) HIP_TRY(hipMemsetAsync(h->d_heavy_left.p, 0, 4, st));
         e = pmdi_launch_chain_order((const long long *)h->d_cost.p, (int *)h->d_lorder.p, a.stats,
                                     pl.split ? (unsigned char *)h->d_group.p : nullptr, pl.light_ids * steps, C, st,
-                                    pl.s2_ok ? (const int *)h->d_handed.p : nullptr, h->sweep_no + 3 - pl.sticky);
+                                    pl.s2_ok ? (const int *)h->d_handed.p : nullptr, h->sweep_no + 3 - pl.sticky,
+                                    pl.s2_ok ? (int *)h->d_heavy_left.p : nullptr);
         if (e != hipSuccess) return fail(PMDI_E_DEVICE, "chain-order launch: %s", hipGetErrorString(e));
         h->have_order = true;
     }
@@ -403,8 +410,16 @@
     if (h->cfg.q2_mode == 1 &&
         ((rc = h->d_anclog.ensure((size_t)C * (size_t)n * P * 4)) || (rc = h->d_evpos.ensure((size_t)C * 2 * (size_t)n * 4))))
         return rc;
-    if (hipMemset(h->d_group.p, (h->plan.s2_ok && h->tun.settled == 2) ? 0 : 1, (size_t)C) != hipSuccess)
+    const bool all_heavy = !(h->plan.s2_ok && h->tun.settled == 2);
+    if (hipMemset(h->d_group.p, all_heavy ? 1 : 0, (size_t)C) != hipSuccess)
         return fail(PMDI_E_DEVICE, "hipMemset failed");
+    const int heavy_first = all_heavy ? C : 0;
+    if ((rc = h->d_heavy_left.ensure(4))) return rc;
+    if (hipMemcpy(h->d_heavy_left.p, &heavy_first, 4, hipMemcpyHostToDevice) != hipSuccess) return fail(PMDI_E_DEVICE, "memcpy failed");
+    if (h->plan.phase_on) {
+        if ((rc = h->d_stamp.ensure((size_t)C * 2 * 8))) return rc;
+        if (hipMemset(h->d_stamp.p, 0, (size_t)C * 2 * 8) != hipSuccess) return fail(PMDI_E_DEVICE, "hipMemset failed");
+    }
     return PMDI_OK;
 }
 
@@ -474,6 +489,7 @@
     env("PMDI_KSPLIT", t->ksplit); env("PMDI_REQUEUE_KSPLIT", t->requeue_ksplit); env("PMDI_SPLIT", t->split);
     env("PMDI_HEAVY_T", t->heavy_threads); env("PMDI_TWO_PER_CU", t->two_per_cu); env("PMDI_VERY_HEAVY", t->very_heavy);
     env("PMDI_START_GATE", t->start_gate); env("PMDI_TICKET", t->ticket); env("PMDI_TERMS_CAP", t->terms_cap); env("PMDI_LDS_TARGET", t->lds_target);
+    env("PMDI_HOLD", t->hold); env("PMDI_SWEEP_GRID", t->sweep_grid);
     if (getenv("PMDI_PHASE_TIMERS")) t->phase_timers = 1;
     auto has = [](const char *name, const char *what) { const char *v = getenv(name); return v && strstr(v, what) != nullptr; };
     t->profiled = (has("LD_PRELOAD", "rocprof") || has("ROCP_TOOL_LIBRARIES", "rocprof") || has("HSA_TOOLS_LIB", "rocprof")) ? 1 : 0;
@@ -540,6 +556,15 @@
     h->npairs = K > 1 ? K * (K - 1) / 2 : 1;
     int rc = 0;
     auto bail = [&](int code) { pmdi_destroy(h); return code; };
+    {
+        const int hold = h->tun.hold < 0 ? 1 : h->tun.hold, grid = h->tun.sweep_grid;
+        if (hold > 2) return bail(fail(PMDI_E_ARG, "tuning.hold=%d outside 0..2", hold));
+        if (grid == 0 || grid < -1) return bail(fail(PMDI_E_ARG, "tuning.sweep_grid=%d: at least one workgroup", grid));
+        h->hold = h->tun.ticket != 0 ? hold : 0;
+        if (h->hold == 0 && grid > 0 && grid < cfg->n_chains)
+            return bail(fail(PMDI_E_ARG, "tuning.sweep_grid=%d < n_chains=%d with one-shot workgroups (hold = 0, or no ticket): chains would stay unswept", grid, cfg->n_chains));
+        h->sweep_grid = (h->hold == 2 && grid > 0 && grid < cfg->n_chains) ? grid : cfg->n_chains;
+    }
     if (hipStreamCreateWithFlags(&h->stream, hipStreamNonBlocking) != hipSuccess) return bail(fail(PMDI_E_DEVICE, "hipStreamCreate failed"));
 
     for (int k = 0; k < K; ++k)
@@ -610,6 +635,34 @@
 {
     if (!h || !out32) return fail(PMDI_E_ARG, "null argument");
     pmdi_plan_layout32(h->plan, h->start_sig != nullptr, h->d_xcnt.p != nullptr, h->cfg.K, h->cfg.P, out32);
+    return PMDI_OK;
+}
+int pmdi_settled_launch(pmdi_handle *h, int32_t *out4)
+{
+    if (!h || !out4) return fail(PMDI_E_ARG, "null argument");
+    out4[0] = out4[1] = out4[2] = out4[3] = 0;
+    if (!h->plan.s2_ok) return PMDI_OK;
+    HIP_TRY(hipSetDevice(h->cfg.device));
+    SweepArgs a;
+    fill_sweep_common(h, a);
+    pmdi_put_tables(h->plan.resume, a);
+    int blocks = 0, cus = 0;
+    HIP_TRY(pmdi_sweep2_blocks_per_cu(a, &blocks));
+    HIP_TRY(hipDeviceGetAttribute(&cus, hipDeviceAttributeMultiprocessorCount, h->cfg.device));
+    out4[0] = h->hold; out4[1] = h->sweep_grid; out4[2] = blocks * cus;
+    if (h->tun.ticket != 0 && h->sweep_no > 0) {
+        HIP_TRY(hipDeviceSynchronize());
+        HIP_TRY(hipMemcpy(&out4[3], h->d_ticket.p, 4, hipMemcpyDeviceToHost));
+    }
+    return PMDI_OK;
+}
+int pmdi_chain_stamps(pmdi_handle *h, int64_t *out)
+{
+    if (!h || !out) return fail(PMDI_E_ARG, "null argument");
+    if (!h->plan.phase_on) return fail(PMDI_E_STATE, "set PMDI_PHASE_TIMERS=1 before pmdi_create");
+    HIP_TRY(hipSetDevice(h->cfg.device));
+    HIP_TRY(hipDeviceSynchronize());
+    HIP_TRY(hipMemcpy(out, h->d_stamp.p, (size_t)h->cfg.n_chains * 2 * 8, hipMemcpyDeviceToHost));
     return PMDI_OK;
 }
 int pmdi_sum_D(const pmdi_handle *h) { return h ? h->sumD : 0; }
diff --git a/particlemdi.jl_amd/csrc/pmdi_host.h b/particlemdi.jl_amd/csrc/pmdi_host.h
--- a/particlemdi.jl_amd/csrc/pmdi_host.h
+++ b/particlemdi.jl_amd/csrc/pmdi_host.h
@@ -55,8 +55,9 @@
     DevBuf d_s_in, d_order, d_Pi, d_logphi, d_flags, d_s_out, d_lw, d_pstar, d_stats, d_err, d_trace;
     DevBuf d_swept_by, d_resume;
     DevBuf d_args[ARGS_COUNT];
-    DevBuf d_usc, d_partstar, d_kstate, d_phase, d_requeue, d_requeue_total, d_handed, d_group, d_cost, d_lorder, d_ticket, d_work, d_anclog, d_evpos, d_xcnt, d_xinc, d_xlab, d_xhdr;
+    DevBuf d_usc, d_partstar, d_kstate, d_phase, d_requeue, d_requeue_total, d_handed, d_group, d_cost, d_lorder, d_ticket, d_heavy_left, d_stamp, d_work, d_anclog, d_evpos, d_xcnt, d_xinc, d_xlab, d_xhdr;
     bool have_order = false;
+    int hold = 0, sweep_grid = 0;
     static constexpr int RING = 64;
     SweepArgs *ring = nullptr;
     hipEvent_t ring_ev[RING] = {};
diff --git a/particlemdi.jl_amd/csrc/pmdi_internal.h b/particlemdi.jl_amd/csrc/pmdi_internal.h
--- a/particlemdi.jl_amd/csrc/pmdi_internal.h
+++ b/particlemdi.jl_amd/csrc/pmdi_internal.h
@@ -123,6 +123,9 @@
     int resume_mode;
     int *ticket;
     int *swept_by;
+    int *heavy_left;
+    int hold;
+    long long *stamp;
 };
 
 struct ClusterBatchArgs {
@@ -179,12 +182,13 @@
 hipError_t pmdi_launch_sweep(const SweepArgs &a, SweepArgs *d_args, int n_chains, int T, hipStream_t stream, SweepArgs *staging = nullptr);
 hipError_t pmdi_sweep_blocks_per_cu(const SweepArgs &a, int T, int *blocks);
 hipError_t pmdi_sweep2_blocks_per_cu(const SweepArgs &a, int *blocks);
-hipError_t pmdi_launch_sweep2(const SweepArgs &a, SweepArgs *d_args, int n_chains, hipStream_t stream, SweepArgs *staging = nullptr);
+hipError_t pmdi_launch_sweep2(const SweepArgs &a, SweepArgs *d_args, int n_chains, int grid, hipStream_t stream, SweepArgs *staging = nullptr);
 hipError_t pmdi_launch_cluster_add(const ClusterBatchArgs &a, hipStream_t stream);
 hipError_t pmdi_launch_cluster_logprob(const ClusterBatchArgs &a, hipStream_t stream);
 hipError_t pmdi_launch_cluster_logmarginal(const ClusterBatchArgs &a, hipStream_t stream);
 hipError_t pmdi_launch_chain_order(const long long *cost, int *order, const long long *stats, unsigned char *group_flag,
-                                   long long light_ops_max, int n_chains, hipStream_t stream, const int *handed = nullptr, int sweep_no = 0);
+                                   long long light_ops_max, int n_chains, hipStream_t stream, const int *handed = nullptr, int sweep_no = 0,
+                                   int *heavy_left = nullptr);
 hipError_t pmdi_launch_featsel(const FeatSelArgs &a, int n_chains, hipStream_t stream);
 hipError_t pmdi_launch_psm_counts(const unsigned char *samples, long long S, int K, long long n, long long row_lo, long long row_hi,
                                   int *counts, hipStream_t stream);
diff --git a/particlemdi.jl_amd/csrc/pmdi_sweep.hip b/particlemdi.jl_amd/csrc/pmdi_sweep.hip
--- a/particlemdi.jl_amd/csrc/pmdi_sweep.hip
+++ b/particlemdi.jl_amd/csrc/pmdi_sweep.hip
@@ -9,11 +9,15 @@
 }
 
 __global__ void chain_order_kernel(const long long *cost, int *order, const long long *stats, unsigned char *group_flag,
-                                   long long light_ops_max, int n_chains, const int *handed, int sweep_no)
+                                   long long light_ops_max, int n_chains, const int *handed, int sweep_no, int *heavy_left)
 {
     const int c = blockIdx.x * blockDim.x + threadIdx.x;
     if (c >= n_chains) return;
-    if (group_flag) group_flag[c] = (stats[(size_t)c * 8] > light_ops_max || (handed && sweep_no - handed[c] < 3)) ? 1 : 0;
+    if (group_flag) {
+        const bool heavy = stats[(size_t)c * 8] > light_ops_max || (handed && sweep_no - handed[c] < 3);
+        group_flag[c] = heavy ? 1 : 0;
+        if (heavy && heavy_left) atomicAdd(heavy_left, 1);
+    }
     const long long mine = cost[c];
     int rank = 0;
     for (int j = 0; j < n_chains; ++j) {
@@ -26,10 +30,10 @@
 }
 
 hipError_t pmdi_launch_chain_order(const long long *cost, int *order, const long long *stats, unsigned char *group_flag,
-                                   long long light_ops_max, int n_chains, hipStream_t stream, const int *handed, int sweep_no)
+                                   long long light_ops_max, int n_chains, hipStream_t stream, const int *handed, int sweep_no, int *heavy_left)
 {
     hipLaunchKernelGGL(chain_order_kernel, dim3((n_chains + 255) / 256), dim3(256), 0, stream, cost, order, stats, group_flag,
-                       light_ops_max, n_chains, handed, sweep_no);
+                       light_ops_max, n_chains, handed, sweep_no, heavy_left);
     return hipGetLastError();
 }
 
diff --git a/particlemdi.jl_amd/csrc/pmdi_sweep2.hip b/particlemdi.jl_amd/csrc/pmdi_sweep2.hip
--- a/particlemdi.jl_amd/csrc/pmdi_sweep2.hip
+++ b/particlemdi.jl_amd/csrc/pmdi_sweep2.hip
@@ -16,24 +16,7 @@
 template <int K, int PPL, int NW, bool GO>
 __global__ void __launch_bounds__(64 * NW, 2) pmdi_sweep2_kernel(const SweepArgs *__restrict__ ap)
 {
-    const SweepArgs &a = *ap;
-    int bslot = (int)blockIdx.x;
-    if (a.ticket) {
-        int *tk = (int *)pm2_smem_;
-        if (threadIdx.x == 0) {
-            const int t = __hip_atomic_fetch_add(a.ticket, 1, __ATOMIC_RELAXED, __HIP_MEMORY_SCOPE_AGENT);
-            __hip_atomic_store(a.ticket + 1 + blockIdx.x, t, __ATOMIC_RELAXED, __HIP_MEMORY_SCOPE_AGENT);
-            *tk = t;
-        }
-        __syncthreads();
-        bslot = *tk;
-        __syncthreads();
-        if (bslot < 0 || bslot >= a.n_slots) return;
-    }
-    const int chain = a.chain_order ? a.chain_order[bslot] : bslot;
-    if (a.group_flag && ((int)a.group_flag[chain] != a.group_sel || bslot < a.rank_lo || bslot >= a.rank_hi)) return;
-    pmdi_s2::Sweep2<K, PPL, NW, GO> s;
-    s.run(ap, chain);
+    pmdi_s2::sweep_slots<K, PPL, NW, GO>(ap);
 }
 
 template <int K>
@@ -90,10 +73,11 @@
     return hipOccupancyMaxActiveBlocksPerMultiprocessor(blocks, fn, 64 * nw, lds);
 }
 
-hipError_t pmdi_launch_sweep2(const SweepArgs &a_in, SweepArgs *d_args, int n_chains, hipStream_t stream, SweepArgs *staging)
+hipError_t pmdi_launch_sweep2(const SweepArgs &a_in, SweepArgs *d_args, int n_chains, int grid, hipStream_t stream, SweepArgs *staging)
 {
     SweepArgs a = a_in;
     a.n_slots = n_chains;
+    if (grid < 1 || grid > n_chains || (grid < n_chains && !(a.ticket && a.hold == 2))) return hipErrorInvalidValue;
     int nw = 0;
     const void *fn = kernel_for(a.K, a.P, &nw, all_gaussian(a));
     if (!fn) return hipErrorInvalidValue;
@@ -110,7 +94,7 @@
     }
     const SweepArgs *ap = d_args;
     void *args[] = {(void *)&ap};
-    e = hipLaunchKernel(fn, dim3((unsigned)n_chains), dim3(64u * (unsigned)nw), args, lds, stream);
+    e = hipLaunchKernel(fn, dim3((unsigned)grid), dim3(64u * (unsigned)nw), args, lds, stream);
     if (e != hipSuccess) return e;
     return hipGetLastError();
 }
diff --git a/particlemdi.jl_amd/csrc/pmdi_sweep2_body.h b/particlemdi.jl_amd/csrc/pmdi_sweep2_body.h
--- a/particlemdi.jl_amd/csrc/pmdi_sweep2_body.h
+++ b/particlemdi.jl_amd/csrc/pmdi_sweep2_body.h
@@ -2034,4 +2034,55 @@
     s.hand_over(pos, fcode, t_start);
 }
 
+PM2_DEV int word_get(int *p) { return pm2_atomic_add(p, 0); }
+PM2_DEV void word_set(int *p, int v) { pm2_atomic_add(p, v - pm2_atomic_add(p, 0)); }
+
+#ifndef PM2_SLOT_HOOK
+#define PM2_SLOT_HOOK() do { } while (0)
+#endif
+
+template <int K, int PPL, int NW, bool GO>
+PM2_COLD void sweep_chain(const SweepArgs *ap, int chain)
+{
+    const u64 v = (u64)ap;
+    const unsigned lo = (unsigned)PM2_UNI((int)(unsigned)v), hi = (unsigned)PM2_UNI((int)(unsigned)(v >> 32));
+    Sweep2<K, PPL, NW, GO> s;
+    s.run((const SweepArgs *)(((u64)hi << 32) | (u64)lo), PM2_UNI(chain));
 }
+
+template <int K, int PPL, int NW, bool GO>
+PM2_DEV void sweep_slots(const SweepArgs *ap)
+{
+    const auto &a = *ap;
+    const int tid = PM2_TID();
+    int *tk = (int *)PM2_SMEM;
+    for (bool first = true;; first = false) {
+        int bslot = PM2_BID();
+        if (a.ticket) {
+            if (tid == 0) {
+                int t = -1;
+                if (first || a.hold == 2 || (a.hold == 1 && a.heavy_left && word_get(a.heavy_left) <= 0)) {
+                    t = pm2_atomic_add(a.ticket, 1);
+                    word_set(a.ticket + 1 + PM2_BID(), t);
+                }
+                *tk = t;
+            }
+            PM2_BARRIER();
+            bslot = *tk;
+            PM2_BARRIER();
+        } else if (!first) return;
+        if (bslot < 0 || bslot >= a.n_slots) return;
+        const int chain = a.chain_order ? PM2_G(const int, a.chain_order)[bslot] : bslot;
+        if (a.group_flag && ((int)PM2_G(const unsigned char, a.group_flag)[chain] != a.group_sel || bslot < a.rank_lo || bslot >= a.rank_hi)) {
+            if (a.ticket && a.hold) continue;
+            return;
+        }
+        PM2_SLOT_HOOK();
+        if (a.stamp && tid == 0) PM2_G(long long, a.stamp)[(size_t)chain * 2] = PM2_WALLCLOCK();
+        sweep_chain<K, PPL, NW, GO>(ap, chain);
+        if (a.stamp && tid == 0) PM2_G(long long, a.stamp)[(size_t)chain * 2 + 1] = PM2_WALLCLOCK();
+        PM2_BARRIER();
+    }
+}
+
+}
diff --git a/particlemdi.jl_amd/csrc/pmdi_sweep_body.h b/particlemdi.jl_amd/csrc/pmdi_sweep_body.h
--- a/particlemdi.jl_amd/csrc/pmdi_sweep_body.h
+++ b/particlemdi.jl_amd/csrc/pmdi_sweep_body.h
@@ -1243,6 +1243,7 @@
     if (bslot >= a.n_slots) return;
     if (a.group_flag && ((int)a.group_flag[chain] != a.group_sel || bslot < a.rank_lo || bslot >= a.rank_hi)) return;
     if (a.requeue_only && !a.requeue[chain]) return;
+    if (a.heavy_left && tid == 0) __hip_atomic_fetch_add(a.heavy_left, -1, __ATOMIC_RELAXED, __HIP_MEMORY_SCOPE_AGENT);
     }
 #define XSPLIT (a.ksplit != 0)
 #define XCNT (glob(a.xcnt) + (size_t)chain * 32)
@@ -1267,7 +1268,10 @@
     if (tid < PMDI_KMAX_I * 8) sh.wk[tid] = 0;
     if (tid < PMDI_KMAX_I) sh.khint[tid] = 0;
     long long ph_t0 = 0, ph_r0 = 0;
-    if (a.phase && tid == 0) { ph_last = clock64(); ph_t0 = ph_last; ph_r0 = wall_clock64(); }
+    if (a.phase && tid == 0) {
+        ph_last = clock64(); ph_t0 = ph_last; ph_r0 = wall_clock64();
+        if (!RESUME && a.stamp && kd0 == 0) a.stamp[(size_t)chain * 2] = ph_r0;
+    }
 
     for (int p = tid; p < P; p += T) sh.lw[p] = a.lw_init;
     for (int c = tid; c <= P; c += T) { sh.lead_of[c] = PMDI_INF_I; sh.slot_of[c] = 0; }
@@ -1990,6 +1994,7 @@
     }
     if (a.phase && tid == 0) {
         sh.ph[14] = clock64() - ph_t0; sh.ph[15] = wall_clock64() - ph_r0;
+        if (!RESUME && a.stamp && kd0 == 0) a.stamp[(size_t)chain * 2 + 1] = ph_r0 + sh.ph[15];
     }
     __syncthreads();
     if (a.phase && tid < 16 && kd0 == 0) a.phase[(size_t)chain * 16 + tid] = sh.ph[tid];
```

Result: faster. 955.3, median of 6 (+6.0%).
